# Inuri04/pgtg

Hardware: AMD Instinct MI355X
Metric: env-steps/sec (batched random-action rollout) at 1/2/4/8 MI355X (higher is better)
Workload: dtype int32; 1 GPU; configs[4]: 1048576 envs of 5x5 procedural maps split over the GPUs, random actions, auto-reset, RCCL-reduced global step counter; envs_total=1048576, envs_per_gpu=1048576, map=5x5, autoreset=True, parallelism=dp1 (env shards, no data-path collective)

## Files before the change

pgtg_amd/csrc/pgtg_env.hip:

```cpp
#include <hip/hip_runtime.h>

#include <math.h>
#include <stdint.h>
#include <stdio.h>
#include <stdlib.h>
#include <string.h>

#include <algorithm>
#include <array>
#include <cstddef>
#include <string>
#include <vector>

#include "pgtg_device.h"
#include "pgtg_episode.h"
#include "pgtg_rollout.h"
#include "pgtg_policy.h"
#include "pgtg_snapshot.h"

namespace pgtg {
namespace dv {
#define PGTG_TBL_QUAL __constant__ static const
#include "pgtg_tables.h"
#undef PGTG_TBL_QUAL
}
namespace hs {
#define PGTG_TBL_QUAL static const
#include "pgtg_tables.h"
#undef PGTG_TBL_QUAL
}

__shared__ __attribute__((aligned(16))) TablesHead sT;
__shared__ __attribute__((aligned(16))) TablesTail sTX;

__device__ __forceinline__ void stage_bytes(const void* __restrict__ gsrc, void* ldst, int bytes) {
  const int n4 = bytes >> 4, tid = (int)threadIdx.x;
  const uint4* src = reinterpret_cast<const uint4*>(gsrc);
  uint4* dst = reinterpret_cast<uint4*>(ldst);
  uint4 r[4];
#pragma unroll
  for (int j = 0; j < 4; j++) r[j] = src[tid + j * kBlock < n4 ? tid + j * kBlock : 0];
#pragma unroll
  for (int j = 0; j < 4; j++)
    if (tid + j * kBlock < n4) dst[tid + j * kBlock] = r[j];
  for (int k = tid + 4 * kBlock; k < n4; k += kBlock) dst[k] = src[k];
  for (int k = n4 * 4 + tid; k < bytes / 4; k += kBlock)
    reinterpret_cast<uint32_t*>(ldst)[k] = reinterpret_cast<const uint32_t*>(gsrc)[k];
}
__device__ __forceinline__ void stage_tables(const Tables* __restrict__ gtab, bool tail) {
  stage_bytes(gtab, &sT, (int)sizeof(TablesHead));
  if (tail) stage_bytes(reinterpret_cast<const uint8_t*>(gtab) + kTabHead, &sTX, (int)sizeof(TablesTail));
}

__device__ __forceinline__ void lds_barrier() {
  __builtin_amdgcn_fence(__ATOMIC_RELEASE, "workgroup", "local");
  __builtin_amdgcn_s_barrier();
  __builtin_amdgcn_fence(__ATOMIC_ACQUIRE, "workgroup", "local");
}

template <bool BIG>
__device__ __forceinline__ void stage_plan(const uint16_t* __restrict__ plan, int nq, uint32_t* dst, int pdw) {
  const uint4* src = reinterpret_cast<const uint4*>(plan);
  for (int k0 = 0; k0 < (BIG ? nq : 1); k0 += 8) {
    uint4 q[8];
#pragma unroll
    for (int k = 0; k < 8; k++) q[k] = src[k0 + k < nq ? k0 + k : k0];
#pragma unroll
    for (int k = 0; k < 8; k++) {
      if (k0 + k < nq) {
        const uint32_t wv[4] = {q[k].x, q[k].y, q[k].z, q[k].w};
#pragma unroll
        for (int j = 0; j < 4; j++)
          if ((k0 + k) * 4 + j < pdw) dst[(k0 + k) * 4 + j] = wv[j];
      }
    }
  }
}

#ifdef PGTG_STAMPS
__device__ unsigned long long g_stamps[1 << 21];
#define STAMP(k)                                                                          \
  do {                                                                                    \
    if ((threadIdx.x & 63) == 0) {                                                        \
      unsigned long long t_ = __builtin_amdgcn_s_memtime();                               \
      g_stamps[((blockIdx.x * (kBlock / 64) + (threadIdx.x >> 6)) * 32 + (k)) & ((1 << 21) - 1)] = t_; \
    }                                                                                     \
  } while (0)
#define STAMPR(k)                                                                                     \
  do {                                                                                                \
    if ((threadIdx.x & 63) == 0)                                                                      \
      g_stamps[(1 << 20) | ((((blockIdx.x * (kBlock / 64) + (threadIdx.x >> 6)) * 8 + (k))) & ((1 << 20) - 1))] = \
          __builtin_amdgcn_s_memrealtime();                                                           \
  } while (0)
#else
#define STAMP(k) \
  do {           \
  } while (0)
#define STAMPR(k) \
  do {            \
  } while (0)
#endif

__device__ __forceinline__ uint32_t bit81(const uint32_t* m3, int sq) { return (m3[sq >> 5] >> (sq & 31)) & 1u; }

__device__ __forceinline__ int seg_dir(int lx, int ly) {
  bool mx = (unsigned)(lx - 3) <= 2u, my = (unsigned)(ly - 3) <= 2u;
  if (ly == 0 && mx) return 0;
  if (lx == 8 && my) return 1;
  if (ly == 8 && mx) return 2;
  if (lx == 0 && my) return 3;
  return -1;
}

struct EnvView {
  int px, py, vx, vy;
  uint32_t phase, flags, path_len, elapsed;
  uint32_t sg, spawn;
  uint64_t used;
};

__device__ __forceinline__ EnvView rec_view(const EnvRec& e) {
  EnvView v;
  v.px = (int)(int16_t)(e.a.x & 0xffffu);
  v.py = (int)(int16_t)(e.a.x >> 16);
  v.vx = (int)(int16_t)(e.a.y & 0xffffu);
  v.vy = (int)(int16_t)(e.a.y >> 16);
  v.phase = e.a.z & 0xffffu;
  v.flags = (e.a.z >> 16) & 0xfu;
  v.path_len = e.a.z >> 20;
  v.elapsed = e.a.w;
  v.sg = e.b.x;
  v.spawn = e.b.y;
  v.used = (uint64_t)e.b.z | ((uint64_t)e.b.w << 32);
  return v;
}
__device__ __forceinline__ EnvView rec_load(const EnvRec* r, uint64_t i) { return rec_view(r[i]); }
__device__ __forceinline__ void rec_store(EnvRec* r, uint64_t i, const EnvView& v) {
  EnvRec e;
  e.a.x = ((uint32_t)v.px & 0xffffu) | ((uint32_t)v.py << 16);
  e.a.y = ((uint32_t)v.vx & 0xffffu) | ((uint32_t)v.vy << 16);
  e.a.z = (v.phase & 0xffffu) | ((v.flags & 0xfu) << 16) | (v.path_len << 20);
  e.a.w = v.elapsed;
  e.b.x = v.sg;
  e.b.y = v.spawn;
  e.b.z = (uint32_t)v.used;
  e.b.w = (uint32_t)(v.used >> 32);
  r[i] = e;
}

__device__ __forceinline__ uint32_t plan_word_mask(const DevCfg& c, int word) {
  const int t0 = 2 * word;
  return t0 + 1 < c.nt ? ~0u : (t0 < c.nt ? 0xffffu : 0u);
}
__device__ __forceinline__ void store_plan_row(const DevCfg& c, const DevState& S, uint64_t i, const uint32_t* pw, int pdw) {
  uint4* dstp = reinterpret_cast<uint4*>(S.plan + i * (uint64_t)c.plan_stride);
  for (int k = 0; k < c.plan_stride / 8; k++) {
    uint32_t wv[4];
#pragma unroll
    for (int j = 0; j < 4; j++) wv[j] = (k * 4 + j < pdw) ? pw[k * 4 + j] & plan_word_mask(c, k * 4 + j) : 0u;
    dstp[k] = make_uint4(wv[0], wv[1], wv[2], wv[3]);
  }
}

struct Plan {
  uint16_t* p;
  __device__ __forceinline__ uint32_t operator[](int t) const { return p[t]; }
};

template <bool BIG>
__device__ __forceinline__ bool used_bit(const EnvView& v, uint32_t p, int t) {
  return BIG ? (p & kPlanUsed) != 0u : ((v.used >> t) & 1ull) != 0ull;
}

template <bool BIG>
__device__ __forceinline__ uint32_t square_flags(const DevCfg& c, const Plan& pl, const EnvView& v, int x, int y) {
  int tx = x / kTile, ty = y / kTile;
  int lx = x - tx * kTile, ly = y - ty * kTile;
  int t = ty * c.tw + tx;
  uint32_t p = pl[t];
  uint32_t ex = plan_exits(p);
  int sq = lx * 9 + ly;
  uint32_t f = 0;
  uint32_t wall = bit81(sT.wall[ex], sq);
  if (wall) f |= SQ_WALL;
  int d = seg_dir(lx, ly);
  if (d >= 0 && ((ex >> d) & 1u)) {
    if (plan_sgdir(p) == d) f |= used_bit<BIG>(v, p, t) ? SQ_USED : SQ_SUBGOAL;
    if ((int)(v.sg & 0xffu) == t && (int)((v.sg >> 8) & 0xffu) == d) f |= SQ_START;
    if ((int)((v.sg >> 16) & 0xffu) == t && (int)(v.sg >> 24) == d) f |= SQ_FINAL;
  }
  const uint32_t ob = bit81(sT.obst[min(plan_omask(p), (uint32_t)PGTG_N_OBST_MASKS - 1u)], sq);
  uint32_t ot = plan_otype(p);
  if (ot && !wall && ob) f |= SQ_ICE << (ot - 1);
  return f;
}
__device__ __forceinline__ uint32_t square_lanes(const DevCfg& c, const Plan& pl, int x, int y) {
  int tx = x / kTile, ty = y / kTile;
  int lx = x - tx * kTile, ly = y - ty * kTile;
  uint32_t ex = plan_exits(pl[ty * c.tw + tx]);
  return ex ? sTX.lanes[ex][lx * 9 + ly] : 0u;
}
__device__ __forceinline__ bool square_spawner(const DevCfg& c, const Plan& pl, int x, int y) {
  int tx = x / kTile, ty = y / kTile;
  int lx = x - tx * kTile, ly = y - ty * kTile;
  uint32_t ex = plan_exits(pl[ty * c.tw + tx]);
  if (!ex) return false;
  int sq = lx * 9 + ly;
  if (bit81(sT.spawner[ex], sq)) return true;
  uint32_t l = sTX.lanes[ex][sq];
  return (tx == 0 && (l >> 31 & 1u)) || (tx == c.tw - 1 && (l >> 30 & 1u)) || (ty == 0 && (l >> 29 & 1u)) ||
         (ty == c.th - 1 && (l >> 28 & 1u));
}
__device__ __forceinline__ bool inside(const DevCfg& c, int x, int y) {
  return (unsigned)x < (unsigned)c.W && (unsigned)y < (unsigned)c.H;
}
__device__ __forceinline__ int phase_color(const DevCfg& c, uint32_t ph) {
  return (int)ph < c.phase_g ? 0 : ((int)ph < c.phase_gy ? 1 : 2);
}

__device__ __forceinline__ int lane_slot_tw(int tw, const Plan& pl, int x, int y) {
  int tx = x / kTile, ty = y / kTile;
  int lx = x - tx * kTile, ly = y - ty * kTile;
  int t = ty * tw + tx;
  uint32_t ex = plan_exits(pl[t]);
  const int li_raw = sTX.li[ex][lx * 9 + ly];
  const int li = ex ? li_raw : 255;
  return li == 255 ? -1 : t * 32 + li;
}
__device__ __forceinline__ int lane_slot(const DevCfg& c, const Plan& pl, int x, int y) {
  return lane_slot_tw(c.tw, pl, x, y);
}
__device__ __forceinline__ int pinned(int x) {
  __asm__ volatile("" : "+s"(x));
  return x;
}
__device__ __forceinline__ bool square_tlight(const DevCfg& c, const Plan& pl, int x, int y) {
  int tx = x / kTile, ty = y / kTile;
  int lx = x - tx * kTile, ly = y - ty * kTile;
  uint32_t p = pl[ty * c.tw + tx];
  int sq = lx * 9 + ly;
  return plan_otype(p) == 4 && !bit81(sT.wall[plan_exits(p)], sq) && bit81(sT.obst[plan_omask(p)], sq);
}
#ifndef PGTG_OCC_MAX
#define PGTG_OCC_MAX 15
#endif
constexpr int kOccMax = PGTG_OCC_MAX;
static_assert(kOccMax >= 1 && kOccMax <= 15, "4-bit occupancy counters");
__device__ __forceinline__ int occ_get(const uint8_t* o, int s) { return (o[s >> 1] >> ((s & 1) << 2)) & 15; }
__device__ __forceinline__ void occ_put(uint8_t* o, int s, int v) {
  const int sh = (s & 1) << 2;
  o[s >> 1] = (uint8_t)((o[s >> 1] & ~(15 << sh)) | (v << sh));
}
__device__ __forceinline__ void occ_inc(uint8_t* o, int s, bool& sat) {
  const int v = occ_get(o, s);
  if (v >= kOccMax) sat = true;
  else occ_put(o, s, v + 1);
}
__device__ __forceinline__ int occ_at(const DevCfg& c, const Plan& pl, const uint8_t* occ, int x, int y) {
  int s = lane_slot(c, pl, x, y);
  return s < 0 ? 0 : occ_get(occ, s);
}
__device__ __forceinline__ int select32(uint32_t x, int k) {
  int pos = 0;
#pragma unroll
  for (int sh = 16; sh >= 1; sh >>= 1) {
    const int c = __popc(x & ((1u << sh) - 1u));
    const bool up = k >= c;
    k -= up ? c : 0;
    x = up ? x >> sh : x;
    pos += up ? sh : 0;
  }
  return (x & 1u) && k == 0 ? pos : -1;
}
__device__ __forceinline__ int kth_bit(uint32_t m, int k) {
  for (int j = 0; j < k; j++) m &= m - 1u;
  return __ffs((int)m) - 1;
}

struct ProfileCdf {
  uint64_t t[4];
};
__device__ __forceinline__ ProfileCdf pin_profile_cdf(const DevCfg& c) {
  ProfileCdf p;
#pragma unroll
  for (int j = 0; j < 4; j++) {
    uint64_t x = c.profile_t[j];
    __asm__ volatile("" : "+s"(x));
    p.t[j] = x;
  }
  return p;
}
__device__ __forceinline__ int profile_of(const ProfileCdf& p, uint64_t u) {
  int prof = 0;
#pragma unroll
  for (int j = 0; j < 4; j++) prof += (u < p.t[j]) ? 0 : 1;
  return prof;
}

constexpr uint32_t kCarEmpty = 1u << 31;
typedef __attribute__((address_space(1))) uint32_t gu32;
struct CarSlots {
  gu32 *w0, *w1, *id;
  uint64_t n;
  __device__ __forceinline__ CarSlots(const DevState& S, uint64_t i)
      : w0((gu32*)(S.car_w0 + i)), w1((gu32*)(S.car_w1 + i)), id((gu32*)(S.car_id + i)), n(S.n) {
    __asm__ volatile("" : "+v"(w0), "+v"(w1), "+v"(id));
  }
// ... 1981 lines not shown
    }
    if (f & SQ_ICE) {
      used_ice = true;
      if (pcg_double(ice) < c.ice_p) {
        int a = (int)pcg_int(ice, 9);
        pxp = acc_x(a);
        pyp = acc_y(a);
      }
    }
    if (f & SQ_BROKEN) {
      used_broken = true;
      if (pcg_double(broken) < c.broken_p) v.flags |= kFlagFlatTire;
    }
    if (f & SQ_SAND) {
      used_sand = true;
      if (pcg_double(sand) < c.sand_p) {
        cx += pxp;
        cy += pyp;
        v.vx = v.vy = 0;
        break;
      }
    }
    cx += pxp;
    cy += pyp;
  }
  (void)gl_t;
  (void)gl_d;
  if (used_ice) stream_store_state(S.ice, i, ice);
  if (used_broken) stream_store_state(S.broken, i, broken);
  if (used_sand) stream_store_state(S.sand, i, sand);
  if (v.flags & kFlagFlatTire) v.vx = v.vy = 0;
  const bool accel = !(ax == 0 && ay == 0);
  if (S.visited) {
    uint32_t* vis = S.visited + i * (uint64_t)c.vis_words;
    int b = (cx + 2) * c.vis_pitch + (cy + 2);
    if (c.visited_penalty != 0.0 && accel && ((vis[b >> 5] >> (b & 31)) & 1u)) {
      if (c.separate_cost) cost += c.visited_penalty; else reward -= c.visited_penalty;
    }
    vis[b >> 5] |= 1u << (b & 31);
  }
  const int ox = v.px, oy = v.py;
  v.px = cx;
  v.py = cy;
  if (c.still_penalty != 0.0 && !accel && ox == cx && oy == cy) {
    if (c.separate_cost) cost += c.still_penalty; else reward -= c.still_penalty;
  }
  v.elapsed += 1u;
  if (c.max_steps > 0 && (int)v.elapsed >= c.max_steps) v.flags |= kFlagTruncated;
  res.reward = c.separate_cost ? perf : reward;
  res.cost = cost;
  return 0;
}

__device__ __forceinline__ uint32_t expand4(uint32_t x) { return ((x & 15u) * 0x00204081u) & 0x01010101u; }
__device__ __forceinline__ uint32_t udiv_f(uint32_t x, uint32_t d, float inv) {
  uint32_t q = (uint32_t)((float)x * inv);
  if (q * d > x) q--;
  if ((q + 1) * d <= x) q++;
  return q;
}

__device__ __forceinline__ void mark_lines(uint32_t* lm, const uint8_t* dst, uint32_t e, uint32_t OB) {
  const uintptr_t a0 = (uintptr_t)dst, base = a0 >> 7;
  uint32_t l = (uint32_t)(((a0 + (uintptr_t)e * OB) >> 7) - base);
  const uint32_t l1 = (uint32_t)(((a0 + (uintptr_t)(e + 1) * OB - 1) >> 7) - base);
  while (l <= l1) {
    const uint32_t hi = min(l1, l | 31u), n = hi - l + 1u;
    __hip_atomic_fetch_or(lm + (l >> 5), (n == 32u ? ~0u : ((1u << n) - 1u)) << (l & 31u), __ATOMIC_RELAXED,
                          __HIP_MEMORY_SCOPE_WORKGROUP);
    l = hi + 1u;
  }
}

__device__ __forceinline__ void write_obs(uint8_t* __restrict__ dst, uint32_t cnt, uint32_t OB, const uint32_t* st,
                                          const uint8_t* sel, int rank = -1, int nthr = kBlock,
                                          const uint32_t* lm = nullptr) {
  if (rank < 0) rank = (int)threadIdx.x;
  const uint32_t total = cnt * OB;
  const uintptr_t a0 = (uintptr_t)dst;
  const uintptr_t c0 = a0 & ~(uintptr_t)15;
  const uint32_t nchunks = (uint32_t)((a0 + total - c0 + 15) >> 4);
  const float invOB = 1.0f / (float)OB;
  for (uint32_t ch = (uint32_t)rank; ch < nchunks; ch += (uint32_t)nthr) {
    const int r = (int)((intptr_t)(c0 + ((uintptr_t)ch << 4)) - (intptr_t)a0);
    if (lm) {
      const uint32_t li = (uint32_t)(((c0 + ((uintptr_t)ch << 4)) >> 7) - (a0 >> 7));
      if (!((lm[li >> 5] >> (li & 31u)) & 1u)) continue;
    } else if (sel) {
      const intptr_t l0 = (intptr_t)((c0 + ((uintptr_t)ch << 4)) & ~(uintptr_t)127) - (intptr_t)a0;
      const uint32_t llo = l0 < 0 ? 0u : (uint32_t)l0;
      const uint32_t lhi = min((uint32_t)(l0 + 127), total - 1u);
      const uint32_t e0 = udiv_f(llo, OB, invOB), e1 = udiv_f(lhi, OB, invOB);
      bool any = false;
      for (uint32_t e = e0; e <= e1; e++) any = any || sel[e] == 1;
      if (!any) continue;
    }
    uint8_t* cp = dst + r;
    if (r >= 0 && (uint32_t)r + 16u <= total) {
      const uint32_t w = (uint32_t)r >> 5;
      const uint64_t two = (uint64_t)st[w] | ((uint64_t)st[w + 1] << 32);
      const uint32_t bits = (uint32_t)(two >> (r & 31));
#ifdef PGTG_NT_OBS
      typedef unsigned int v4u __attribute__((ext_vector_type(4)));
      v4u o = {expand4(bits), expand4(bits >> 4), expand4(bits >> 8), expand4(bits >> 12)};
      __builtin_nontemporal_store(o, reinterpret_cast<v4u*>(cp));
#else
      *reinterpret_cast<uint4*>(cp) = make_uint4(expand4(bits), expand4(bits >> 4), expand4(bits >> 8), expand4(bits >> 12));
#endif
    } else {
      for (int b = 0; b < 16; b++) {
        const int rb = r + b;
        if (rb >= 0 && (uint32_t)rb < total) cp[b] = (uint8_t)((st[rb >> 5] >> (rb & 31)) & 1u);
      }
    }
  }
}

struct Lds {
  int envs;
  int plan_stride_dw;
  int scratch_dw;
  int traf_dw;
  int hist_dw;
  int seg_bits;
  int sub_envs;
  int stream_words;
  int spread;
  int compact;
  int queue;
  int gen_off;
  int lm_words;
  int stagger;
  int stagger_wgs;
  int ramp_pct;
  int img_in_traf;
  int prio;
  int abl;
};
constexpr int kQueueLanes = 64;
constexpr int kMaxQueueGrid = 4096;
constexpr int kQctrBlocks = 2 * kMaxQueueGrid;
constexpr int kQctrOvfLen = kQctrBlocks + 3;
constexpr int kQctrWords = kQctrOvfLen + 24;
__device__ __forceinline__ uint32_t wave_sum(uint32_t x) {
#pragma unroll
  for (int o = 32; o > 0; o >>= 1) x += (uint32_t)__shfl_xor((int)x, o);
  return x;
}
__host__ __device__ inline uint64_t queue_req_cap(uint64_t nblk, uint64_t grid, int envs) {
  const uint64_t c = 3 * ((nblk + grid - 1) / grid) * (uint64_t)envs;
  return c < (uint64_t)kQueueLanes ? (uint64_t)kQueueLanes : c;
}
constexpr uint64_t kStaggerMaxTicks = 20000;
constexpr int kQueueDepth = 2;
constexpr int kBlockDepth = 3;
constexpr uint32_t kQueueStale = 0x80u;
constexpr int kViewDw = 8;

__host__ __device__ inline uint32_t queue_tag(uint32_t spawn) { return ~spawn; }
__host__ __device__ inline int odd_up(int x) { return x | 1; }
__host__ inline int img_words(int envs, int bits) { return ((int)(((int64_t)envs * bits + 31) / 32) + 2 + 3) & ~3; }

__host__ inline void lds_tail(Lds& l, const DevCfg& c);
__host__ inline Lds lds_layout(const DevCfg& c, int envs) {
  Lds l;
  l.envs = envs;
  l.plan_stride_dw = odd_up((c.nt + 1) / 2);
  l.scratch_dw = c.need_car ? 0 : 3;
  l.traf_dw = c.need_car ? odd_up(c.traf_bytes / 4) : 0;
  l.hist_dw = (c.n_rules > 0 || c.need_car) ? 5 : 0;
  l.seg_bits = c.n_channels * c.win * c.win;
  const int budget_words = 12 * 1024;
  int sub = l.seg_bits > 0 ? (int)(((int64_t)budget_words - 3) * 32 / l.seg_bits) : envs;
  l.sub_envs = sub > envs ? envs : (sub < 1 ? 1 : sub);
  l.stream_words = img_words(l.sub_envs, l.seg_bits);
  l.spread = c.need_car ? 1 : 0;
  l.compact = 1;
  l.queue = !c.need_car && c.n_rules == 0 && !c.fixed_map && !c.generic_channels && envs <= kBlock - 64 && l.sub_envs >= envs;
  l.stagger = 0;
  l.stagger_wgs = 0;
  l.ramp_pct = 25;
  l.img_in_traf = 0;
  l.abl = 0;
  l.prio = 0;
#ifdef PGTG_TUNING
  if (const char* e = getenv("PGTG_ABL")) l.abl = atoi(e);
  if (const char* e = getenv("PGTG_PRIO")) l.prio = atoi(e);
  if (const char* e = getenv("PGTG_RAMP")) l.ramp_pct = atoi(e);
  if (const char* e = getenv("PGTG_SPREAD")) l.spread = atoi(e);
  if (const char* e = getenv("PGTG_COMPACT")) l.compact = atoi(e);
  if (const char* e = getenv("PGTG_QUEUE")) l.queue = l.queue && atoi(e);
#endif
  lds_tail(l, c);
  return l;
}
__host__ inline int tail_bytes(const Lds& l) {
  return kBlock + (l.queue ? 128 : 32) + 4 * l.lm_words + (l.queue && l.envs <= 32 ? 4 * kViewDw * l.envs : 0);
}
__host__ inline void lds_tail(Lds& l, const DevCfg& c) {
  const int64_t total = (int64_t)l.envs * l.seg_bits;
  const int lines = (int)((127 + total) / 128) + 1;
  l.lm_words = (!c.need_car && l.sub_envs >= l.envs && lines <= 64 * 32) ? (lines + 31) / 32 : 0;
#ifdef PGTG_TUNING
  if (const char* e = getenv("PGTG_LINEMASK")) l.lm_words = atoi(e) ? l.lm_words : 0;
#endif
  l.gen_off = (int)(((size_t)l.envs * (l.plan_stride_dw + l.scratch_dw + l.traf_dw + l.hist_dw) + l.stream_words) +
                    tail_bytes(l) / 4);
}
__host__ inline size_t lds_bytes(const Lds& l) {
  return (size_t)4 * ((size_t)l.envs * (l.plan_stride_dw + l.scratch_dw + l.traf_dw + l.hist_dw) + l.stream_words) +
         tail_bytes(l) + (l.queue ? (size_t)4 * kQueueLanes * l.plan_stride_dw : 0);
}

__host__ inline void lds_img_in_traf(Lds& l, const DevCfg& c) {
  if (!c.need_car || !c.obs_fast || l.envs < 1) return;
  if ((int64_t)img_words(l.envs, l.seg_bits) > (int64_t)l.envs * l.traf_dw) return;
  l.img_in_traf = 1;
  l.sub_envs = l.envs;
  l.stream_words = 0;
  l.hist_dw = 7;
  lds_tail(l, c);
}

enum { MODE_STEP = 0, MODE_RESET_SEEDED = 1, MODE_RESET_UNSEEDED = 2, MODE_OBSERVE = 3 };

__device__ __forceinline__ void write_small_outputs(const DevCfg& c, const PgtgOutputs& o, uint64_t i, const EnvView& v,
                                                    const ObsInfo& oi, bool final) {
  if (!final) {
    if (o.position) reinterpret_cast<int2*>(o.position)[i] = make_int2(oi.posx, oi.posy);
    if (o.velocity) reinterpret_cast<int2*>(o.velocity)[i] = make_int2(v.vx, v.vy);
    if (o.next_subgoal) o.next_subgoal[i] = oi.nsd;
  } else {
    if (o.final_position) reinterpret_cast<int2*>(o.final_position)[i] = make_int2(oi.posx, oi.posy);
    if (o.final_velocity) reinterpret_cast<int2*>(o.final_velocity)[i] = make_int2(v.vx, v.vy);
    if (o.final_next_subgoal) o.final_next_subgoal[i] = oi.nsd;
  }
}

template <bool TR, bool BIG>
__device__ __forceinline__ void obs_pass(const DevCfg& c, const DevState& S, const Plan& pl, const EnvView& v,
                                         const PgtgOutputs& o, uint8_t* dst, uint64_t env0, int nb, bool want,
                                         bool final, const uint8_t* sel, uint32_t* st, const Lds& L,
                                         const uint8_t* occ, int slot) {
  for (int sb = 0; sb < nb; sb += L.sub_envs) {
    const int cnt = min(L.sub_envs, nb - sb);
    if (want && slot >= sb && slot < sb + cnt) {
      ObsInfo oi;
      build_obs<TR, BIG, true, !TR>(c, S, pl, v, st, (uint32_t)(slot - sb) * (uint32_t)c.obs_bytes, oi, occ);
      write_small_outputs(c, o, env0 + slot, v, oi, final);
    }
    lds_barrier();
    if (dst)
      write_obs(dst + (env0 + sb) * (uint64_t)c.obs_bytes, (uint32_t)cnt, (uint32_t)c.obs_bytes, st, sel ? sel + sb : nullptr);
    lds_barrier();
  }
}

__device__ __forceinline__ uint64_t stagger_start(const Lds& L, const DevState& S) {
  if (!L.stagger) return 0;
  const uint64_t t0 = wall_clock64();
  if (blockIdx.x == 0 || blockIdx.x >= (unsigned)L.stagger_wgs) return t0;
  const uint64_t span = min(S.wg_ticks[0] * (uint64_t)L.ramp_pct / 100ull, (unsigned long long)kStaggerMaxTicks);
  const uint64_t wait = span * blockIdx.x / (unsigned)L.stagger_wgs;
  while (wall_clock64() - t0 < wait) __builtin_amdgcn_s_sleep(16);
  return t0;
}
__device__ __forceinline__ void stagger_record(const Lds& L, const DevState& S, uint64_t t0) {
  if (L.stagger && blockIdx.x == 0 && threadIdx.x == 0) S.wg_ticks[0] = wall_clock64() - t0;
}

template <bool TR, bool BIG>
__global__ void __launch_bounds__(kBlock, TR ? 3 : 4) k_env(const DevCfg* __restrict__ cfg, const Tables* __restrict__ gtab,
                                                 DevState S, const uint8_t* __restrict__ actions,
                                                 const uint8_t* __restrict__ mask, PgtgOutputs out, int mode, Lds L,
                                                 uint32_t tr_slot) {
  extern __shared__ uint32_t lds[];
  const DevCfg& c = *cfg;
  const int tid = threadIdx.x;
  const uint64_t t_start = TR ? 0 : stagger_start(L, S);
  STAMP(0);
  if ((TR && c.need_car) && mode != MODE_OBSERVE && blockIdx.x == 0 && tid == 0) S.tr_count[tr_slot ^ 1u] = 0u;
  stage_tables(gtab, c.generic_channels || (TR && c.need_car));
  const uint64_t env0 = (uint64_t)blockIdx.x * L.envs;
  const int nb = (int)min((uint64_t)L.envs, S.n - env0);
  const int per_wave = (!L.spread || L.envs >= kBlock) ? 64 : L.envs / 4;
  const bool has_slot = (tid & 63) < per_wave;
  const int slot = has_slot ? (tid >> 6) * per_wave + (tid & 63) : 0;
  const uint64_t i = env0 + slot;
  const bool live = has_slot && slot < nb;
  const int my_slot = slot;
  uint32_t* plan_w = lds + my_slot * L.plan_stride_dw;
  uint32_t* traf_w = lds + L.envs * (L.plan_stride_dw + L.scratch_dw) + my_slot * L.traf_dw;
  uint32_t* hist_w = lds + L.envs * (L.plan_stride_dw + L.scratch_dw + L.traf_dw) + my_slot * L.hist_dw;
  const int env_dw = L.plan_stride_dw + L.scratch_dw + L.traf_dw + L.hist_dw;
  uint32_t* st = (TR && L.img_in_traf) ? lds + L.envs * (L.plan_stride_dw + L.scratch_dw) : lds + L.envs * env_dw;
  uint8_t* sel = reinterpret_cast<uint8_t*>(lds + L.envs * env_dw + L.stream_words);
  uint64_t* wmask = reinterpret_cast<uint64_t*>(sel + kBlock);
  uint32_t* lm = L.lm_words ? reinterpret_cast<uint32_t*>(sel + kBlock + 32) : nullptr;
  const bool img_traf = TR && L.img_in_traf;
  const int xf_off = img_traf ? L.envs * (L.plan_stride_dw + L.scratch_dw + L.traf_dw) + 4
                   : L.envs * L.plan_stride_dw + ((TR && c.need_car) ? L.envs * L.scratch_dw : 0);
  const int xf_dw = img_traf ? L.hist_dw : (TR && c.need_car) ? L.traf_dw : L.scratch_dw;
  uint32_t* xf = lds + xf_off + my_slot * xf_dw;
  uint8_t* occ = reinterpret_cast<uint8_t*>(traf_w);
  uint16_t* sp_l = reinterpret_cast<uint16_t*>(occ + c.sp_cache_off);
  uint8_t* hist = reinterpret_cast<uint8_t*>(hist_w);
  Plan pl{reinterpret_cast<uint16_t*>(plan_w)};

  EnvView v{};
  TrafState ts{0, 0, 0, 0};
  bool occ_sat = false;
  bool occ_valid = false;
  int err = 0;
  int act = 0;
  if (live) {
    v = rec_load(S.rec, i);
    if (mode == MODE_STEP) act = actions[i];
    if ((TR && c.need_car)) {
      uint4 tr4 = S.traf[i];
      ts.n_cars = tr4.x & 0xffffu;
      ts.n_spawners = tr4.x >> 16;
      ts.next_id = tr4.y;
      ts.tail = tr4.z;
      ts.fresh = (tr4.w & kTrafFresh) ? 1u : 0u;
      occ_valid = (tr4.w & kTrafOccValid) != 0u;
    }
    stage_plan<BIG>(S.plan + i * (uint64_t)c.plan_stride, c.plan_dq, plan_w, L.plan_stride_dw);
  }
  for (int k = tid; k < L.lm_words; k += kBlock) lm[k] = 0u;
  lds_barrier();
  if (live && (TR && c.need_car) && occ_valid) {
    const int nw = c.nt * 4;
    const gu32* ob = ts.fresh ? fresh_block(S, i) + S.fresh_occ : (const gu32*)(S.occ + i);
    const uint64_t ostep = ts.fresh ? 1ull : S.n;
    for (int w0 = 0; w0 < nw; w0 += 16) {
      uint32_t r[16];
#pragma unroll
      for (int u = 0; u < 16; u++) r[u] = ob[(uint64_t)min(w0 + u, nw - 1) * ostep];
#pragma unroll
      for (int u = 0; u < 16; u++)
        if (w0 + u < nw) traf_w[w0 + u] = r[u];
    }
  }
  if (live && (TR && c.need_car) && !occ_valid) {
    for (int w = 0; w < c.nt * 4; w++) traf_w[w] = 0u;
    const CarSlots cs(S, i);
    const gu32* rb = ts.fresh ? fresh_block(S, i) : cs.w0;
    const uint64_t rstep = ts.fresh ? 1ull : S.n;
    const int tail = (int)ts.tail, tw = pinned(c.tw);
    uint32_t nx16[16];
#pragma unroll
    for (int g = 0; g < 16; g++) nx16[g] = rb[(uint64_t)(g < tail ? g : 0) * rstep];
    for (int k0 = 0; k0 < tail; k0 += 16) {
      uint32_t a16[16];
#pragma unroll
      for (int g = 0; g < 16; g++) a16[g] = nx16[g];
#pragma unroll
      for (int g = 0; g < 16; g++) nx16[g] = rb[(uint64_t)(k0 + 16 + g < tail ? k0 + 16 + g : 0) * rstep];
      int sl[16];
#pragma unroll
      for (int g = 0; g < 16; g++) sl[g] = lane_slot_tw(tw, pl, (int)(a16[g] & 255u), (int)((a16[g] >> 8) & 255u));
#pragma unroll
      for (int g = 0; g < 16; g++) {
        if (k0 + g < tail && !(a16[g] & kCarEmpty)) {
          if (sl[g] < 0) err = PGTG_E_UNSUPPORTED;
          else occ_inc(occ, sl[g], occ_sat);
        }
      }
    }
  }
  if (live && (TR && c.need_car)) {
    const int nsp = min((int)ts.n_spawners, kSpCache);
    const uint4* src = reinterpret_cast<const uint4*>(S.spawners + i * (uint64_t)S.sp_pitch);
    const int q_last = (int)(S.sp_pitch / 8u) - 1;
    uint4 q4[kSpCache / 8];
#pragma unroll
    for (int q = 0; q < kSpCache / 8; q++) q4[q] = src[min(q, q_last)];
    uint32_t* dl = reinterpret_cast<uint32_t*>(sp_l);
#pragma unroll
    for (int q = 0; q < kSpCache / 8; q++) {
      if (q * 8 < nsp) {
        dl[4 * q] = q4[q].x;
        dl[4 * q + 1] = q4[q].y;
        dl[4 * q + 2] = q4[q].z;
        dl[4 * q + 3] = q4[q].w;
      }
    }
  }
  STAMP(1);
  uint8_t my_sel = 0;
  if (live) {
    if (mode == MODE_STEP) {
      StepResult res{0.0, 0.0, 0u};
      if (!err) err = env_step<TR, BIG>(c, S, i, v, pl, act, res, occ, occ_sat, sp_l, ts, hist);
      if ((TR && c.need_car) && !occ_sat) {
        const int nw = c.nt * 4;
        for (int w = 0; w < nw; w++) S.occ[(uint64_t)w * S.n + i] = traf_w[w];
      }
      occ_valid = (TR && c.need_car) && !occ_sat && err == 0;
      const bool done = (v.flags & (kFlagTerminated | kFlagTruncated)) != 0;
      if (BIG && res.plan_dirty && !(done && c.autoreset && err == 0)) store_plan_row(c, S, i, plan_w, L.plan_stride_dw);
      if (out.reward) out.reward[i] = res.reward;
      if (out.cost) out.cost[i] = res.cost;
      if (out.terminated) out.terminated[i] = (v.flags & kFlagTerminated) ? 1 : 0;
      if (out.truncated) out.truncated[i] = (v.flags & kFlagTruncated) ? 1 : 0;
      if (out.braking) out.braking[i] = (uint8_t)res.triggered;
      my_sel = (done && c.autoreset && err == 0) ? 1 : 0;
      if (lm && my_sel && out.final_obs) mark_lines(lm, out.final_obs + env0 * (uint64_t)c.obs_bytes, (uint32_t)slot, (uint32_t)c.obs_bytes);
    } else if (mode == MODE_RESET_SEEDED || mode == MODE_RESET_UNSEEDED) {
      const bool do_reset = mask == nullptr || mask[i] != 0;
      if (do_reset && mode == MODE_RESET_SEEDED) v.spawn = 0;
      my_sel = do_reset ? 2 : 0;
    }
  }
  if (has_slot) sel[slot] = my_sel;
  const uint8_t* occ_img = occ;
  if (img_traf) {
    if (live) {
      const int pix = min(max(0, v.px), c.W - 1), piy = min(max(0, v.py), c.H - 1);
      const int t = (piy / kTile) * c.tw + pix / kTile;
#pragma unroll
      for (int q = 0; q < 4; q++) hist_w[q] = traf_w[t * 4 + q];
    }
    occ_img = hist;
  }
  STAMP(2);
  const bool single = L.sub_envs >= nb;
  const bool reset_now = my_sel != 0;
  if (L.compact) {
    const uint64_t m = __ballot(reset_now);
    if ((tid & 63) == 0) wmask[tid >> 6] = m;
  }
  int n_final = 0;
  if (L.compact) {
    lds_barrier();
    if (mode == MODE_STEP)
      for (int w = 0; w < kBlock / 64; w++) n_final += __popcll(wmask[w]);
  } else {
    n_final = __syncthreads_count(my_sel == 1);
  }
  const bool want_final = mode == MODE_STEP && n_final && (out.final_obs || out.final_position || out.final_velocity);
  int n_resets = 0, wslot = -1;
  if (L.compact) {
#pragma unroll
    for (int w = 0; w < kBlock / 64; w++) {
      const uint64_t m = wmask[w];
      const int cw = __popcll(m);
      if (tid >= n_resets && tid < n_resets + cw) wslot = w * per_wave + select64(m, tid - n_resets);
      n_resets += cw;
    }
  }
  const int t_help = L.compact ? ((n_resets + 63) / 64) * 64
                               : ((L.spread || L.envs >= kBlock) ? kBlock : ((L.envs + 63) / 64) * 64);
  const bool helpers = single && t_help < kBlock;
  if (single) {
    if (live && (my_sel != 2)) {
      ObsInfo oi;
      build_obs<TR, BIG, true, !TR>(c, S, pl, v, st, (uint32_t)slot * (uint32_t)c.obs_bytes, oi, occ_img, 0, -1, true, false, img_traf);
      write_small_outputs(c, out, i, v, oi, my_sel == 1);
    }
    if (L.compact && reset_now) xf[0] = v.spawn;
    STAMP(28);
    lds_barrier();
    STAMP(29);
    if (want_final && out.final_obs && !helpers)
      write_obs(out.final_obs + env0 * (uint64_t)c.obs_bytes, (uint32_t)nb, (uint32_t)c.obs_bytes, st, sel, -1, kBlock, lm);
  } else {
    if (want_final) obs_pass<TR, BIG>(c, S, pl, v, out, out.final_obs, env0, nb, my_sel == 1, true, sel, st, L, occ, slot);
    if (L.compact) {
      if (reset_now) xf[0] = v.spawn;
      lds_barrier();
    }
  }
  STAMP(3);
  bool tr_push = false;
  if (!L.compact) n_resets = __syncthreads_count(reset_now);
  if (tid == 0 && n_resets) atomicAdd(&S.counters[1], (unsigned long long)n_resets);
  if (helpers && want_final && out.final_obs && tid >= t_help)
    write_obs(out.final_obs + env0 * (uint64_t)c.obs_bytes, (uint32_t)nb, (uint32_t)c.obs_bytes, st, sel, tid - t_help,
              kBlock - t_help, lm);
  if (L.compact) {
    if (wslot >= 0) {
      uint32_t* xw = lds + xf_off + wslot * xf_dw;
      uint32_t* pw = lds + wslot * L.plan_stride_dw;
      const uint64_t iw = env0 + wslot;
      EnvView vv{};
      vv.spawn = xw[0];
      TrafState tw{0, 0, 0, 0};
      const int e2 = env_reset<TR, BIG>(c, S, iw, vv, reinterpret_cast<uint16_t*>(pw), tw);
      store_plan_row(c, S, iw, pw, L.plan_stride_dw);
      xw[0] = ((uint32_t)vv.px & 0xffffu) | ((uint32_t)vv.py << 16);
      xw[1] = vv.sg;
      xw[2] = vv.path_len | (uint32_t)(-e2) << 16;
    }
    lds_barrier();
    if (reset_now) {
      const uint32_t x0 = xf[0], x2 = xf[2];
      v.px = (int)(int16_t)(x0 & 0xffffu);
      v.py = (int)(int16_t)(x0 >> 16);
      v.sg = xf[1];
      v.path_len = x2 & 0xffffu;
      v.spawn += 5u;
      v.used = 0;
      v.flags = 0;
      v.phase = 0;
      v.elapsed = 0;
      v.vx = v.vy = 0;
      const int e2 = -(int)(x2 >> 16);
      if (e2) err = e2;
      tr_push = (TR && c.need_car) && e2 == 0;
      if ((TR && c.need_car) && e2 == 0) ts = TrafState{0, 0, 0, 0};
    }
  } else if (reset_now) {
    int e2 = env_reset<TR, BIG>(c, S, i, v, pl.p, ts);
    if (e2) err = e2;
    tr_push = (TR && c.need_car) && e2 == 0;
    store_plan_row(c, S, i, plan_w, L.plan_stride_dw);
  }
  STAMP(4);
  if (live) {
    if (mode != MODE_OBSERVE) {
      rec_store(S.rec, i, v);
      if ((TR && c.need_car))
        S.traf[i] = make_uint4(ts.n_cars | ts.n_spawners << 16, ts.next_id, ts.tail,
                               (occ_valid && !reset_now ? kTrafOccValid : 0u) | (ts.fresh ? kTrafFresh : 0u));
    }
    if (mode != MODE_OBSERVE || err) S.err[i] = (uint8_t)(-err);
    if (S.qstate && reset_now) S.qstate[i] = (uint8_t)kQueueStale;
  }
  if (TR && c.need_car) {
    const uint64_t m = __ballot(tr_push);
    if (m) {
      const int lane = tid & 63, leader = __ffsll((long long)m) - 1;
      uint32_t base = 0;
      if (lane == leader) base = atomicAdd(&S.tr_count[tr_slot], (uint32_t)__popcll(m));
      base = __shfl(base, leader);
      if (tr_push) S.tr_list[base + __popcll(m & ((1ull << lane) - 1ull))] = (uint32_t)i;
    }
  }
  STAMP(5);
  if (single) {
    if (helpers && !L.compact) lds_barrier();
    if (reset_now) {
      ObsInfo oi;
      build_obs<TR, BIG, true, !TR>(c, S, pl, v, st, (uint32_t)slot * (uint32_t)c.obs_bytes, oi, nullptr);
      write_small_outputs(c, out, i, v, oi, false);
    }
    STAMP(30);
    lds_barrier();
    STAMP(31);
    if (out.obs)
      write_obs(out.obs + env0 * (uint64_t)c.obs_bytes, (uint32_t)nb, (uint32_t)c.obs_bytes, st, nullptr);
  } else {
    obs_pass<TR, BIG>(c, S, pl, v, out, out.obs, env0, nb, live, false, nullptr, st, L, reset_now ? nullptr : occ,
                 slot);
  }
  if (mode == MODE_STEP && tid == 0) atomicAdd(&S.counters[0], (unsigned long long)nb);
  if (!TR) stagger_record(L, S, t_start);
  STAMP(6);
  if (TR) STAMPR(0);
}

template <bool BIG>
__device__ __forceinline__ void gen_queue_entry(const DevCfg& c, const DevState& S, uint64_t i, uint32_t k,
                                                uint16_t* plan, int pdw, uint32_t* __restrict__ dst,
                                                bool no_store = false, bool fold_ok = true) {
  SeedPool sp = ss_pool(S.seed[i]);
  Pcg map_rng = ss_child(sp, k);
  int st_t, st_d, gl_t, gl_d;
  uint64_t ix[4];
  generate_map<BIG>(c, BIG ? S.epk : sT.epk, map_rng, plan, st_t, st_d, gl_t, gl_d, ix);
  uint64_t dirs[4] = {0ull, 0ull, 0ull, 0ull};
  const bool fold = !BIG && c.dual && fold_ok;
  int len = compile_generated<BIG>(c, plan, st_t, gl_t, ix, fold ? dirs : nullptr);
  int px = 0, py = 0, err = 0;
  if (len <= 0 || !((plan_exits(plan[st_t]) >> st_d) & 1u)) {
    err = len < 0 ? PGTG_E_DEVICE : PGTG_E_MAP;
    len = 0;
  } else {
    const int j = (int)pcg_int(map_rng, 3);
    const int tx = st_t % c.tw, ty = st_t / c.tw;
    int lx, ly;
    switch (st_d) {
      case 0: lx = 3 + j; ly = 0; break;
      case 1: lx = 8; ly = 3 + j; break;
      case 2: lx = 3 + j; ly = 8; break;
      default: lx = 0; ly = 3 + j; break;
    }
    px = tx * kTile + lx;
    py = ty * kTile + ly;
  }
  const uint32_t* pw = reinterpret_cast<const uint32_t*>(plan);
  uint4* d4 = reinterpret_cast<uint4*>(dst);
  const int pwords = c.plan_dq * 4;
#ifdef PGTG_TUNING
  if (no_store) {
    if (len == 12345 && px == 7) d4[0] = make_uint4(0, 0, 0, 0);
    return;
  }
#endif
  for (int q = 0; q < pwords / 4; q++) {
    uint32_t wv[4];
#pragma unroll
    for (int j = 0; j < 4; j++) {
      wv[j] = (q * 4 + j < pdw) ? (pw[q * 4 + j] & plan_word_mask(c, q * 4 + j)) : 0u;
      if (fold) {
        const int t0 = 2 * (q * 4 + j);
        const uint32_t d0 = (uint32_t)((dirs[0] >> t0) & 1ull) + 2u * (uint32_t)((dirs[1] >> t0) & 1ull) +
                            3u * (uint32_t)((dirs[2] >> t0) & 1ull) + 4u * (uint32_t)((dirs[3] >> t0) & 1ull);
        const uint32_t d1 = t0 + 1 < 64 ? (uint32_t)((dirs[0] >> (t0 + 1)) & 1ull) + 2u * (uint32_t)((dirs[1] >> (t0 + 1)) & 1ull) +
                                          3u * (uint32_t)((dirs[2] >> (t0 + 1)) & 1ull) + 4u * (uint32_t)((dirs[3] >> (t0 + 1)) & 1ull)
                                        : 0u;
        wv[j] |= (d0 << 11 | d1 << 27) & plan_word_mask(c, q * 4 + j);
      }
    }
    d4[q] = make_uint4(wv[0], wv[1], wv[2], wv[3]);
  }
  d4[pwords / 4] = make_uint4(((uint32_t)px & 0xffffu) | ((uint32_t)py << 16),
                              (uint32_t)st_t | (uint32_t)st_d << 8 | (uint32_t)gl_t << 16 | (uint32_t)gl_d << 24,
                              (uint32_t)len | (uint32_t)(-err) << 16, queue_tag(k));
  for (int q = pwords / 4 + 1; q < c.qrec_dw / 4; q++) d4[q] = make_uint4(0u, 0u, 0u, 0u);
}

#ifdef PGTG_TUNING
#define ABLATE(L, bit) (((L).abl & (bit)) != 0)
#else
#define ABLATE(L, bit) false
#endif

__device__ __forceinline__ void sub_barrier(uint32_t* ctr, uint32_t target) {
  __builtin_amdgcn_fence(__ATOMIC_RELEASE, "workgroup", "local");
  if ((threadIdx.x & 63) == 0) __hip_atomic_fetch_add(ctr, 1u, __ATOMIC_RELAXED, __HIP_MEMORY_SCOPE_WORKGROUP);
  while (__hip_atomic_load(ctr, __ATOMIC_RELAXED, __HIP_MEMORY_SCOPE_WORKGROUP) < target) __builtin_amdgcn_s_sleep(1);
  __builtin_amdgcn_fence(__ATOMIC_ACQUIRE, "workgroup", "local");
}

template <bool BIG>
__device__ __forceinline__ void group_obs(const DevCfg& c, const DevState& S, const EnvView& v, bool want,
                                          uint32_t* st, ObsInfo& oi, const Lds& L, int wave, int lane,
                                          uint32_t* ctr, uint32_t& bar, int np, int rank, uint32_t* vw,
                                          bool post = true) {
  const int vtid = wave * 64 + lane;
  const int E = L.envs;
  if (E <= 32) {
    if (wave == 0 && lane < E) {
      uint32_t* q = vw + lane * kViewDw;
      q[0] = (uint32_t)v.px;
      q[1] = (uint32_t)v.py;
      q[2] = v.sg;
      q[3] = v.phase;
      q[4] = (uint32_t)v.used;
      q[5] = (uint32_t)(v.used >> 32);
      q[6] = want ? 1u : 0u;
    }
    sub_barrier(ctr, bar += (uint32_t)np);
    STAMP(post ? 9 : 16);
    const int G = np * 64 / E, e = rank % E, sub = rank / E;
    if (sub >= G) return;
    const uint32_t* q = vw + e * kViewDw;
    if (!q[6]) return;
    const int C = c.n_channels, lo = sub * C / G, hi = (sub + 1) * C / G;
    if (lo == hi && sub != 0) return;
    EnvView ve{};
    ve.px = (int)q[0];
    ve.py = (int)q[1];
    ve.sg = q[2];
    ve.phase = q[3];
    ve.used = (uint64_t)q[4] | (uint64_t)q[5] << 32;
    STAMP(post ? 10 : 17);
    extern __shared__ uint32_t lds[];
    const Plan pl{reinterpret_cast<uint16_t*>(lds + e * L.plan_stride_dw)};
    build_obs<false, BIG, false, false>(c, S, pl, ve, st, (uint32_t)e * (uint32_t)c.obs_bytes, oi, nullptr, lo, hi, sub == 0,
                                 true);
    STAMP(post ? 11 : 18);
    return;
  }
  if (want) {
    extern __shared__ uint32_t lds[];
    const int slot = vtid;
    const Plan pl{reinterpret_cast<uint16_t*>(lds + slot * L.plan_stride_dw)};
    build_obs<false, BIG, false, false>(c, S, pl, v, st, (uint32_t)slot * (uint32_t)c.obs_bytes, oi, nullptr);
  }
}

template <bool BIG>
__device__ __forceinline__ uint3 ring_take(const DevCfg& c, const DevState& S, const Lds& L, uint64_t i, uint32_t qh,
                                           uint32_t k0, uint32_t* plan_w, int pdw, int depth = kQueueDepth) {
  const uint4* q4 = reinterpret_cast<const uint4*>(S.qbuf + (i * (uint64_t)depth + qh) * (uint64_t)c.qrec_dw);
  uint4* dstp = reinterpret_cast<uint4*>(S.plan + i * (uint64_t)c.plan_stride);
  const int nq = c.plan_dq;
  const uint4 meta = q4[nq];
  for (int k0q = 0; k0q < (BIG ? nq : 1); k0q += 8) {
    uint4 qw[8];
#pragma unroll
    for (int k = 0; k < 8; k++) qw[k] = q4[k0q + k < nq ? k0q + k : k0q];
#pragma unroll
    for (int k = 0; k < 8; k++) {
      if (k0q + k < nq) {
        if (!ABLATE(L, 32)) dstp[k0q + k] = qw[k];
        const uint32_t wv[4] = {qw[k].x, qw[k].y, qw[k].z, qw[k].w};
#pragma unroll
        for (int j = 0; j < 4; j++)
          if ((k0q + k) * 4 + j < pdw) plan_w[(k0q + k) * 4 + j] = wv[j];
      }
    }
  }
  if (!ABLATE(L, 32))
    for (int k = nq; k < c.plan_stride / 8; k++) dstp[k] = make_uint4(0u, 0u, 0u, 0u);
  if (c.need_ice || c.need_broken || c.need_sand) {
    SeedPool sp = ss_pool(S.seed[i]);
    if (c.need_ice) stream_store_all(S.ice, i, ss_child(sp, k0 + 2u));
    if (c.need_broken) stream_store_all(S.broken, i, ss_child(sp, k0 + 3u));
    if (c.need_sand) stream_store_all(S.sand, i, ss_child(sp, k0 + 4u));
  }
  const int e2 = (meta.w != queue_tag(k0) && !ABLATE(L, 1 | 16)) ? PGTG_E_DEVICE : -(int)(meta.z >> 16);
  return make_uint3(meta.x, meta.y, (meta.z & 0xffffu) | (uint32_t)(-e2) << 16);
}

template <bool BIG>
__global__ void __launch_bounds__(kBlock, 4) k_envq(const DevCfg* __restrict__ cfg, const Tables* __restrict__ gtab,
                                                    DevState S, const uint8_t* __restrict__ actions, PgtgOutputs out,
                                                    Lds L, uint32_t qsel) {
  extern __shared__ uint32_t lds[];
  const DevCfg& c = *cfg;
  const int tid = threadIdx.x, wave = tid >> 6, lane = tid & 63;
  const uint64_t t_start = stagger_start(L, S);
  STAMP(0);
  STAMPR(2);
  const int env_waves = (L.envs + 63) / 64, gen_wave = env_waves;
  const bool env_wave = wave < env_waves;
  const uint32_t par = qsel >> 2;
  const uint64_t nblk = (S.n + (uint64_t)L.envs - 1) / (uint64_t)L.envs;
  const uint64_t cap = queue_req_cap(nblk, gridDim.x, L.envs);
  uint2* req_new = S.qreq + ((uint64_t)par * gridDim.x + blockIdx.x) * cap;
  const uint2* req_old = S.qreq + ((uint64_t)(par ^ 1u) * gridDim.x + blockIdx.x) * cap;
  const bool one_round = nblk <= gridDim.x;
  const uint32_t ox = blockIdx.x & 7u, set_new = qsel & 3u, set_old = (set_new + 2u) % 3u;
  const uint64_t ocap = ((gridDim.x + 7u) / 8u) * (uint64_t)L.envs;
  uint32_t cnt = 0;
  uint2 r0 = make_uint2(0u, 0u);
  if (wave == gen_wave) {
    cnt = S.qctr[(par ^ 1u) * gridDim.x + blockIdx.x];
    r0 = req_old[lane];
  }
  if (blockIdx.x == 0 && tid < 8) S.qctr[kQctrOvfLen + ((set_new + 1u) % 3u) * 8u + tid] = 0u;
  const int pdw = L.plan_stride_dw;
  stage_tables(gtab, false);
  uint32_t* st = lds + L.envs * (pdw + L.scratch_dw + L.traf_dw + L.hist_dw);
  uint8_t* sel = reinterpret_cast<uint8_t*>(st + L.stream_words);
  uint32_t* ctr = reinterpret_cast<uint32_t*>(sel + kBlock);
  uint32_t* lm = L.lm_words ? reinterpret_cast<uint32_t*>(sel + kBlock + 128) : nullptr;
  uint32_t* vw = reinterpret_cast<uint32_t*>(sel + kBlock + 128) + L.lm_words;
  uint32_t* qn = ctr + 1;
  uint32_t* nxt = ctr + 2;
  uint32_t* bctr = S.qctr + kQctrBlocks;
  if (blockIdx.x == 0 && tid == 0) bctr[((qsel & 3u) + 1u) % 3u] = 0u;
  if (tid == 0) {
    *ctr = 0u;
    *qn = 0u;
  }
  lds_barrier();

  if (wave == gen_wave) {
    STAMP(1);
    uint16_t* gplan = reinterpret_cast<uint16_t*>(lds + L.gen_off + lane * pdw);
    uint32_t made = 0, ovs = 0;
    if (!ABLATE(L, 1)) {
      const uint2* ovf = S.qovf + ((uint64_t)(par ^ 1u) * 8u + ox) * ocap;
      uint32_t ob = 0, on = 0, olen = 0, tot = 0;
      const uint32_t nj = (gridDim.x - ox + 7u) / 8u, jme = blockIdx.x / 8u;
      if (one_round) {
        olen = S.qctr[kQctrOvfLen + set_old * 8u + ox];
        if (olen > 0) {
          uint32_t pre = 0;
          for (uint32_t j0 = 0; j0 < nj; j0 += kQueueLanes) {
            const uint32_t j = j0 + (uint32_t)lane;
            const uint32_t sp = j < nj ? kQueueLanes - min(S.qctr[(par ^ 1u) * gridDim.x + ox + 8u * j], (uint32_t)kQueueLanes) : 0u;
            pre += wave_sum(j < jme ? sp : 0u);
            tot += wave_sum(sp);
          }
          on = olen > pre ? min(olen - pre, kQueueLanes - min(cnt, (uint32_t)kQueueLanes)) : 0u;
          ob = pre;
        }
      }
      for (uint32_t base = 0;; base += kQueueLanes) {
        const uint32_t own = base < cnt ? min((uint32_t)kQueueLanes, cnt - base) : 0u;
        const uint32_t oth = base == 0 ? on : 0u;
        if (own + oth == 0) break;
        made += own + oth;
        ovs += oth;
        if ((uint32_t)lane < own + oth) {
          const uint2 r = (uint32_t)lane >= own ? ovf[ob + (lane - own)] : base == 0 ? r0 : req_old[base + lane];
          const uint64_t ie = r.x >> 1;
          gen_queue_entry<BIG>(c, S, ie, r.y, gplan, pdw, S.qbuf + (ie * kQueueDepth + (r.x & 1u)) * (uint64_t)c.qrec_dw,
                               ABLATE(L, 16), false);
        }
        if (base + kQueueLanes >= cnt) break;
      }
      for (uint64_t st0 = tot + (uint64_t)jme * kQueueLanes; st0 < olen; st0 += (uint64_t)nj * kQueueLanes) {
        const uint32_t m = (uint32_t)min((uint64_t)kQueueLanes, olen - st0);
        made += m;
        ovs += m;
        if ((uint32_t)lane < m) {
          const uint2 r = ovf[st0 + lane];
          const uint64_t ie = r.x >> 1;
          gen_queue_entry<BIG>(c, S, ie, r.y, gplan, pdw, S.qbuf + (ie * kQueueDepth + (r.x & 1u)) * (uint64_t)c.qrec_dw,
                               ABLATE(L, 16), false);
        }
      }
    }
    if (lane == 0 && made) atomicAdd(&S.counters[2], (unsigned long long)made);
    if (lane == 0 && ovs) atomicAdd(&S.counters[3], (unsigned long long)ovs);
    STAMP(7);
    STAMPR(3);
    return;
  }

  const int np = kBlock / 64 - 1;
  const int nthr = np * 64;
  uint32_t bar = 0;
  for (uint64_t blk = blockIdx.x; blk < nblk;) {
    STAMP(0);
    uint32_t got = 0xffffffffu;
    if (tid == 0 && nblk > gridDim.x && *qn + 2u * (uint32_t)L.envs <= cap) got = atomicAdd(&bctr[qsel & 3u], 1u);
    int tid_o = tid;
    asm volatile("" : "+v"(tid_o));
    const int lane = tid_o & 63;
    const int rank = (wave < gen_wave ? wave : wave - 1) * 64 + lane;
    const int slot = tid_o;
    uint32_t* plan_w = lds + (env_wave ? slot : 0) * pdw;
    Plan pl{reinterpret_cast<uint16_t*>(plan_w)};
    const uint64_t env0 = blk * (uint64_t)L.envs;
    const int nb = (int)min((uint64_t)L.envs, S.n - env0);
    const uint64_t i = env0 + slot;
    const bool live = env_wave && slot < nb;
    EnvView v{};
    uint32_t qh = 0;
    int act = 0;
    if (live) {
      v = rec_load(S.rec, i);
      qh = S.qstate[i] & 1u;
      act = actions[i];
      stage_plan<BIG>(S.plan + i * (uint64_t)c.plan_stride, c.plan_dq, plan_w, pdw);
    }
    for (int k = rank; k < L.lm_words; k += nthr) lm[k] = 0u;
    sub_barrier(ctr, bar += (uint32_t)np);
    STAMP(1);
    uint8_t my_sel = 0;
    int err = 0;
    if (live) {
      StepResult res{0.0, 0.0, 0u};
      bool occ_sat = false;
      TrafState ts{0, 0, 0, 0};
      err = env_step<false, BIG>(c, S, i, v, pl, act, res, nullptr, occ_sat, nullptr, ts, nullptr);
      STAMP(22);
      const bool done = (v.flags & (kFlagTerminated | kFlagTruncated)) != 0;
      if (out.reward) out.reward[i] = res.reward;
      if (out.cost) out.cost[i] = res.cost;
      if (out.terminated) out.terminated[i] = (v.flags & kFlagTerminated) ? 1 : 0;
      if (out.truncated) out.truncated[i] = (v.flags & kFlagTruncated) ? 1 : 0;
      if (out.braking) out.braking[i] = 0;
      my_sel = (done && c.autoreset && err == 0) ? 1 : 0;
      if (BIG && res.plan_dirty && !my_sel) store_plan_row(c, S, i, plan_w, pdw);
      if (lm && my_sel && out.final_obs) mark_lines(lm, out.final_obs + env0 * (uint64_t)c.obs_bytes, (uint32_t)slot, (uint32_t)c.obs_bytes);
      STAMP(23);
    }
    {
      ObsInfo oi;
      group_obs<BIG>(c, S, v, live, st, oi, L, wave, lane, ctr, bar, np, rank, vw);
      if (live) write_small_outputs(c, out, i, v, oi, my_sel == 1);
    }
    if (env_wave) sel[slot] = my_sel;
    const uint64_t rm = __ballot(my_sel == 1);
    if (env_wave && lane == 0 && rm) atomicAdd(&S.counters[1], (unsigned long long)__popcll(rm));
    STAMP(2);
    STAMP(28);
    sub_barrier(ctr, bar += (uint32_t)np);
    STAMP(29);
    if (out.final_obs && !ABLATE(L, 2))
      write_obs(out.final_obs + env0 * (uint64_t)c.obs_bytes, (uint32_t)nb, (uint32_t)c.obs_bytes, st, sel, rank, nthr, lm);
    STAMP(3);
    sub_barrier(ctr, bar += (uint32_t)np);
    const bool reset_now = my_sel != 0;
    const uint32_t k0 = v.spawn;
    if (reset_now) {
      const uint4* q4 = reinterpret_cast<const uint4*>(S.qbuf + (i * kQueueDepth + qh) * (uint64_t)c.qrec_dw);
      uint4* dstp = reinterpret_cast<uint4*>(S.plan + i * (uint64_t)c.plan_stride);
      const int nq = c.plan_dq;
      const uint4 meta = q4[nq];
      for (int k0q = 0; k0q < (BIG ? nq : 1); k0q += 8) {
        uint4 qw[8];
#pragma unroll
        for (int k = 0; k < 8; k++) qw[k] = q4[k0q + k < nq ? k0q + k : k0q];
#pragma unroll
        for (int k = 0; k < 8; k++) {
          if (k0q + k < nq) {
            if (!ABLATE(L, 32)) dstp[k0q + k] = qw[k];
            const uint32_t wv[4] = {qw[k].x, qw[k].y, qw[k].z, qw[k].w};
#pragma unroll
            for (int j = 0; j < 4; j++)
              if ((k0q + k) * 4 + j < pdw) plan_w[(k0q + k) * 4 + j] = wv[j];
          }
        }
      }
      if (!ABLATE(L, 32))
        for (int k = nq; k < c.plan_stride / 8; k++) dstp[k] = make_uint4(0u, 0u, 0u, 0u);
      if (c.need_ice || c.need_broken || c.need_sand) {
        SeedPool sp = ss_pool(S.seed[i]);
        if (c.need_ice) stream_store_all(S.ice, i, ss_child(sp, k0 + 2u));
        if (c.need_broken) stream_store_all(S.broken, i, ss_child(sp, k0 + 3u));
        if (c.need_sand) stream_store_all(S.sand, i, ss_child(sp, k0 + 4u));
      }
      v.spawn = k0 + 5u;
      v.sg = meta.y;
      v.used = 0;
      v.path_len = meta.z & 0xffffu;
      v.flags = 0;
      v.phase = 0;
      v.elapsed = 0;
      v.vx = v.vy = 0;
      v.px = (int)(int16_t)(meta.x & 0xffffu);
      v.py = (int)(int16_t)(meta.x >> 16);
      const int e2 = (meta.w != queue_tag(k0) && !ABLATE(L, 1 | 16)) ? PGTG_E_DEVICE : -(int)(meta.z >> 16);
      if (e2) err = e2;
      if (S.visited && e2 == 0) {
        uint32_t* vis = S.visited + i * (uint64_t)c.vis_words;
        for (int q2 = 0; q2 < c.vis_words; q2++) vis[q2] = 0;
        int b = (v.px + 2) * c.vis_pitch + (v.py + 2);
        vis[b >> 5] |= 1u << (b & 31);
      }
    }
    STAMP(4);
    const uint64_t rb = __ballot(reset_now);
    if (rb) {
      uint32_t base = 0;
      if (lane == 0) base = atomicAdd(qn, (uint32_t)__popcll(rb));
      base = __builtin_amdgcn_readfirstlane(base);
      const uint32_t k = (uint32_t)__popcll(rb);
      const uint32_t ovn = (one_round && base + k > (uint32_t)kQueueLanes) ? base + k - max(base, (uint32_t)kQueueLanes) : 0u;
      uint32_t obase = 0;
      if (ovn) {
        if (lane == 0) obase = atomicAdd(&S.qctr[kQctrOvfLen + set_new * 8u + ox], ovn);
        obase = __builtin_amdgcn_readfirstlane(obase);
      }
      if (reset_now) {
        const uint32_t p = base + (uint32_t)__popcll(rb & ((1ull << lane) - 1ull));
        const uint2 r = make_uint2((uint32_t)i << 1 | qh, k0 + 10u);
        if (one_round && p >= (uint32_t)kQueueLanes)
          S.qovf[((uint64_t)par * 8u + ox) * ocap + obase + (p - max(base, (uint32_t)kQueueLanes))] = r;
        else
          req_new[p] = r;
        S.qstate[i] = (uint8_t)(qh ^ 1u);
      }
    }
    if (live) {
      rec_store(S.rec, i, v);
      S.err[i] = (uint8_t)(-err);
    }
    STAMP(5);
    {
      ObsInfo oi;
      group_obs<BIG>(c, S, v, reset_now, st, oi, L, wave, lane, ctr, bar, np, rank, vw, false);
      if (reset_now) write_small_outputs(c, out, i, v, oi, false);
    }
    if (tid == 0) *nxt = got;
    STAMP(30);
    sub_barrier(ctr, bar += (uint32_t)np);
    STAMP(31);
    if (tid == 0)
      S.qctr[par * gridDim.x + blockIdx.x] = one_round ? min(*qn, (uint32_t)kQueueLanes) : *qn;
    const uint32_t g = *nxt;
    if (out.obs && !ABLATE(L, 4))
      write_obs(out.obs + env0 * (uint64_t)c.obs_bytes, (uint32_t)nb, (uint32_t)c.obs_bytes, st, nullptr, rank, nthr);
    if (tid == 0) atomicAdd(&S.counters[0], (unsigned long long)nb);
    if (blk == blockIdx.x) stagger_record(L, S, t_start);
    STAMP(6);
    blk = g == 0xffffffffu ? nblk : (uint64_t)gridDim.x + g;
  }  STAMPR(3);
}

template <bool BIG>
__global__ void __launch_bounds__(kBlock, 4) k_envb(const DevCfg* __restrict__ cfg, const Tables* __restrict__ gtab,
                                                    DevState S, const uint8_t* __restrict__ actions, PgtgOutputs out,
                                                    Lds L) {
  extern __shared__ uint32_t lds[];
  const DevCfg& c = *cfg;
  const int tid = threadIdx.x, wave = tid >> 6, lane = tid & 63;
  const uint64_t t_start = stagger_start(L, S);
  STAMP(0);
  STAMPR(2);
  stage_tables(gtab, false);
  const uint64_t env0 = (uint64_t)blockIdx.x * L.envs;
  const int nb = (int)min((uint64_t)L.envs, S.n - env0);
  const int env_waves = (L.envs + 63) / 64, gen_wave = env_waves;
#ifdef PGTG_TUNING
  if (wave != gen_wave) {
    if (L.prio == 1) __builtin_amdgcn_s_setprio(1);
    else if (L.prio == 2) __builtin_amdgcn_s_setprio(2);
    else if (L.prio == 3) __builtin_amdgcn_s_setprio(3);
  }
#endif
  const int qcap = env_waves > 2 ? 2 * kQueueLanes : kQueueLanes;
  const bool env_wave = wave < env_waves;
  const int slot = tid;
  const uint64_t i = env0 + slot;
  const bool live = env_wave && slot < nb;
  const int pdw = L.plan_stride_dw;
  uint32_t* plan_w = lds + (env_wave ? slot : 0) * pdw;
  uint32_t* xf = lds + L.envs * pdw;
  uint32_t* st = lds + L.envs * (pdw + L.scratch_dw + L.traf_dw + L.hist_dw);
  uint8_t* sel = reinterpret_cast<uint8_t*>(st + L.stream_words);
  uint64_t* fm = reinterpret_cast<uint64_t*>(sel + kBlock);
  uint32_t* ctr = reinterpret_cast<uint32_t*>(fm + 3 * kBlockDepth);
  uint32_t* lm = L.lm_words ? reinterpret_cast<uint32_t*>(sel + kBlock + 128) : nullptr;
  uint32_t* vw = reinterpret_cast<uint32_t*>(sel + kBlock + 128) + L.lm_words;
  Plan pl{reinterpret_cast<uint16_t*>(plan_w)};

  EnvView v{};
  uint32_t qs = 0;
  int act = 0;
  if (live) {
    v = rec_load(S.rec, i);
    qs = S.qstate[i];
    act = actions[i];
    stage_plan<BIG>(S.plan + i * (uint64_t)c.plan_stride, c.plan_dq, plan_w, pdw);
    xf[slot * L.scratch_dw] = v.spawn;
    xf[slot * L.scratch_dw + 1] = qs;
  }
  const uint32_t qn = qs & 3u, qh = (qs >> 2) & 3u;
  if (env_wave) {
#pragma unroll
    for (int l = 0; l < kBlockDepth; l++) {
      const uint64_t m = __ballot(live && qn <= (uint32_t)l);
      if (lane == 0) fm[l * 3 + wave] = m;
    }
  }
  if (tid == 0) *ctr = 0u;
  for (int k = tid; k < L.lm_words; k += kBlock) lm[k] = 0u;
  lds_barrier();
  STAMP(1);
  int F[kBlockDepth];
#pragma unroll
  for (int l = 0; l < kBlockDepth; l++) {
    F[l] = 0;
    for (int w = 0; w < env_waves; w++) F[l] += __popcll(fm[l * 3 + w]);
  }
  const bool any_empty = F[0] != 0;
#ifdef PGTG_STAMPS
  if ((threadIdx.x & 63) == 0)
    g_stamps[((blockIdx.x * (kBlock / 64) + (threadIdx.x >> 6)) * 32 + 12) & ((1 << 21) - 1)] =
        (unsigned long long)F[0] | (unsigned long long)F[1] << 16 | (unsigned long long)F[2] << 32;
#endif

  if (wave == gen_wave) {
    uint16_t* gplan = reinterpret_cast<uint16_t*>(lds + L.gen_off + lane * pdw);
    auto refill = [&](int k, int l) {
      int e = 0, pre = 0;
      for (int w = 0; w < env_waves; w++) {
        const uint64_t m = fm[l * 3 + w];
        const int cw = __popcll(m);
        if (k >= pre && k < pre + cw) e = w * 64 + select64(m, k - pre);
        pre += cw;
      }
      const uint64_t ie = env0 + e;
      const uint32_t qe = xf[e * L.scratch_dw + 1];
      const uint32_t rslot = (((qe >> 2) & 3u) + (uint32_t)l) % (uint32_t)kBlockDepth;
      gen_queue_entry<BIG>(c, S, ie, xf[e * L.scratch_dw] + 5u * (uint32_t)l, gplan, pdw,
                      S.qbuf + (ie * kBlockDepth + rslot) * (uint64_t)c.qrec_dw, ABLATE(L, 16), !ABLATE(L, 512));
    };
    if (ABLATE(L, 1)) {
      if (any_empty) __syncthreads();
      return;
    }
    for (int k = lane; k < F[0]; k += kQueueLanes) refill(k, 0);
    if (any_empty) __syncthreads();
    for (int k0 = lane; k0 < qcap; k0 += kQueueLanes) {
      int k = k0, l = 1;
      while (l < kBlockDepth && k >= F[l]) {
        k -= F[l];
        l++;
      }
      if (l < kBlockDepth) refill(k, l);
    }
    if (lane == 0) {
      int rest = 0;
      for (int l = 1; l < kBlockDepth; l++) rest += F[l];
      atomicAdd(&S.counters[2], (unsigned long long)(F[0] + min(rest, qcap)));
    }
    STAMP(7);
    STAMPR(3);
    return;
  }

  const int np = kBlock / 64 - 1;
  const int rank = (wave < gen_wave ? wave : wave - 1) * 64 + lane, nthr = np * 64;
  uint32_t bar = 0;
  uint8_t my_sel = 0;
  int err = 0;
  if (live) {
    StepResult res{0.0, 0.0, 0u};
    bool occ_sat = false;
    TrafState ts{0, 0, 0, 0};
    err = env_step<false, BIG>(c, S, i, v, pl, act, res, nullptr, occ_sat, nullptr, ts, nullptr);
    STAMP(22);
    const bool done = (v.flags & (kFlagTerminated | kFlagTruncated)) != 0;
    if (out.reward) out.reward[i] = res.reward;
    if (out.cost) out.cost[i] = res.cost;
    if (out.terminated) out.terminated[i] = (v.flags & kFlagTerminated) ? 1 : 0;
    if (out.truncated) out.truncated[i] = (v.flags & kFlagTruncated) ? 1 : 0;
    if (out.braking) out.braking[i] = 0;
    my_sel = (done && c.autoreset && err == 0) ? 1 : 0;
    if (BIG && res.plan_dirty && !my_sel) store_plan_row(c, S, i, plan_w, pdw);
    if (lm && my_sel && out.final_obs) mark_lines(lm, out.final_obs + env0 * (uint64_t)c.obs_bytes, (uint32_t)slot, (uint32_t)c.obs_bytes);
    STAMP(23);
  }
  {
    ObsInfo oi;
    group_obs<BIG>(c, S, v, live, st, oi, L, wave, lane, ctr, bar, np, rank, vw);
    if (live) write_small_outputs(c, out, i, v, oi, my_sel == 1);
  }
  if (env_wave) sel[slot] = my_sel;
  const uint64_t rm = __ballot(my_sel == 1);
  if (env_wave && lane == 0 && rm) atomicAdd(&S.counters[1], (unsigned long long)__popcll(rm));
  STAMP(2);
  STAMP(28);
  sub_barrier(ctr, bar += (uint32_t)np);
  STAMP(29);
  if (out.final_obs && !ABLATE(L, 2))
    write_obs(out.final_obs + env0 * (uint64_t)c.obs_bytes, (uint32_t)nb, (uint32_t)c.obs_bytes, st,
              ABLATE(L, 128) ? nullptr : sel, rank, nthr, ABLATE(L, 128) ? nullptr : lm);
  STAMP(3);
  sub_barrier(ctr, bar += (uint32_t)np);
  if (any_empty) __syncthreads();
  const bool reset_now = my_sel != 0;
  if (reset_now) {
    const uint32_t k0 = v.spawn;
    const uint3 tk = ring_take<BIG>(c, S, L, i, qh, k0, plan_w, pdw, kBlockDepth);
    v.spawn = k0 + 5u;
    v.sg = tk.y;
    v.used = 0;
    v.path_len = tk.z & 0xffffu;
    v.flags = 0;
    v.phase = 0;
    v.elapsed = 0;
    v.vx = v.vy = 0;
    v.px = (int)(int16_t)(tk.x & 0xffffu);
    v.py = (int)(int16_t)(tk.x >> 16);
    const int e2 = -(int)(tk.z >> 16);
    if (e2) err = e2;
    if (S.visited && e2 == 0) {
      uint32_t* vis = S.visited + i * (uint64_t)c.vis_words;
      for (int q2 = 0; q2 < c.vis_words; q2++) vis[q2] = 0;
      int b = (v.px + 2) * c.vis_pitch + (v.py + 2);
      vis[b >> 5] |= 1u << (b & 31);
    }
  }
  STAMP(4);
  if (live) {
    rec_store(S.rec, i, v);
    S.err[i] = (uint8_t)(-err);
    uint32_t have = qn == 0u ? 1u : qn;
    int base = 0;
#pragma unroll
    for (int l = 1; l < kBlockDepth; l++) {
      int pre = 0;
      for (int w = 0; w < wave; w++) pre += __popcll(fm[l * 3 + w]);
      if (qn <= (uint32_t)l && base + pre + __popcll(fm[l * 3 + wave] & ((1ull << lane) - 1ull)) < qcap) have++;
      base += F[l];
    }
    const uint32_t nq = reset_now ? have - 1u : have;
    const uint32_t nh = reset_now ? (qh + 1u) % (uint32_t)kBlockDepth : qh;
    S.qstate[i] = (uint8_t)(nq | nh << 2);
  }
  STAMP(5);
  {
    ObsInfo oi;
    group_obs<BIG>(c, S, v, reset_now, st, oi, L, wave, lane, ctr, bar, np, rank, vw, false);
    if (reset_now) write_small_outputs(c, out, i, v, oi, false);
  }
  STAMP(30);
  sub_barrier(ctr, bar += (uint32_t)np);
  STAMP(31);
  if (out.obs && !ABLATE(L, 4))
    write_obs(out.obs + env0 * (uint64_t)c.obs_bytes, (uint32_t)nb, (uint32_t)c.obs_bytes, st, nullptr, rank, nthr);
  if (tid == 0) atomicAdd(&S.counters[0], (unsigned long long)nb);
  stagger_record(L, S, t_start);
  STAMP(6);
  STAMPR(3);
}


template <bool BIG>
__global__ void __launch_bounds__(kBlock) k_qfill(const DevCfg* __restrict__ cfg, const Tables* __restrict__ gtab,
                                                  DevState S, int pdw) {
  extern __shared__ uint32_t lds[];
  const DevCfg& c = *cfg;
  stage_tables(gtab, false);
  lds_barrier();
  const uint64_t i = (uint64_t)blockIdx.x * kBlock + threadIdx.x;
  uint32_t made = 0;
  if (i < S.n) {
    const uint32_t qs = S.qstate[i];
    const bool stale = (qs & kQueueStale) != 0;
    const uint32_t qh = stale ? 0u : (qs & 1u);
    const uint32_t spawn = S.rec[i].b.y;
    const int tag_w = c.plan_dq * 4 + 3;
    uint16_t* plan = reinterpret_cast<uint16_t*>(lds + threadIdx.x * pdw);
    for (uint32_t l = 0; l < (uint32_t)kQueueDepth; l++) {
      uint32_t* dst = S.qbuf + (i * kQueueDepth + (qh ^ l)) * (uint64_t)c.qrec_dw;
      if (stale || dst[tag_w] != queue_tag(spawn + 5u * l)) {
        gen_queue_entry<BIG>(c, S, i, spawn + 5u * l, plan, pdw, dst);
        made++;
      }
    }
    if (stale) S.qstate[i] = 0;
  }
  const uint32_t wsum = (uint32_t)__popcll(__ballot(made & 1u)) + 2u * (uint32_t)__popcll(__ballot(made & 2u));
  if ((threadIdx.x & 63) == 0 && wsum) atomicAdd(&S.counters[2], (unsigned long long)wsum);
}

template <bool BIG>
__global__ void __launch_bounds__(kBlock) k_qfill_b(const DevCfg* __restrict__ cfg, const Tables* __restrict__ gtab,
                                                    DevState S, int pdw) {
  extern __shared__ uint32_t lds[];
  const DevCfg& c = *cfg;
  stage_tables(gtab, false);
  lds_barrier();
  const uint64_t i = (uint64_t)blockIdx.x * kBlock + threadIdx.x;
  uint32_t made = 0;
  if (i < S.n) {
    const uint32_t qs = S.qstate[i];
    const uint32_t qn = (qs & kQueueStale) ? 0u : (qs & 3u), qh = (qs & kQueueStale) ? 0u : ((qs >> 2) & 3u);
    if (qn < (uint32_t)kBlockDepth) {
      const uint32_t spawn = S.rec[i].b.y;
      uint16_t* plan = reinterpret_cast<uint16_t*>(lds + threadIdx.x * pdw);
      for (uint32_t l = qn; l < (uint32_t)kBlockDepth; l++)
        gen_queue_entry<BIG>(c, S, i, spawn + 5u * l, plan, pdw,
                             S.qbuf + (i * kBlockDepth + (qh + l) % (uint32_t)kBlockDepth) * (uint64_t)c.qrec_dw);
      S.qstate[i] = (uint8_t)((uint32_t)kBlockDepth | qh << 2);
      made = (uint32_t)kBlockDepth - qn;
    }
  }
  const uint32_t wsum = (uint32_t)__popcll(__ballot(made & 1u)) + 2u * (uint32_t)__popcll(__ballot(made & 2u));
  if ((threadIdx.x & 63) == 0 && wsum) atomicAdd(&S.counters[2], (unsigned long long)wsum);
}

#ifdef PGTG_STAMPS
__global__ void __launch_bounds__(kBlock) k_gen_bench(const DevCfg* __restrict__ cfg, const Tables* __restrict__ gtab,
                                                      DevState S, int reps, int active, int pdw) {
  extern __shared__ uint32_t lds[];
  const DevCfg& c = *cfg;
  {
    const uint32_t* src = reinterpret_cast<const uint32_t*>(gtab);
    uint32_t* dstt = reinterpret_cast<uint32_t*>(&sT);
    for (int k = threadIdx.x; k < (int)(sizeof(TablesHead) / 4); k += blockDim.x) dstt[k] = src[k];
  }
  __syncthreads();
  const uint64_t i = (uint64_t)blockIdx.x * kBlock + threadIdx.x;
  uint16_t* plan = reinterpret_cast<uint16_t*>(lds + threadIdx.x * pdw);
  unsigned long long tg = 0, tc = 0;
  uint32_t chk = 0;
  if ((threadIdx.x & 63) < active && i < S.n) {
    SeedPool sp = ss_pool(S.seed[i]);
    for (int r = 0; r < reps; r++) {
      Pcg g = ss_child(sp, 5u * (uint32_t)r);
      int st_t, st_d, gl_t, gl_d;
      const unsigned long long t0 = __builtin_amdgcn_s_memtime();
      uint64_t ix[4];
      generate_map<false>(c, sT.epk, g, plan, st_t, st_d, gl_t, gl_d, ix);
      const unsigned long long t1 = __builtin_amdgcn_s_memtime();
      const int len = compile_generated<false>(c, plan, st_t, gl_t, ix);
      const unsigned long long t2 = __builtin_amdgcn_s_memtime();
      tg += t1 - t0;
      tc += t2 - t1;
      chk += (uint32_t)len + plan[st_t];
    }
  }
  const uint64_t wv = (uint64_t)blockIdx.x * (kBlock / 64) + (threadIdx.x >> 6);
  if ((threadIdx.x & 63) == 0) {
    g_stamps[(wv * 32 + 0) & ((1 << 21) - 1)] = tg;
    g_stamps[(wv * 32 + 1) & ((1 << 21) - 1)] = tc;
  }
  if (chk == 0xdeadbeefu) S.err[i] = 1;
}
#endif

__global__ void __launch_bounds__(kBlock) k_traffic(const DevCfg* __restrict__ cfg, const Tables* __restrict__ gtab,
                                                    DevState S, PgtgOutputs out, uint32_t tr_slot, int plan_dw,
                                                    int rs_dw, int cap_w) {
  extern __shared__ uint32_t lds[];
  STAMP(27);
  STAMPR(1);
  const DevCfg& c = *cfg;
  const uint32_t n = S.tr_count[tr_slot];
  const uint32_t W = gridDim.x * (kBlock / 64);
  const uint32_t rounds = (n + W * (uint32_t)cap_w - 1) / (W * (uint32_t)cap_w);
  if (rounds == 0) return;
  const uint32_t e = (n + W * rounds - 1) / (W * rounds);
  if ((uint64_t)blockIdx.x * (kBlock / 64) * e >= n) return;
  const int g = min(kMaxGroup, 64 / (int)e);
  const int wave = (int)(threadIdx.x >> 6), lane = (int)(threadIdx.x & 63u);
  const int slot = lane / g, sub = lane - slot * g;
  stage_tables(gtab, true);
  __syncthreads();
  STAMP(25);
#ifdef PGTG_STAMPS
  if ((threadIdx.x & 63) == 0)
    g_stamps[((blockIdx.x * (kBlock / 64) + (threadIdx.x >> 6)) * 32 + 15) & ((1 << 21) - 1)] =
        (unsigned long long)n | (unsigned long long)rounds << 32 | (unsigned long long)e << 40 | (unsigned long long)cap_w << 48;
#endif
  if ((uint32_t)slot >= e) return;
  const int ls = wave * cap_w + slot;
  uint32_t* plan_w = lds + ls * plan_dw;
  uint8_t* rs = reinterpret_cast<uint8_t*>(lds + (kBlock / 64) * cap_w * plan_dw + ls * rs_dw);
  for (uint32_t r = 0; r < rounds; r++) {
    const uint32_t j = (r * W + blockIdx.x * (kBlock / 64) + (uint32_t)wave) * e + (uint32_t)slot;
    if (j >= n) break;
    const uint64_t i = S.tr_list[j];
    if (c.nt > kSmallTiles) stage_plan<true>(S.plan + i * (uint64_t)c.plan_stride, c.plan_dq, plan_w, plan_dw);
    else stage_plan<false>(S.plan + i * (uint64_t)c.plan_stride, c.plan_dq, plan_w, plan_dw);
    Plan pl{reinterpret_cast<uint16_t*>(plan_w)};
    const EnvView v = rec_load(S.rec, i);
    const int pix = min(max(0, v.px), c.W - 1), piy = min(max(0, v.py), c.H - 1);
    const int at = (piy / kTile) * c.tw + pix / kTile;
    Pcg cr = stream_load(S.car, i);
    TrafState ts{0, 0, 0, 0};
    uint32_t CR[3] = {0u, 0u, 0u};
    const int err = traffic_reset(c, S, i, pl, cr, rs, ts, at, CR, sub, g);
    const int q0 = lane - sub;
    const int err0 = __shfl(err, q0), k0 = __shfl((int)ts.n_cars, q0);
    if (err0 == 0) {
      store_initial_counters(c, S, i, pl, rs, k0, sub, g);
      if (!c.obs_fast && c.traffic_ch >= 0 && out.obs && k0 > 0) {
        const int win = c.win;
        const int x0 = c.sliding ? v.px - c.ss : (pix / kTile) * kTile;
        const int y0 = c.sliding ? v.py - c.ss : (piy / kTile) * kTile;
        const uint16_t* sqs = reinterpret_cast<const uint16_t*>(rs);
        uint8_t* o = out.obs + i * (uint64_t)c.obs_bytes + (uint64_t)c.traffic_ch * (uint64_t)(win * win);
        for (int m = sub; m < k0; m += g) {
          const uint32_t code = sqs[m];
          const int a = (int)(code & 255u) - x0, b = (int)(code >> 8) - y0;
          if (a >= 0 && a < win && b >= 0 && b < win) o[a * win + b] = 1;
        }
      }
    }
    if (sub == 0) {
      stream_store_state(S.car, i, cr);
      S.traf[i] = make_uint4(ts.n_cars | ts.n_spawners << 16, ts.next_id, ts.tail, err == 0 ? kTrafOccValid | kTrafFresh : 0u);
      if (err) S.err[i] = (uint8_t)(-err);
      if (c.obs_fast && c.traffic_ch >= 0 && out.obs) {
        uint8_t* o = out.obs + i * (uint64_t)c.obs_bytes + (uint64_t)c.traffic_ch * 81u;
#pragma unroll
        for (int k = 0; k < 3; k++) {
          uint32_t m = CR[k];
          while (m) {
            const int b = __ffs((int)m) - 1;
            m &= m - 1u;
            o[k * 32 + b] = 1;
          }
        }
      }
    }
    wave_lds_sync();
  }
  STAMP(24);
}

__global__ void __launch_bounds__(kBlock) k_squares(const DevCfg* __restrict__ cfg, const Tables* __restrict__ gtab,
                                                    DevState S, uint64_t i, uint64_t* __restrict__ words) {
  __shared__ uint16_t plan_s[kMaxTiles];
  const DevCfg& c = *cfg;
  const int tid = threadIdx.x;
  {
    const uint32_t* src = reinterpret_cast<const uint32_t*>(gtab);
    uint32_t* dstt = reinterpret_cast<uint32_t*>(&sT);
    for (int k = tid; k < (int)(sizeof(TablesHead) / 4); k += blockDim.x) dstt[k] = src[k];
    uint32_t* dstx = reinterpret_cast<uint32_t*>(&sTX);
    for (int k = tid; k < (int)(sizeof(TablesTail) / 4); k += blockDim.x) dstx[k] = src[kTabHead / 4 + k];
    for (int t = tid; t < c.nt; t += blockDim.x) plan_s[t] = S.plan[i * (uint64_t)c.plan_stride + t];
  }
  __syncthreads();
  const EnvView v = rec_load(S.rec, i);
  const Plan pl{plan_s};
  for (int q = tid; q < c.W * c.H; q += blockDim.x) {
    const int x = q / c.H, y = q - x * c.H;
    const uint32_t f = c.nt > kSmallTiles ? square_flags<true>(c, pl, v, x, y) : square_flags<false>(c, pl, v, x, y);
    uint64_t w = square_lanes(c, pl, x, y);
    if (f & SQ_WALL) w |= 1ull << 32;
    if (square_spawner(c, pl, x, y)) w |= 1ull << 37;
    if (f & SQ_START) w |= 1ull << 38;
    if (f & SQ_SUBGOAL) w |= 1ull << 39;
    if (f & SQ_USED) w |= 1ull << 40;
    if (f & SQ_FINAL) w |= 1ull << 41;
    if (f & SQ_ICE) w |= 1ull << 42;
    if (f & SQ_BROKEN) w |= 1ull << 43;
    if (f & SQ_SAND) w |= 1ull << 44;
    if (f & SQ_TLIGHT) w |= 1ull << 45;
    words[q] = w;
  }
}

__global__ void k_random_actions(uint8_t* a, uint64_t n, uint64_t seed, uint64_t t, uint64_t offset) {
  uint64_t i = (uint64_t)blockIdx.x * blockDim.x + threadIdx.x;
  if (i >= n) return;
  const uint64_t g = i + offset;
  uint64_t z = seed ^ (t * 0x9E3779B97F4A7C15ull) ^ (g * 0xD1B54A32D192ED03ull);
  z += 0x9E3779B97F4A7C15ull;
  z = (z ^ (z >> 30)) * 0xBF58476D1CE4E5B9ull;
  z = (z ^ (z >> 27)) * 0x94D049BB133111EBull;
  z ^= z >> 31;
  a[i] = (uint8_t)(((z >> 32) * 9ull) >> 32);
}

typedef unsigned int u32x4 __attribute__((ext_vector_type(4)));
template <int U, bool NT>
__global__ void __launch_bounds__(256) k_hbm_copy(const u32x4* __restrict__ src, u32x4* __restrict__ dst, uint64_t n16) {
  const uint64_t stride = (uint64_t)gridDim.x * 256 * U;
  for (uint64_t b = (uint64_t)blockIdx.x * 256 * U + threadIdx.x; b < n16; b += stride) {
    u32x4 r[U];
#pragma unroll
    for (int j = 0; j < U; j++) {
      const uint64_t k = b + j * 256 < n16 ? b + j * 256 : b;
      r[j] = NT ? __builtin_nontemporal_load(src + k) : src[k];
    }
#pragma unroll
    for (int j = 0; j < U; j++)
      if (b + j * 256 < n16) {
        if (NT) __builtin_nontemporal_store(r[j], dst + b + j * 256);
        else dst[b + j * 256] = r[j];
      }
  }
}

__device__ __forceinline__ uint64_t dg_w(uint64_t j) {
  uint64_t z = j + 1 + 0x9E3779B97F4A7C15ull;
  z = (z ^ (z >> 30)) * 0xBF58476D1CE4E5B9ull;
  z = (z ^ (z >> 27)) * 0x94D049BB133111EBull;
  return z ^ (z >> 31);
}
__global__ void __launch_bounds__(256) k_car_digest(DevState S, uint64_t* __restrict__ out) {
  const uint64_t i = (uint64_t)blockIdx.x * blockDim.x + threadIdx.x;
  if (i >= S.n) return;
  constexpr uint64_t CB = 1ull << 40;
  const uint4 t = S.traf[i];
  const CarSlots cs(S, i);
  const bool fresh = (t.w & kTrafFresh) != 0u;
  const gu32* fb = fresh_block(S, i);
  uint64_t d = (uint64_t)(t.x & 0xffffu) * dg_w(CB), j = 0;
  for (int k = 0; k < (int)t.z; k++) {
    const uint32_t w0 = fresh ? fb[k] : cs.w0[cs.at(k)];
    if (w0 & kCarEmpty) continue;
    const uint32_t id = fresh ? (uint32_t)k : cs.id[cs.at(k)];
    const uint64_t pk = (uint64_t)id | (uint64_t)(w0 & 255u) << 32 | (uint64_t)((w0 >> 8) & 255u) << 40 |
                        (uint64_t)((w0 >> 16) & 31u) << 48 | (uint64_t)((w0 >> 21) & 7u) << 53 |
                        (uint64_t)((w0 >> 24) & 3u) << 56;
    const uint32_t w1 = fresh ? 0u : cs.w1[cs.at(k)];
    d += (pk + 1) * dg_w(CB + 1 + 2 * j) + (uint64_t)w1 * dg_w(CB + 2 + 2 * j);
    j++;
  }
  out[i] = d;
}

struct FlatArgs {
  const uint8_t* obs;
  const int32_t* pos;
  const int32_t* vel;
  const int32_t* nsd;
  const uint8_t* term;
  const uint8_t* trunc;
  void* dst;
  const double* rew;
  float* rew32;
  uint8_t* dones;
  uint8_t* tonly;
  const uint8_t* fobs;
  const int32_t* fpos;
  const int32_t* fvel;
  const int32_t* fnsd;
  void* fdst;
  uint64_t n;
  int32_t D, OB, w2, cw2, nsd_on, final;
  uint8_t order[PGTG_MAX_CHANNELS];
};
template <typename T>
__device__ __forceinline__ T flat_tail(const FlatArgs& a, int k, int nsdv, int px, int py, int vx, int vy) {
  if (a.nsd_on) {
    if (k < 9) return (T)(k == nsdv ? 1 : 0);
    k -= 9;
  }
  if (k < 9) return (T)(k == px ? 1 : 0);
  if (k < 18) return (T)(k - 9 == py ? 1 : 0);
  return (T)(k == 18 ? vx : vy);
}
typedef uint32_t u32x4 __attribute__((ext_vector_type(4)));
constexpr int kFlatU = 18;
__device__ __forceinline__ void* uniform_ptr(const void* p) {
  const uint64_t u = (uint64_t)(uintptr_t)p;
  const uint32_t lo = __builtin_amdgcn_readfirstlane((uint32_t)u), hi = __builtin_amdgcn_readfirstlane((uint32_t)(u >> 32));
  return (void*)(uintptr_t)((uint64_t)hi << 32 | lo);
}
__device__ __forceinline__ void flat_store(__amdgpu_buffer_rsrc_t r, uint32_t off, float v) {
  __builtin_amdgcn_raw_buffer_store_b32(__builtin_bit_cast(uint32_t, v), r, off, 0, 0);
}
__device__ __forceinline__ void flat_store(__amdgpu_buffer_rsrc_t r, uint32_t off, int8_t v) {
  __builtin_amdgcn_raw_buffer_store_b8((uint8_t)v, r, off, 0, 0);
}
template <typename T, int V>
__device__ __forceinline__ void flat_store_v(__amdgpu_buffer_rsrc_t r, uint32_t off, const T (&f)[V]) {
  if constexpr (V == 1) {
    flat_store(r, off, f[0]);
  } else {
    static_assert(V == 2 && sizeof(T) == 4, "pairs of float32 only");
    typedef uint32_t u32x2 __attribute__((ext_vector_type(2)));
    const u32x2 x = {__builtin_bit_cast(uint32_t, f[0]), __builtin_bit_cast(uint32_t, f[1])};
    __builtin_amdgcn_raw_buffer_store_b64(x, r, off, 0, 0);
  }
}
template <typename T, bool ONE, int V>
__global__ void __launch_bounds__(256, 6) k_flatten(FlatArgs a) {
  __shared__ uint32_t offs[kFlatU * 64];
  __shared__ uint32_t rows[512];
  __shared__ uint32_t nrows;
  const int t = threadIdx.x;
  const uint32_t D = (uint32_t)a.D, w2 = (uint32_t)a.w2, cw2 = (uint32_t)a.cw2;
  for (uint32_t j = t; j < (uint32_t)(kFlatU * 64); j += 256) {
    const uint32_t slot = j < cw2 ? j / w2 : 0u;
    offs[j] = j < cw2 ? (uint32_t)a.order[slot] * w2 + (j - slot * w2) : 0u;
  }
  if (t == 0) nrows = 0u;
  __syncthreads();
  const uint64_t K = (a.n + gridDim.x - 1) / gridDim.x;
  const uint64_t e = (uint64_t)blockIdx.x * K + (uint64_t)t;
// ... 38 lines not shown
    const uint32_t lo4 = (uint32_t)ln * 4u, ovel = ln >= 2 ? lo4 - 8u : 1u << 20, onsd = ln >= 4 ? lo4 - 16u : 1u << 20;
    uint32_t offv[NC + 1][V];
#pragma unroll
    for (int u = 0; u <= NC; u++)
#pragma unroll
      for (int h = 0; h < V; h++) {
        const uint32_t j = (uint32_t)(V * ln + h) + (u == NC ? pb : (uint32_t)u) * CH;
        offv[u][h] = j < cw2 ? offs[j] : 0u;
      }
    auto load_row = [&](uint32_t r, Row& m) {
      const uint32_t ent = __builtin_amdgcn_readfirstlane(rows[r]);
      const bool fr = ent >= 256u;
      const uint64_t er = (uint64_t)blockIdx.x * K + (ent & 255u);
      const uint8_t* orow = (fr ? a.fobs : a.obs) + er * (uint64_t)OB;
      T* row = reinterpret_cast<T*>(fr ? a.fdst : a.dst) + er * (uint64_t)D;
      const auto src = __builtin_amdgcn_make_buffer_rsrc(uniform_ptr(orow), 0, (int)OB, 0x00020000);
      m.dst = __builtin_amdgcn_make_buffer_rsrc(uniform_ptr(row), 0,
                                                __builtin_amdgcn_readfirstlane((int)(D * sizeof(T))), 0x00020000);
      m.dsto = __builtin_amdgcn_make_buffer_rsrc(uniform_ptr(row), 0,
                                                 __builtin_amdgcn_readfirstlane((int)(pb * CH * sizeof(T))), 0x00020000);
      const auto dpos = __builtin_amdgcn_make_buffer_rsrc(uniform_ptr((fr ? a.fpos : a.pos) + 2 * er), 0, 8, 0x00020000);
      const auto dvel = __builtin_amdgcn_make_buffer_rsrc(uniform_ptr((fr ? a.fvel : a.vel) + 2 * er), 0, 8, 0x00020000);
      const auto dnsd = __builtin_amdgcn_make_buffer_rsrc(
          uniform_ptr(a.nsd_on ? (fr ? a.fnsd : a.nsd) + er : (fr ? a.fpos : a.pos)), 0, a.nsd_on ? 4 : 0, 0x00020000);
      m.mv[0] = (int)__builtin_amdgcn_raw_buffer_load_b32(dpos, lo4, 0, 0);
      m.mv[1] = (int)__builtin_amdgcn_raw_buffer_load_b32(dvel, ovel, 0, 0);
      m.mv[2] = (int)__builtin_amdgcn_raw_buffer_load_b32(dnsd, onsd, 0, 0);
      m.q0 = __builtin_amdgcn_raw_buffer_load_b128(src, lo4 * 4u, 0, 0);
      m.q1 = __builtin_amdgcn_raw_buffer_load_b128(src, 1024u + lo4 * 4u, 0, 0);
      m.tb = __builtin_amdgcn_raw_buffer_load_b8(src, obt + (uint32_t)ln, 0, 0);
    };
    auto store_row = [&](const Row& m) {
      win[wv][ln] = m.q0;
      win[wv][64 + ln] = m.q1;
      if ((uint32_t)ln < OB - obt) wb[obt + (uint32_t)ln] = (uint8_t)m.tb;
      const int mv = m.mv[0] + m.mv[1] + m.mv[2];
      const int px = __builtin_amdgcn_readlane(mv, 0), py = __builtin_amdgcn_readlane(mv, 1);
      const int vx = __builtin_amdgcn_readlane(mv, 2), vy = __builtin_amdgcn_readlane(mv, 3);
      const int nsdv = __builtin_amdgcn_readlane(mv, 4) + 1;
#pragma unroll
      for (int p = 0; p < NC; p++) {
        T f[V];
#pragma unroll
        for (int h = 0; h < V; h++) f[h] = (T)wb[offv[p][h]];
        flat_store_v<T, V>(m.dsto, lo + (uint32_t)p * CH * (uint32_t)sizeof(T), f);
      }
      uint32_t obb[V];
#pragma unroll
      for (int h = 0; h < V; h++) obb[h] = wb[offv[NC][h]];
#pragma unroll
      for (int s = 0; s < 2; s++) {
        const uint32_t pc = pb + (uint32_t)s;
        T f[V];
#pragma unroll
        for (int h = 0; h < V; h++) {
          const int k = V * ln + h + (int)(pc * CH) - (int)cw2;
          const int k2 = a.nsd_on ? k - 9 : k;
          int tv = (int)(k2 == px);
          tv = k2 < 9 ? tv : (int)(k2 - 9 == py);
          tv = k2 < 18 ? tv : (k2 == 18 ? vx : vy);
          tv = (a.nsd_on && k < 9) ? (int)(k == nsdv) : tv;
          f[h] = k < 0 ? (T)obb[h] : (T)tv;
        }
        if (pc * CH < D) flat_store_v<T, V>(m.dst, lo + pc * CH * (uint32_t)sizeof(T), f);
      }
    };
    Row mA{}, mB{};
    uint32_t r = wv;
    if (r < nr) {
      load_row(r, mA);
      load_row(min(r + 4u, nr - 1u), mB);
      store_row(mA);
      r += 4u;
      while (r < nr) {
        load_row(min(r + 4u, nr - 1u), mA);
        store_row(mB);
        r += 4u;
        if (r >= nr) break;
        load_row(min(r + 4u, nr - 1u), mB);
        store_row(mA);
        r += 4u;
      }
    }
  } else {
    for (uint32_t r = wv; r < nr; r += 4u) {
      const uint32_t ent = rows[r];
      const bool fr = ent >= 256u;
      const uint64_t er = (uint64_t)blockIdx.x * K + (ent & 255u);
      const uint8_t* __restrict__ orow = (fr ? a.fobs : a.obs) + er * (uint64_t)a.OB;
      T* __restrict__ row = reinterpret_cast<T*>(fr ? a.fdst : a.dst) + er * (uint64_t)D;
      const int32_t* pos = fr ? a.fpos : a.pos;
      const int32_t* vel = fr ? a.fvel : a.vel;
      const int nsdv = a.nsd_on ? (fr ? a.fnsd : a.nsd)[er] + 1 : -1;
      const int px = pos[2 * er], py = pos[2 * er + 1], vx = vel[2 * er], vy = vel[2 * er + 1];
      for (uint32_t j0 = 0; j0 < D; j0 += kFlatU * 64u) {
        uint32_t ob[kFlatU];
#pragma unroll
        for (int u = 0; u < kFlatU; u++) {
          const uint32_t j = j0 + (uint32_t)ln + (uint32_t)u * 64u;
          const uint32_t off = j0 == 0 ? offs[j - j0] : (j < cw2 ? (uint32_t)a.order[j / w2] * w2 + j % w2 : 0u);
          ob[u] = orow[j < cw2 ? off : 0u];
        }
#pragma unroll
        for (int p = 0; p < kFlatU; p++) {
          const uint32_t j = j0 + (uint32_t)ln + (uint32_t)p * 64u;
          const T f = j < cw2 ? (T)ob[p] : flat_tail<T>(a, (int)(j - cw2), nsdv, px, py, vx, vy);
          if (j < D) row[j] = f;
        }
      }
    }
  }
}

__global__ void k_fill_seeds(uint64_t* seed, uint64_t n, uint64_t base, const uint64_t* src, const uint8_t* mask) {
  uint64_t i = (uint64_t)blockIdx.x * blockDim.x + threadIdx.x;
  if (i < n && (mask == nullptr || mask[i] != 0)) seed[i] = src ? src[i] : base + i;
}

}

using namespace pgtg;

struct pgtg_handle {
  int device = 0;
  uint64_t n = 0;
  hipStream_t stream = nullptr;
  DevCfg hcfg{};
  DevCfg* dcfg = nullptr;
  Tables* dtab = nullptr;
  DevState S{};
  PgtgOutputs out{};
  Lds L{};
  size_t lds = 0;
  std::vector<void*> allocs;
  std::string err;
  uint64_t seed_offset = 0;
  uint64_t* seed_stage = nullptr;
  int tune_epb = 0, tune_obs_sub = 0, tune_kt_grid = 0, tune_kt_cap = 0, tune_kt_wpc = 0;
  int timing = 0;
  uint64_t step_launches = 0;
  std::vector<hipEvent_t> evpool;
  size_t ev_used = 0;
  double acc_ms = 0.0;
  uint64_t acc_n = 0;
  std::vector<uint32_t> epk;
  std::vector<uint16_t> ewl;
  uint32_t tr_slot = 0;
  int kt_grid = 0, kt_cap = 16;
  int kt_plan_dw = 0, kt_rs_dw = 0;
  size_t kt_lds = 0;
  uint64_t q_launch = 0;
  uint64_t q_grid = 0;
  int q_block = -1;
  int tune_queue_mode = 0;
  FlatArgs flat{};
  const void* flat_fn = nullptr;
  uint64_t flat_wgs = 1536;
  void* flat_dst = nullptr;
  void* final_flat_dst = nullptr;
  float* flat_rew32 = nullptr;
  uint8_t* flat_dones = nullptr;
  uint8_t* flat_tonly = nullptr;
  int flat_dtype = 0;
  EpisodeArgs ep{};
  uint64_t ep_rows = 0;
};


static const void* step_fn(const pgtg_handle* h, int mode) {
  const bool big = h->hcfg.nt > kSmallTiles;
  if (h->hcfg.need_car || h->hcfg.n_rules > 0) return big ? (const void*)k_env<true, true> : (const void*)k_env<true, false>;
  if (mode == MODE_STEP && h->L.queue) {
    if (h->q_block == 1) return big ? (const void*)k_envb<true> : (const void*)k_envb<false>;
    return big ? (const void*)k_envq<true> : (const void*)k_envq<false>;
  }
  return big ? (const void*)k_env<false, true> : (const void*)k_env<false, false>;
}

static int queue_depth(const pgtg_handle* h) { return h->q_block == 1 ? kBlockDepth : kQueueDepth; }

static thread_local std::string g_create_err;

#define HIPCHK(h, x)                                                                 \
  do {                                                                               \
    hipError_t e_ = (x);                                                             \
    if (e_ != hipSuccess) {                                                          \
      (h)->err = std::string(#x) + ": " + hipGetErrorString(e_);                     \
      return PGTG_E_DEVICE;                                                          \
    }                                                                                \
  } while (0)

static int timing_flush(pgtg_handle* h) {
  for (size_t k = 0; k + 1 < h->ev_used; k += 2) {
    float ms = 0.f;
    HIPCHK(h, hipEventSynchronize(h->evpool[k + 1]));
    HIPCHK(h, hipEventElapsedTime(&ms, h->evpool[k], h->evpool[k + 1]));
    h->acc_ms += ms;
    h->acc_n++;
  }
  h->ev_used = 0;
  return 0;
}

template <typename T>
static int dalloc(pgtg_handle* h, T** p, size_t count) {
  void* q = nullptr;
  if (count == 0) count = 1;
  HIPCHK(h, hipMalloc(&q, count * sizeof(T)));
  HIPCHK(h, hipMemset(q, 0, count * sizeof(T)));
  h->allocs.push_back(q);
  *p = reinterpret_cast<T*>(q);
  return 0;
}

static int fail(pgtg_handle* h, int code, const std::string& m) {
  h->err = m;
  return code;
}

static int8_t nsd_dir(int dx, int dy) {
  double angle = atan2(-(double)dy, (double)dx);
  double q = (angle + M_PI) / (M_PI / 4);
  double mq = fmod(q, 8.0);
  if (mq < 0) mq += 8.0;
  static const int remap[8] = {2, 1, 0, 7, 6, 5, 4, 3};
  return (int8_t)remap[(int)mq];
}
static int8_t compass_dir(int dx, int dy, int s) {
  if (abs(dx) <= s && abs(dy) <= s) return -1;
  double angle = atan2((double)dy, (double)dx);
  double P8 = M_PI / 8;
  if (-P8 <= angle && angle < P8) return 2;
  if (P8 <= angle && angle < 3 * P8) return 3;
  if (3 * P8 <= angle && angle < 5 * P8) return 4;
  if (5 * P8 <= angle && angle < 7 * P8) return 5;
  if (angle >= 7 * P8 || angle < -7 * P8) return 6;
  if (-7 * P8 <= angle && angle < -5 * P8) return 7;
  if (-5 * P8 <= angle && angle < -3 * P8) return 0;
  if (-3 * P8 <= angle && angle < -P8) return 1;
  return -1;
}

static uint64_t u53_threshold(double p) {
  if (!(p > 0.0)) return 0;
  if (p >= 1.0) return 1ull << 53;
  return (uint64_t)ceil(ldexp(p, 53));
}

static int derive_cfg(pgtg_handle* h, const PgtgConfig& in, DevCfg& c) {
  memset(&c, 0, sizeof c);
  if (in.abi_version != PGTG_ABI_VERSION) return fail(h, PGTG_E_INVALID, "ABI version mismatch");
  int tw = in.fixed_map ? in.fm_w : in.width, th = in.fixed_map ? in.fm_h : in.height;
  if (tw < 1 || th < 1) return fail(h, PGTG_E_INVALID, "map width and height must be >= 1");
  if (tw * th > PGTG_MAX_TILES) return fail(h, PGTG_E_UNSUPPORTED, "this build supports width*height <= 256 tiles");
  c.tw = tw;
  c.th = th;
  c.nt = tw * th;
  c.W = tw * kTile;
  c.H = th * kTile;
  c.fixed_map = in.fixed_map;
  c.tune_fault = in.tune_fault;
  if (in.fixed_map) {
    for (int t = 0; t < c.nt; t++) {
      uint32_t p = in.fm_exits[t] & 15u;
      if (in.fm_obst_type[t] >= 0) p |= (uint32_t)(in.fm_obst_type[t] + 1) << 4 | (uint32_t)in.fm_obst_mask[t] << 7;
      c.fixed_plan[t] = (uint16_t)p;
    }
    int st = in.fm_start[1] * tw + in.fm_start[0], gl = in.fm_goal[1] * tw + in.fm_goal[0];
    if (in.fm_start[0] < 0 || in.fm_start[0] >= tw || in.fm_start[1] < 0 || in.fm_start[1] >= th || in.fm_goal[0] < 0 ||
        in.fm_goal[0] >= tw || in.fm_goal[1] < 0 || in.fm_goal[1] >= th)
      return fail(h, PGTG_E_INVALID, "fixed map start/goal outside the map");
    c.fixed_sg = (uint32_t)st | (uint32_t)in.fm_start[2] << 8 | (uint32_t)gl << 16 | (uint32_t)in.fm_goal[2] << 24;
  }
  c.start_mode = in.start_mode;
  c.goal_mode = in.goal_mode;
  c.sx = in.start_x;
  c.sy = in.start_y;
  c.sdir = in.start_dir;
  c.gx = in.goal_x;
  c.gy = in.goal_y;
  c.gdir = in.goal_dir;
  c.min_distance = in.min_distance;
  {
    std::vector<int> keys;
    std::vector<std::vector<std::array<int, 2>>> dst(c.nt);
    std::vector<int> seen(c.nt, 0);
    auto add1 = [&](int a, int b, int d) {
      if (!seen[a]) {
        seen[a] = 1;
        keys.push_back(a);
      }
      dst[a].push_back({b, d});
    };
    for (int x = 0; x < tw; x++)
      for (int y = 0; y < th; y++) {
        int t = y * tw + x;
        if (x < tw - 1) {
          add1(t, t + 1, 1);
          add1(t + 1, t, 3);
        }
        if (y < th - 1) {
          add1(t, t + tw, 2);
          add1(t + tw, t, 0);
        }
      }
    std::vector<int> ea, eb, ed;
    for (int a : keys)
      for (const auto& bd : dst[a]) {
        ea.push_back(a);
        eb.push_back(bd[0]);
        ed.push_back(bd[1]);
      }
    const int n = (int)ea.size();
    if (n > kMaxEdges) return fail(h, PGTG_E_UNSUPPORTED, "too many map edges");
    c.n_edges = n;
    memset(c.h0, 0, sizeof c.h0);
    for (int e = 0; e < n; e++) c.h0[ea[e] >> 6][ed[e]] |= 1ull << (ea[e] & 63);
    std::vector<int> pos(c.nt * 4, -1);
    for (int e = 0; e < n; e++) pos[ea[e] * 4 + ed[e]] = e;
    h->epk.assign(n, 0u);
    for (int e = 0; e < n; e++) {
      int a = ea[e], b = eb[e], d = ed[e];
      const int rev = pos[b * 4 + (d + 2) % 4];
// ... 136 lines not shown
    c.car_slots = 3 * cap + kCompactSlack;
    if (in.tune_car_slots > 0) {
      if (in.tune_car_slots < c.car_slots) return fail(h, PGTG_E_INVALID, "tune_car_slots < 3 x car capacity + 4");
      c.car_slots = in.tune_car_slots;
    }
    c.max_spawners = c.nt * 5;
    c.sp_cache_off = c.nt * 16;
    c.traf_bytes = c.sp_cache_off + 2 * kSpCache;
    c.rs_jj_off = ((2 * cap + 3) / 4) * 4;
    c.rs_seen_off = c.rs_jj_off + ((2 * cap + 3) / 4) * 4;
    c.rs_pre_off = c.rs_seen_off + 4 * c.nt;
    c.rs_bytes = (c.rs_pre_off + 2 * (c.W + 1) + 3) / 4 * 4;
    c.rs_bytes = std::max(c.rs_bytes, c.rs_jj_off + 16 * c.nt);
    c.rs_cm_off = 0;
    if (c.th <= 7) {
      c.rs_cm_off = c.rs_bytes;
      c.rs_bytes += 8 * c.W;
    }
  }
  {
    const double ys[5] = {0.95, 0.75, 0.3, 0.98, 0.1}, rv[5] = {0.01, 0.05, 0.15, 0.001, 0.3};
    const int mf[5] = {2, 1, 0, 3, 0};
    const double pl[5] = {0.9, 0.7, 0.3, 0.95, 0.1}, sm[5] = {0.8, 1.0, 1.3, 0.6, 1.5}, rd[5] = {0.1, 0.15, 0.05, 0.3, 0.1};
    for (int k = 0; k < 5; k++) {
      c.beh_t[BEH_YELLOW][k] = u53_threshold(ys[k]);
      c.beh_t[BEH_RED][k] = u53_threshold(rv[k]);
      c.beh_min_follow[k] = mf[k];
      c.beh_patience_thr[k] = (int)floor(pl[k] * 10);
      c.beh_t[BEH_GO][k] = u53_threshold(1.0 - pl[k]);
      c.beh_t[BEH_SPEED][k] = u53_threshold(sm[k]);
      c.beh_t[BEH_DELAY][k] = u53_threshold(rd[k]);
    }
  }
  {
    double tot = 0.0, p[5];
    for (int k = 0; k < 5; k++) tot += in.profile_pct[k];
    for (int k = 0; k < 5; k++) p[k] = tot > 0 ? in.profile_pct[k] / tot : (k == 1 ? 1.0 : 0.0);
    double acc = 0.0, cdf[5];
    for (int k = 0; k < 5; k++) {
      acc += p[k];
      cdf[k] = acc;
    }
    for (int k = 0; k < 5; k++) c.profile_t[k] = u53_threshold(cdf[k] / cdf[4]);
  }
  c.n_rules = in.n_rules;
  if (in.n_rules < 0 || in.n_rules > PGTG_MAX_RULES) return fail(h, PGTG_E_INVALID, "bad rule count");
  for (int k = 0; k < in.n_rules; k++) c.rules[k] = in.rules[k];
  {
    bool possible = c.need_car;
    for (int k = 0; k < in.n_rules; k++) possible = possible || in.rules[k].min_traffic <= 0;
    if (!possible) c.n_rules = 0;
  }
  c.nsd_off = c.W > c.H ? c.W : c.H;
  c.nsd_pitch = 2 * c.nsd_off + 1;
  c.cmp_off = c.nsd_off + 2;
  c.cmp_pitch = 2 * c.cmp_off + 1;
  c.vis_pitch = c.H + 4;
  c.vis_words = ((c.W + 4) * (c.H + 4) + 31) / 32;
  c.plan_dq = (c.nt + 7) / 8;
  c.plan_stride = (!c.need_car && !c.fixed_map && c.nt >= 16) ? ((c.nt + 63) / 64) * 64 : c.plan_dq * 8;
  c.qrec_dw = (c.plan_dq * 4 + 4 + 31) & ~31;
#ifdef PGTG_TUNING
  if (const char* e = getenv("PGTG_QPAD"))
    if (!atoi(e)) c.qrec_dw = c.plan_dq * 4 + 4;
  if (const char* e = getenv("PGTG_PPAD"))
    if (!atoi(e)) c.plan_stride = c.plan_dq * 8;
#endif
  return 0;
}

extern "C" {

static int choose_launch(pgtg_handle* h, bool allow_queue) {
  const DevCfg& c = h->hcfg;
  const uint64_t n_envs = h->n;
  const bool queue_able = allow_queue && !c.need_car && c.n_rules == 0 && !c.fixed_map && !c.generic_channels && c.nt >= 16;
  int envs = c.need_car ? 128
           : n_envs <= (uint64_t)8 * 1024 ? 16
           : n_envs <= (uint64_t)16 * 1024 ? 32
           : n_envs <= (uint64_t)64 * 1024 ? 64
           : (n_envs <= (uint64_t)128 * 1024 || queue_able) ? 128 : kBlock;
  if (h->tune_epb) envs = h->tune_epb;
  if (envs != 16 && envs != 32 && envs != 64 && envs != 128 && envs != 192 && envs != kBlock) envs = kBlock;
  if (envs == 192 && !queue_able) envs = kBlock;
  while (envs > 16 && lds_bytes(lds_layout(c, envs)) + sizeof(Tables) > 150 * 1024) envs /= 2;
  h->L = lds_layout(c, envs);
  if (c.need_car) {
    auto shrink = [&](Lds l) {
      while (l.sub_envs > 8 && lds_bytes(l) + sizeof(Tables) > 80 * 1024) {
        l.sub_envs /= 2;
        l.stream_words = img_words(l.sub_envs, l.seg_bits);
      }
      return l;
    };
    Lds best = shrink(lds_layout(c, envs));
    while (best.envs > 16 && lds_bytes(best) + sizeof(Tables) > 80 * 1024) best = shrink(lds_layout(c, best.envs / 2));
    if (lds_bytes(best) + sizeof(Tables) > 80 * 1024) best = shrink(lds_layout(c, envs));
    if ((h->tune_epb == 0 && n_envs >= (uint64_t)256 * kBlock) || h->tune_epb == kBlock) {
      Lds l = lds_layout(c, kBlock);
      while (l.sub_envs > 8 && lds_bytes(l) + sizeof(Tables) > 160 * 1024) {
        l.sub_envs /= 2;
        l.stream_words = img_words(l.sub_envs, l.seg_bits);
      }
      if (lds_bytes(l) + sizeof(Tables) <= 160 * 1024) best = l;
    }
    h->L = best;
  }
  if (!c.need_car && h->L.envs == kBlock) {
    const uint64_t blocks = (n_envs + kBlock - 1) / kBlock;
    const int want = (int)std::min<uint64_t>(4, (blocks + 255) / 256);
    auto fit = [&](const Lds& l) { return (int)((160 * 1024) / (lds_bytes(l) + sizeof(Tables))); };
    while (fit(h->L) < want && h->L.sub_envs > 64) {
      h->L.sub_envs /= 2;
      h->L.stream_words = img_words(h->L.sub_envs, h->L.seg_bits);
    }
  }
  if (h->tune_obs_sub >= 1 && h->tune_obs_sub < h->L.sub_envs) {
    h->L.sub_envs = h->tune_obs_sub;
    h->L.stream_words = img_words(h->tune_obs_sub, h->L.seg_bits);
  } else {
    lds_img_in_traf(h->L, c);
  }
  if (c.need_car) {
    h->kt_plan_dw = odd_up((c.nt + 1) / 2);
    h->kt_rs_dw = odd_up(c.rs_bytes / 4);
    const size_t per_env = (size_t)4 * (h->kt_plan_dw + h->kt_rs_dw);
    int wpc = h->tune_kt_wpc ? std::max(1, std::min(4, h->tune_kt_wpc)) : 2;
    for (;; wpc--) {
      h->kt_cap = 32;
      while (h->kt_cap > 1 && wpc * (4 * h->kt_cap * per_env + sizeof(Tables) + 256) > 160 * 1024) h->kt_cap--;
      if (wpc == 1 || wpc * (4 * h->kt_cap * per_env + sizeof(Tables) + 256) <= 160 * 1024) break;
    }
    if (h->tune_kt_cap >= 1 && h->tune_kt_cap <= h->kt_cap) h->kt_cap = h->tune_kt_cap;
    h->kt_lds = 4 * h->kt_cap * per_env;
    int ncu = 0;
    if (hipDeviceGetAttribute(&ncu, hipDeviceAttributeMultiprocessorCount, h->device) != hipSuccess || ncu < 1) ncu = 256;
    h->kt_grid = (int)std::min<uint64_t>((uint64_t)ncu * wpc, (h->n + 3) / 4);
    if (h->tune_kt_grid > 0) h->kt_grid = h->tune_kt_grid;
    if (h->kt_lds + sizeof(Tables) > 160 * 1024) return fail(h, PGTG_E_UNSUPPORTED, "LDS budget exceeded (traffic reset scratch)");
    if (h->kt_lds > 64 * 1024)
      (void)hipFuncSetAttribute((const void*)k_traffic, hipFuncAttributeMaxDynamicSharedMemorySize, (int)h->kt_lds);
  }
  h->L.queue = h->L.queue && allow_queue && h->L.sub_envs >= h->L.envs && h->L.envs <= kBlock - 64;
  lds_tail(h->L, c);
  if (h->L.queue && lds_bytes(h->L) + kTabHead > 40 * 1024) {
    h->L.queue = 0;
    lds_tail(h->L, c);
  }
  h->lds = lds_bytes(h->L);
  if (h->lds + sizeof(Tables) > 160 * 1024) return fail(h, PGTG_E_UNSUPPORTED, "LDS budget exceeded");
  if (h->lds > 64 * 1024) {
    const void* fns[] = {(const void*)k_env<true, false>, (const void*)k_env<false, false>, (const void*)k_envq<false>,
                         (const void*)k_env<true, true>, (const void*)k_env<false, true>, (const void*)k_envq<true>,
                         (const void*)k_envb<false>, (const void*)k_envb<true>};
    for (const void* f : fns) (void)hipFuncSetAttribute(f, hipFuncAttributeMaxDynamicSharedMemorySize, (int)h->lds);
  }
  if (!c.need_car && c.n_rules == 0) {
    int ncu = 0, per_cu = 0;
    if (hipDeviceGetAttribute(&ncu, hipDeviceAttributeMultiprocessorCount, h->device) != hipSuccess || ncu < 1) ncu = 256;
    const void* fn = step_fn(h, MODE_STEP);
    if (hipOccupancyMaxActiveBlocksPerMultiprocessor(&per_cu, fn, kBlock, h->lds) != hipSuccess || per_cu < 1) per_cu = 1;
    h->L.stagger_wgs = ncu * per_cu;
    const uint64_t blocks = (h->n + h->L.envs - 1) / h->L.envs;
    h->L.stagger = blocks >= (uint64_t)2 * h->L.stagger_wgs ? 1 : 0;
    h->q_grid = std::max<uint64_t>(1, std::min(std::min(blocks, (uint64_t)h->L.stagger_wgs), (uint64_t)kMaxQueueGrid));
    if (h->q_block < 0 && h->L.queue)
      h->q_block = h->tune_queue_mode ? (h->tune_queue_mode == 2 ? 1 : 0)
                                      : (blocks <= (uint64_t)2 * h->L.stagger_wgs ? 1 : 0);
#ifdef PGTG_TUNING
    if (const char* e = getenv("PGTG_STAGGER")) h->L.stagger = atoi(e);
#endif
  }
  return PGTG_OK;
}

int pgtg_create(const PgtgConfig* cfg, uint64_t n_envs, int32_t device, pgtg_handle** out) {
  if (!cfg || !out) return PGTG_E_INVALID;
  pgtg_handle* h = new pgtg_handle();
  *out = nullptr;
  h->device = device;
  h->n = n_envs;
  h->tune_epb = cfg->tune_envs_per_block;
  h->tune_obs_sub = cfg->tune_obs_sub;
  h->tune_kt_grid = cfg->tune_kt_grid;
  h->tune_kt_cap = cfg->tune_kt_cap;
  h->tune_kt_wpc = cfg->tune_kt_wpc;
  h->tune_queue_mode = cfg->tune_queue_mode;
  int rc = 0;
  if (n_envs == 0) rc = fail(h, PGTG_E_INVALID, "n_envs must be > 0");
  if (!rc) rc = derive_cfg(h, *cfg, h->hcfg);
  if (rc) {
    g_create_err = h->err;
    delete h;
    return rc;
  }
  if (hipSetDevice(device) != hipSuccess) {
    g_create_err = "hipSetDevice failed";
    delete h;
    return PGTG_E_DEVICE;
  }
  const DevCfg& c = h->hcfg;
  DevState& S = h->S;
  S.n = n_envs;
  uint64_t n = n_envs;
#define ALLOC(p, cnt)                 \
  if ((rc = dalloc(h, &(p), (cnt)))) { \
    g_create_err = h->err;            \
    pgtg_destroy(h);                  \
    return rc;                        \
  }
  ALLOC(h->dcfg, 1);
  ALLOC(S.rec, n);
  ALLOC(S.seed, n);
  ALLOC(S.plan, n * (uint64_t)c.plan_stride);
  ALLOC(S.err, n);
  ALLOC(S.counters, 4);
  ALLOC(S.wg_ticks, 1);
  DevStream* streams[4] = {&S.car, &S.ice, &S.broken, &S.sand};
  int needs[4] = {c.need_car, c.need_ice, c.need_broken, c.need_sand};
  for (int k = 0; k < 4; k++)
    if (needs[k]) {
      ALLOC(streams[k]->shi, n);
      ALLOC(streams[k]->slo, n);
      ALLOC(streams[k]->ihi, n);
      ALLOC(streams[k]->ilo, n);
      ALLOC(streams[k]->buf, n);
    }
  if (c.visited_penalty != 0.0) ALLOC(S.visited, n * (uint64_t)c.vis_words);
  if (c.nt > kSmallTiles) {
    uint32_t* e = nullptr;
    ALLOC(e, h->epk.size());
    if (hipMemcpy(e, h->epk.data(), h->epk.size() * sizeof(uint32_t), hipMemcpyHostToDevice) != hipSuccess) {
      g_create_err = "edge table upload failed";
      pgtg_destroy(h);
      return PGTG_E_DEVICE;
    }
    S.epk = e;
  }
  if (c.need_car) {
    ALLOC(S.car_w0, (uint64_t)c.car_slots * n);
    ALLOC(S.car_w1, (uint64_t)c.car_slots * n);
    S.sp_pitch = (uint32_t)((c.max_spawners + 7) & ~7);
    S.fresh_occ = (uint32_t)((c.car_cap + 3) & ~3);
    S.fresh_dw = S.fresh_occ + (uint32_t)c.nt * 4u;
    ALLOC(S.car_id, (uint64_t)c.car_slots * n);
    ALLOC(S.traf, n);
    ALLOC(S.occ, (uint64_t)c.nt * 4 * n);
    ALLOC(S.fresh, (uint64_t)S.fresh_dw * n);
    ALLOC(S.spawners, (uint64_t)S.sp_pitch * n);
    ALLOC(S.tr_list, n);
    ALLOC(S.tr_count, 2);
  }
  {
    std::vector<int8_t> nsd((size_t)c.nsd_pitch * c.nsd_pitch), cmp((size_t)c.cmp_pitch * c.cmp_pitch);
    for (int a = 0; a < c.nsd_pitch; a++)
      for (int b = 0; b < c.nsd_pitch; b++) nsd[(size_t)a * c.nsd_pitch + b] = nsd_dir(a - c.nsd_off, b - c.nsd_off);
    for (int a = 0; a < c.cmp_pitch; a++)
      for (int b = 0; b < c.cmp_pitch; b++)
        cmp[(size_t)a * c.cmp_pitch + b] = compass_dir(a - c.cmp_off, b - c.cmp_off, cfg->sliding_size);
    int8_t *dn = nullptr, *dc = nullptr;
    ALLOC(dn, nsd.size());
    ALLOC(dc, cmp.size());
    if (hipMemcpy(dn, nsd.data(), nsd.size(), hipMemcpyHostToDevice) != hipSuccess ||
        hipMemcpy(dc, cmp.data(), cmp.size(), hipMemcpyHostToDevice) != hipSuccess) {
      g_create_err = "table upload failed";
      pgtg_destroy(h);
      return PGTG_E_DEVICE;
    }
    S.nsd_tab = dn;
    S.cmp_tab = dc;
  }
#undef ALLOC
  {
    Tables t;
    memset(&t, 0, sizeof t);
    memcpy(t.wall, hs::kTileWall, sizeof t.wall);
    memcpy(t.seg, hs::kExitSeg, sizeof t.seg);
    memcpy(t.obst, hs::kObstMask, sizeof t.obst);
    memcpy(t.spawner, hs::kLaneSpawner, sizeof t.spawner);
    memcpy(t.lanes, hs::kLanes, sizeof t.lanes);
    memcpy(t.ind, c.ind_reward, sizeof t.ind);
    if (c.n_edges <= kSmallEdges) memcpy(t.epk, h->epk.data(), h->epk.size() * sizeof(uint32_t));
    if (c.n_edges <= kSmallEdges) memcpy(t.ewl, h->ewl.data(), h->ewl.size() * sizeof(uint16_t));
    memcpy(t.bt, c.bt, sizeof t.bt);
    memcpy(t.bd, c.bd, sizeof t.bd);
    for (int k = 0; k < PGTG_MAX_CHANNELS; k++) t.chan[k] = (uint8_t)c.channels[k];
    memset(t.li, 255, sizeof t.li);
    memset(t.slot_sq, 255, sizeof t.slot_sq);
    for (int ex = 0; ex < 16; ex++) {
      int n = 0;
      for (int lx = 0; lx < 9; lx++)
        for (int ly = 0; ly < 9; ly++) {
          int sq = lx * 9 + ly;
          uint32_t ln = hs::kLanes[ex][sq];
          if (ln) {
            t.li[ex][sq] = (uint8_t)n;
            t.slot_sq[ex][n] = (uint8_t)sq;
            n++;
            t.lanecol[ex][lx] |= (uint16_t)(1u << ly);
          }
          if ((hs::kLaneSpawner[ex][sq >> 5] >> (sq & 31)) & 1u) t.spcol[ex][lx] |= (uint16_t)(1u << ly);
          for (int ty = 0; ty < 4; ty++)
            if ((ln >> (28 + ty)) & 1u) t.allcol[ex][ty][lx] |= (uint16_t)(1u << ly);
        }
    }
    memcpy(t.lane_route, hs::kLaneRoute, sizeof t.lane_route);
    memcpy(t.route_type_lane, hs::kRouteTypeLane, sizeof t.route_type_lane);
    for (int r = 0; r < cfg->n_rules && r < PGTG_MAX_RULES; r++) memcpy(t.rule_w[r], cfg->rules[r].weight, sizeof t.rule_w[r]);
    memcpy(t.beh_t, h->hcfg.beh_t, sizeof t.beh_t);
    memcpy(t.beh_mf, h->hcfg.beh_min_follow, sizeof t.beh_mf);
    memcpy(t.beh_pt, h->hcfg.beh_patience_thr, sizeof t.beh_pt);
    if ((rc = dalloc(h, &h->dtab, 1)) || hipMemcpy(h->dtab, &t, sizeof t, hipMemcpyHostToDevice) != hipSuccess) {
      g_create_err = "table upload failed";
      pgtg_destroy(h);
      return PGTG_E_DEVICE;
    }
  }
  if (hipMemcpy(h->dcfg, &h->hcfg, sizeof(DevCfg), hipMemcpyHostToDevice) != hipSuccess) {
    g_create_err = "config upload failed";
    pgtg_destroy(h);
    return PGTG_E_DEVICE;
  }
  if ((rc = choose_launch(h, true))) {
    g_create_err = h->err;
    pgtg_destroy(h);
    return rc;
  }
  if (h->L.queue) {
    if ((rc = dalloc(h, &h->S.qbuf, n * (uint64_t)queue_depth(h) * (uint64_t)c.qrec_dw)) || (rc = dalloc(h, &h->S.qstate, n)) ||
        (!h->q_block &&
         ((rc = dalloc(h, &h->S.qreq, 2 * h->q_grid * queue_req_cap((n + h->L.envs - 1) / h->L.envs, h->q_grid, h->L.envs))) ||
          (rc = dalloc(h, &h->S.qovf, 2 * 8 * ((h->q_grid + 7) / 8) * (uint64_t)h->L.envs)) ||
          (rc = dalloc(h, &h->S.qctr, kQctrWords))))) {
      g_create_err = h->err;
      pgtg_destroy(h);
      return rc;
    }
  }
  *out = h;
  return PGTG_OK;
}

int pgtg_destroy(pgtg_handle* h) {
  if (!h) return PGTG_OK;
  for (void* p : h->allocs) (void)hipFree(p);
  for (auto e : h->evpool) (void)hipEventDestroy(e);
  delete h;
  return PGTG_OK;
}

int pgtg_set_stream(pgtg_handle* h, void* stream) {
  if (!h) return PGTG_E_INVALID;
  h->stream = reinterpret_cast<hipStream_t>(stream);
  return PGTG_OK;
}

int pgtg_set_outputs(pgtg_handle* h, const PgtgOutputs* o) {
  if (!h || !o) return PGTG_E_INVALID;
  if (h->ep.out_ret && (!o->reward || !o->terminated || !o->truncated))
    return fail(h, PGTG_E_INVALID, "episode statistics are bound: the reward, terminated and truncated outputs must stay");
  h->out = *o;
  return PGTG_OK;
}

static int launch_episode(pgtg_handle* h) {
  EpisodeArgs a = h->ep;
  a.rew = h->out.reward;
  a.term = h->out.terminated;
  a.trunc = h->out.truncated;
  hipLaunchKernelGGL(k_episode, dim3((unsigned)h->ep_rows), dim3(kEpisodeBlock), 0, h->stream, a);
  HIPCHK(h, hipGetLastError());
  return PGTG_OK;
}

static int episode_zero(pgtg_handle* h, const uint8_t* mask) {
  if (!h->ep.ret) return PGTG_OK;
  hipLaunchKernelGGL(k_episode_zero, dim3((unsigned)h->ep_rows), dim3(kEpisodeBlock), 0, h->stream, h->ep.ret, h->ep.len,
                     mask, h->n);
  HIPCHK(h, hipGetLastError());
  return PGTG_OK;
}

static int launch_flatten(pgtg_handle* h, int mode, uint64_t grid) {
  FlatArgs a = h->flat;
  const PgtgOutputs& o = h->out;
  const bool final = mode == 1;
  a.obs = final ? o.final_obs : o.obs;
  a.pos = final ? o.final_position : o.position;
  a.vel = final ? o.final_velocity : o.velocity;
  a.nsd = final ? o.final_next_subgoal : o.next_subgoal;
  a.term = o.terminated;
  a.trunc = o.truncated;
  a.dst = final ? h->final_flat_dst : h->flat_dst;
  a.fobs = o.final_obs;
  a.fpos = o.final_position;
  a.fvel = o.final_velocity;
  a.fnsd = o.final_next_subgoal;
  a.fdst = h->final_flat_dst;
  a.final = mode;
  a.rew = o.reward;
  a.rew32 = final ? nullptr : h->flat_rew32;
  a.dones = final ? nullptr : h->flat_dones;
  a.tonly = final ? nullptr : h->flat_tonly;
  const bool one = a.D <= kFlatU * 64 && a.OB <= 2048;
  const bool pair = one && !h->flat_dtype && a.D % 2 == 0;
  const void* fn = h->flat_dtype ? (one ? (const void*)k_flatten<int8_t, true, 1> : (const void*)k_flatten<int8_t, false, 1>)
                                 : (pair ? (const void*)k_flatten<float, true, 2>
                                         : (one ? (const void*)k_flatten<float, true, 1> : (const void*)k_flatten<float, false, 1>));
  if (h->flat_fn != fn) {
    int ncu = 0, per_cu = 0;
    if (hipDeviceGetAttribute(&ncu, hipDeviceAttributeMultiprocessorCount, h->device) != hipSuccess || ncu < 1) ncu = 256;
    if (hipOccupancyMaxActiveBlocksPerMultiprocessor(&per_cu, fn, 256, 0) != hipSuccess || per_cu < 1) per_cu = 1;
    h->flat_fn = fn;
    h->flat_wgs = (uint64_t)ncu * (uint64_t)per_cu;
  }
  const uint64_t G = grid ? grid : std::max<uint64_t>(std::min<uint64_t>(h->n, h->flat_wgs), (h->n + 255) / 256);
  if (h->flat_dtype) {
    if (one) hipLaunchKernelGGL((k_flatten<int8_t, true, 1>), dim3((unsigned)G), dim3(256), 0, h->stream, a);
    else hipLaunchKernelGGL((k_flatten<int8_t, false, 1>), dim3((unsigned)G), dim3(256), 0, h->stream, a);
  } else if (pair) {
    hipLaunchKernelGGL((k_flatten<float, true, 2>), dim3((unsigned)G), dim3(256), 0, h->stream, a);
  } else {
    if (one) hipLaunchKernelGGL((k_flatten<float, true, 1>), dim3((unsigned)G), dim3(256), 0, h->stream, a);
    else hipLaunchKernelGGL((k_flatten<float, false, 1>), dim3((unsigned)G), dim3(256), 0, h->stream, a);
  }
  HIPCHK(h, hipGetLastError());
  return PGTG_OK;
}

static int launch(pgtg_handle* h, const uint8_t* actions, const uint8_t* mask, int mode) {
  HIPCHK(h, hipSetDevice(h->device));
  uint64_t blocks = (h->n + h->L.envs - 1) / h->L.envs;
  const bool timed = h->timing > 0 && mode == MODE_STEP && (h->step_launches++ % (uint64_t)h->timing) == 0;
  if (timed) {
    if (h->evpool.empty()) {
      h->evpool.resize(2048);
      for (auto& e : h->evpool) HIPCHK(h, hipEventCreate(&e));
    }
    if (h->ev_used + 2 > h->evpool.size()) {
      int rc = timing_flush(h);
      if (rc) return rc;
    }
    HIPCHK(h, hipEventRecord(h->evpool[h->ev_used], h->stream));
  }
  const void* fn = step_fn(h, mode);
  void* args[] = {&h->dcfg, &h->dtab, &h->S, &actions, &mask, &h->out, &mode, &h->L, &h->tr_slot};
  if (fn == (const void*)k_envb<false> || fn == (const void*)k_envb<true>) {
    void* bargs[] = {&h->dcfg, &h->dtab, &h->S, &actions, &h->out, &h->L};
    HIPCHK(h, hipLaunchKernel(fn, dim3((unsigned)blocks), dim3(kBlock), bargs, h->lds, h->stream));
  } else if (fn == (const void*)k_envq<false> || fn == (const void*)k_envq<true>) {
    uint32_t qsel = (uint32_t)(h->q_launch % 3) | (uint32_t)(h->q_launch & 1) << 2;
    h->q_launch++;
    void* qargs[] = {&h->dcfg, &h->dtab, &h->S, &actions, &h->out, &h->L, &qsel};
    HIPCHK(h, hipLaunchKernel(fn, dim3((unsigned)std::min(blocks, h->q_grid)), dim3(kBlock), qargs, h->lds, h->stream));
  } else {
    HIPCHK(h, hipLaunchKernel(fn, dim3((unsigned)blocks), dim3(kBlock), args, h->lds, h->stream));
  }
  HIPCHK(h, hipGetLastError());
  if (h->hcfg.need_car && mode != MODE_OBSERVE) {
    hipLaunchKernelGGL(k_traffic, dim3((unsigned)h->kt_grid), dim3(kBlock), h->kt_lds, h->stream, h->dcfg, h->dtab,
                       h->S, h->out, h->tr_slot, h->kt_plan_dw, h->kt_rs_dw, h->kt_cap);
    HIPCHK(h, hipGetLastError());
    h->tr_slot ^= 1u;
  }
  {
    const bool fl = h->flat_dst != nullptr, ff = h->final_flat_dst != nullptr && mode == MODE_STEP;
    if (fl || ff)
      if (int rc = launch_flatten(h, fl && ff ? 2 : (ff ? 1 : 0), 0)) return rc;
  }
  if (timed) {
    HIPCHK(h, hipEventRecord(h->evpool[h->ev_used + 1], h->stream));
    h->ev_used += 2;
  }
  if (h->ep.out_ret && mode == MODE_STEP)
    if (int rc = launch_episode(h)) return rc;
  return PGTG_OK;
}

static int queue_fill(pgtg_handle* h) {
  if (!h->L.queue || !h->S.qbuf) return PGTG_OK;
  if (h->S.qctr) HIPCHK(h, hipMemsetAsync(h->S.qctr, 0, kQctrWords * sizeof(uint32_t), h->stream));
#ifdef PGTG_TUNING
  if (const char* e = getenv("PGTG_QFILL"))
    if (!atoi(e)) return PGTG_OK;
#endif
  const int pdw = h->L.plan_stride_dw;
  const size_t lds = (size_t)4 * kBlock * pdw;
  const bool big = h->hcfg.nt > kSmallTiles;
  const void* fn = h->q_block == 1 ? (big ? (const void*)k_qfill_b<true> : (const void*)k_qfill_b<false>)
                                   : (big ? (const void*)k_qfill<true> : (const void*)k_qfill<false>);
  if (lds > 64 * 1024) HIPCHK(h, hipFuncSetAttribute(fn, hipFuncAttributeMaxDynamicSharedMemorySize, (int)lds));
  const uint64_t blocks = (h->n + kBlock - 1) / kBlock;
  void* args[] = {&h->dcfg, &h->dtab, &h->S, (void*)&pdw};
  HIPCHK(h, hipLaunchKernel(fn, dim3((unsigned)blocks), dim3(kBlock), args, lds, h->stream));
  HIPCHK(h, hipGetLastError());
  return PGTG_OK;
}

int pgtg_reset(pgtg_handle* h, const uint64_t* seeds_host, uint64_t seed_base, const uint8_t* mask_dev) {
  if (!h) return PGTG_E_INVALID;
  HIPCHK(h, hipSetDevice(h->device));
  if (seeds_host && !mask_dev) {
    HIPCHK(h, hipMemcpyAsync(h->S.seed, seeds_host, h->n * sizeof(uint64_t), hipMemcpyHostToDevice, h->stream));
  } else {
    const uint64_t* src = nullptr;
    if (seeds_host) {
      if (!h->seed_stage)
        if (int rc = dalloc(h, &h->seed_stage, h->n)) return rc;
      HIPCHK(h, hipMemcpyAsync(h->seed_stage, seeds_host, h->n * sizeof(uint64_t), hipMemcpyHostToDevice, h->stream));
      src = h->seed_stage;
    }
    hipLaunchKernelGGL(k_fill_seeds, dim3((unsigned)((h->n + 255) / 256)), dim3(256), 0, h->stream, h->S.seed, h->n,
                       seed_base, src, mask_dev);
    HIPCHK(h, hipGetLastError());
  }
  if (int rc = launch(h, nullptr, mask_dev, MODE_RESET_SEEDED)) return rc;
  if (int rc = episode_zero(h, mask_dev)) return rc;
  return queue_fill(h);
}

int pgtg_reset_unseeded(pgtg_handle* h, const uint8_t* mask_dev) {
  if (!h) return PGTG_E_INVALID;
  if (int rc = launch(h, nullptr, mask_dev, MODE_RESET_UNSEEDED)) return rc;
  if (int rc = episode_zero(h, mask_dev)) return rc;
  return queue_fill(h);
}

int pgtg_step(pgtg_handle* h, const uint8_t* actions_dev) {
  if (!h || !actions_dev) return PGTG_E_INVALID;
  return launch(h, actions_dev, nullptr, MODE_STEP);
}

int pgtg_step_many(pgtg_handle* h, const uint8_t* actions_dev, uint64_t row_stride, uint64_t ticks) {
  if (!h || !actions_dev || row_stride < h->n) return PGTG_E_INVALID;
  for (uint64_t k = 0; k < ticks; k++)
    if (int rc = launch(h, actions_dev + k * row_stride, nullptr, MODE_STEP)) return rc;
  return PGTG_OK;
}

int pgtg_observe(pgtg_handle* h) {
  if (!h) return PGTG_E_INVALID;
  return launch(h, nullptr, nullptr, MODE_OBSERVE);
}

int pgtg_random_actions(pgtg_handle* h, uint8_t* actions_dev, uint64_t seed, uint64_t t, uint64_t env_offset) {
  if (!h || !actions_dev) return PGTG_E_INVALID;
  HIPCHK(h, hipSetDevice(h->device));
  hipLaunchKernelGGL(k_random_actions, dim3((unsigned)((h->n + 255) / 256)), dim3(256), 0, h->stream, actions_dev, h->n,
                     seed, t, env_offset);
  HIPCHK(h, hipGetLastError());
  return PGTG_OK;
}

static int read_traf(pgtg_handle* h, uint64_t env, uint4* t) {
  HIPCHK(h, hipMemcpy(t, h->S.traf + env, sizeof *t, hipMemcpyDeviceToHost));
  return 0;
}

int pgtg_get_env_state(pgtg_handle* h, uint64_t env, PgtgEnvState* st) {
  if (!h || !st || env >= h->n) return PGTG_E_INVALID;
  HIPCHK(h, hipSetDevice(h->device));
  HIPCHK(h, hipStreamSynchronize(h->stream));
  EnvRec r;
  uint64_t seed;
  uint8_t e;
  HIPCHK(h, hipMemcpy(&r, h->S.rec + env, sizeof r, hipMemcpyDeviceToHost));
  HIPCHK(h, hipMemcpy(&seed, h->S.seed + env, sizeof seed, hipMemcpyDeviceToHost));
  HIPCHK(h, hipMemcpy(&e, h->S.err + env, 1, hipMemcpyDeviceToHost));
  memset(st, 0, sizeof *st);
  st->x = (int16_t)(r.a.x & 0xffffu);
  st->y = (int16_t)(r.a.x >> 16);
  st->vx = (int16_t)(r.a.y & 0xffffu);
  st->vy = (int16_t)(r.a.y >> 16);
  st->phase = (int)(r.a.z & 0xffffu);
  uint32_t fl = (r.a.z >> 16) & 0xfu;
  st->terminated = (fl & kFlagTerminated) ? 1 : 0;
  st->flat_tire = (fl & kFlagFlatTire) ? 1 : 0;
  st->path_len = (int)(r.a.z >> 20);
  st->elapsed = (int)r.a.w;
  st->spawn_counter = r.b.y;
  st->used_subgoals[0] = (uint64_t)r.b.z | ((uint64_t)r.b.w << 32);
  if (h->hcfg.nt > kSmallTiles) {
    std::vector<uint16_t> p(h->hcfg.plan_stride);
    HIPCHK(h, hipMemcpy(p.data(), h->S.plan + env * (uint64_t)h->hcfg.plan_stride, p.size() * 2, hipMemcpyDeviceToHost));
    st->used_subgoals[0] = 0;
    for (int t = 0; t < h->hcfg.nt; t++) st->used_subgoals[t >> 6] |= (uint64_t)((p[t] & kPlanUsed) != 0) << (t & 63);
  }
  st->seed = seed;
  st->error = -(int)e;
  if (h->hcfg.need_car) {
    uint4 t;
    if (int rc = read_traf(h, env, &t)) return rc;
    st->n_cars = (int)(t.x & 0xffffu);
    st->n_spawners = (int)(t.x >> 16);
    st->next_car_id = (int)t.y;
    st->car_tail = (int)t.z;
  }
  return PGTG_OK;
}


static int host_read_cars(pgtg_handle* h, uint64_t env, const uint4& t, std::vector<PgtgCar>& cars) {
  cars.clear();
  const int tail = (int)t.z;
  if (tail == 0) return 0;
  const uint64_t N = h->n;
  std::vector<uint32_t> w0(tail), w1(tail, 0u), id(tail);
  if (t.w & kTrafFresh) {
    HIPCHK(h, hipMemcpy(w0.data(), h->S.fresh + env * (uint64_t)h->S.fresh_dw, 4 * (size_t)tail, hipMemcpyDeviceToHost));
    for (int k = 0; k < tail; k++) id[k] = (uint32_t)k;
  } else {
    HIPCHK(h, hipMemcpy2D(w0.data(), 4, h->S.car_w0 + env, N * 4, 4, tail, hipMemcpyDeviceToHost));
    HIPCHK(h, hipMemcpy2D(w1.data(), 4, h->S.car_w1 + env, N * 4, 4, tail, hipMemcpyDeviceToHost));
    HIPCHK(h, hipMemcpy2D(id.data(), 4, h->S.car_id + env, N * 4, 4, tail, hipMemcpyDeviceToHost));
  }
  for (int k = 0; k < tail; k++) {
    if (w0[k] & kCarEmpty) continue;
    cars.push_back(PgtgCar{(int32_t)id[k], (int32_t)(w0[k] & 255u), (int32_t)((w0[k] >> 8) & 255u),
                           (int32_t)((w0[k] >> 16) & 31u), (int32_t)((w0[k] >> 21) & 7u), (int32_t)w1[k],
                           (int32_t)((w0[k] >> 24) & 3u)});
  }
  if ((int)cars.size() != (int)(t.x & 0xffffu)) return fail(h, PGTG_E_DEVICE, "car slots disagree with the car count");
  return 0;
}

static int host_write_cars(pgtg_handle* h, uint64_t env, uint4 t, const std::vector<PgtgCar>& cars, uint32_t next_id) {
  const int n = (int)cars.size();
  if (n > h->hcfg.car_cap) return fail(h, PGTG_E_UNSUPPORTED, "more cars than the handle's car capacity");
  const uint64_t N = h->n;
  std::vector<uint32_t> w0(n), w1(n), id(n);
  for (int k = 0; k < n; k++) {
    const PgtgCar& q = cars[k];
    w0[k] = (uint32_t)q.x | (uint32_t)q.y << 8 | (uint32_t)q.route << 16 | (uint32_t)q.profile << 21 |
            (uint32_t)q.delay << 24;
    w1[k] = (uint32_t)q.patience;
    id[k] = (uint32_t)q.id;
  }
  if (n > 0) {
    HIPCHK(h, hipMemcpy2D(h->S.car_w0 + env, N * 4, w0.data(), 4, 4, n, hipMemcpyHostToDevice));
    HIPCHK(h, hipMemcpy2D(h->S.car_w1 + env, N * 4, w1.data(), 4, 4, n, hipMemcpyHostToDevice));
    HIPCHK(h, hipMemcpy2D(h->S.car_id + env, N * 4, id.data(), 4, 4, n, hipMemcpyHostToDevice));
  }
  t.x = (t.x & 0xffff0000u) | (uint32_t)n;
  t.y = next_id;
  t.z = (uint32_t)n;
  t.w = 0u;
  HIPCHK(h, hipMemcpy(h->S.traf + env, &t, sizeof t, hipMemcpyHostToDevice));
  return 0;
}

int pgtg_get_cars(pgtg_handle* h, uint64_t env, PgtgCar* cars, int32_t cap, int32_t* n) {
  if (!h || env >= h->n || !n) return PGTG_E_INVALID;
  *n = 0;
  if (!h->hcfg.need_car) return PGTG_OK;
  HIPCHK(h, hipSetDevice(h->device));
  HIPCHK(h, hipStreamSynchronize(h->stream));
  uint4 t;
  if (int rc = read_traf(h, env, &t)) return rc;
  *n = (int)(t.x & 0xffffu);
  if (cars && cap > 0 && *n > 0) {
    std::vector<PgtgCar> v;
    if (int rc = host_read_cars(h, env, t, v)) return rc;
    for (int k = 0; k < (int)v.size() && k < cap; k++) cars[k] = v[k];
  }
  return PGTG_OK;
}

int pgtg_get_map_plan(pgtg_handle* h, uint64_t env, int32_t* w, int32_t* h_, uint8_t* exits, int8_t* otype,
                      int8_t* omask, int32_t* start3, int32_t* goal3) {
  if (!h || env >= h->n) return PGTG_E_INVALID;
  HIPCHK(h, hipSetDevice(h->device));
  HIPCHK(h, hipStreamSynchronize(h->stream));
  const DevCfg& c = h->hcfg;
  std::vector<uint16_t> p(c.plan_stride);
  EnvRec r;
  HIPCHK(h, hipMemcpy(p.data(), h->S.plan + env * (uint64_t)c.plan_stride, c.plan_stride * 2, hipMemcpyDeviceToHost));
  HIPCHK(h, hipMemcpy(&r, h->S.rec + env, sizeof r, hipMemcpyDeviceToHost));
  *w = c.tw;
  *h_ = c.th;
  for (int t = 0; t < c.nt; t++) {
    exits[t] = (uint8_t)plan_exits(p[t]);
    int ot = (int)plan_otype(p[t]);
    otype[t] = (int8_t)(ot - 1);
    omask[t] = (int8_t)(ot ? (int)plan_omask(p[t]) : -1);
  }
  uint32_t sg = r.b.x;
  start3[0] = (int)(sg & 0xffu) % c.tw;
  start3[1] = (int)(sg & 0xffu) / c.tw;
  start3[2] = (int)((sg >> 8) & 0xffu);
  goal3[0] = (int)((sg >> 16) & 0xffu) % c.tw;
  goal3[1] = (int)((sg >> 16) & 0xffu) / c.tw;
  goal3[2] = (int)(sg >> 24);
  return PGTG_OK;
}

int pgtg_get_squares(pgtg_handle* h, uint64_t env, uint64_t* words, int32_t cap, int32_t* width, int32_t* height) {
  if (!h || env >= h->n) return PGTG_E_INVALID;
  const DevCfg& c = h->hcfg;
  if (width) *width = c.W;
  if (height) *height = c.H;
  if (!words) return PGTG_OK;
  if (cap < c.W * c.H) return fail(h, PGTG_E_INVALID, "squares buffer too small");
  HIPCHK(h, hipSetDevice(h->device));
  uint64_t* d = nullptr;
  HIPCHK(h, hipMalloc(&d, (size_t)c.W * c.H * 8));
  hipLaunchKernelGGL(k_squares, dim3(1), dim3(kBlock), 0, h->stream, h->dcfg, h->dtab, h->S, env, d);
  hipError_t e = hipGetLastError();
  if (e == hipSuccess) e = hipStreamSynchronize(h->stream);
  if (e == hipSuccess) e = hipMemcpy(words, d, (size_t)c.W * c.H * 8, hipMemcpyDeviceToHost);
  (void)hipFree(d);
  if (e != hipSuccess) return fail(h, PGTG_E_DEVICE, std::string("pgtg_get_squares: ") + hipGetErrorString(e));
  return PGTG_OK;
}

int pgtg_set_rules(pgtg_handle* h, const PgtgRule* rules, int32_t n_rules) {
  if (!h || n_rules < 0 || n_rules > PGTG_MAX_RULES || (n_rules > 0 && !rules))
    return h ? fail(h, PGTG_E_INVALID, "bad rule count") : PGTG_E_INVALID;
  HIPCHK(h, hipSetDevice(h->device));
  HIPCHK(h, hipStreamSynchronize(h->stream));
  DevCfg& c = h->hcfg;
  const DevCfg old_cfg = c;
  const Lds old_L = h->L;
  const size_t old_lds = h->lds;
  bool possible = c.need_car;
  for (int k = 0; k < n_rules; k++) {
    c.rules[k] = rules[k];
    possible = possible || rules[k].min_traffic <= 0;
  }
  c.n_rules = possible ? n_rules : 0;
  if ((old_cfg.n_rules > 0) != (c.n_rules > 0)) {
    if (int rc = choose_launch(h, h->S.qbuf != nullptr)) {
      c = old_cfg;
      h->L = old_L;
      h->lds = old_lds;
      return rc;
    }
  }
  const bool refill = h->L.queue && !old_L.queue;
  uint8_t w[PGTG_MAX_RULES][6][20] = {};
  for (int k = 0; k < n_rules; k++) memcpy(w[k], rules[k].weight, sizeof w[k]);
  HIPCHK(h, hipMemcpy(h->dcfg, &c, sizeof(DevCfg), hipMemcpyHostToDevice));
  HIPCHK(h, hipMemcpy(reinterpret_cast<uint8_t*>(h->dtab) + kTabHead + offsetof(TablesTail, rule_w), w, sizeof w, hipMemcpyHostToDevice));
  if (refill) return queue_fill(h);
  return PGTG_OK;
}

int pgtg_set_agent(pgtg_handle* h, uint64_t env, int32_t x, int32_t y, int32_t vx, int32_t vy) {
  if (!h || env >= h->n) return PGTG_E_INVALID;
  HIPCHK(h, hipSetDevice(h->device));
  HIPCHK(h, hipStreamSynchronize(h->stream));
  EnvRec r;
  HIPCHK(h, hipMemcpy(&r, h->S.rec + env, sizeof r, hipMemcpyDeviceToHost));
  r.a.x = ((uint32_t)x & 0xffffu) | ((uint32_t)y << 16);
  r.a.y = ((uint32_t)vx & 0xffffu) | ((uint32_t)vy << 16);
  HIPCHK(h, hipMemcpy(h->S.rec + env, &r, sizeof r, hipMemcpyHostToDevice));
  return PGTG_OK;
}

int pgtg_add_car(pgtg_handle* h, uint64_t env, int32_t x, int32_t y, int32_t route, int32_t profile, int32_t car_id) {
  if (!h || env >= h->n) return PGTG_E_INVALID;
  if (!h->hcfg.need_car) return fail(h, PGTG_E_UNSUPPORTED, "create the handle with min_car_capacity > 0 or traffic");
  if (x < 0 || y < 0 || x >= h->hcfg.W || y >= h->hcfg.H || route < 0 || route >= 20 || profile < 0 || profile >= 5)
    return fail(h, PGTG_E_INVALID, "car outside the map or bad route/profile");
  HIPCHK(h, hipSetDevice(h->device));
  HIPCHK(h, hipStreamSynchronize(h->stream));
  uint4 t;
  if (int rc = read_traf(h, env, &t)) return rc;
  std::vector<PgtgCar> v;
  if (int rc = host_read_cars(h, env, t, v)) return rc;
  if ((int)v.size() >= h->hcfg.car_cap) return fail(h, PGTG_E_UNSUPPORTED, "car capacity exhausted");
  const uint32_t id = car_id < 0 ? t.y : (uint32_t)car_id;
  v.push_back(PgtgCar{(int32_t)id, x, y, route, profile, 0, 0});
  return host_write_cars(h, env, t, v, car_id < 0 ? t.y + 1u : t.y);
}

namespace {
struct StateSection {
  uint32_t id;
  void* ptr;
  uint32_t kind;
  uint64_t row;
  uint64_t bytes;
};
struct PgtgStateHeader {
  char magic[4];
  uint32_t version;
  uint64_t n;
  uint32_t n_sections, nt, car_cap, plan_stride;
  uint32_t max_spawners, vis_words, qrec_dw, car_slots;
  uint64_t cfg_hash;
};
struct PgtgSectionEntry {
  uint32_t id, pad;
  uint64_t bytes;
};
constexpr uint32_t kStateVersion = 5;
uint64_t cfg_hash(const DevCfg& c) {
  const uint8_t* p = reinterpret_cast<const uint8_t*>(&c);
  uint64_t h = 0xcbf29ce484222325ull;
  for (size_t k = 0; k < sizeof c; k++) h = (h ^ p[k]) * 0x100000001b3ull;
  return h;
}
}

static std::vector<StateSection> state_sections(pgtg_handle* h) {
  const DevCfg& c = h->hcfg;
  const DevState& S = h->S;
  const uint64_t n = h->n;
  std::vector<StateSection> v;
  auto rows = [&](uint32_t id, void* p, uint64_t row_bytes) {
    if (p) v.push_back({id, p, kSecRows, row_bytes, n * row_bytes});
  };
  auto slots = [&](uint32_t id, void* p, uint64_t nrows) {
    if (p) v.push_back({id, p, kSecSlots, nrows, nrows * n * 4});
  };
  rows(1, S.rec, sizeof(EnvRec));
  rows(2, S.seed, 8);
  rows(3, S.plan, (uint64_t)c.plan_stride * 2);
  rows(4, S.err, 1);
  if (S.counters) v.push_back({5, S.counters, kSecBatch, 16, 16});
  const DevStream* st[4] = {&S.car, &S.ice, &S.broken, &S.sand};
  for (uint32_t k = 0; k < 4; k++) {
    rows(10 + 5 * k, st[k]->shi, 8);
    rows(11 + 5 * k, st[k]->slo, 8);
    rows(12 + 5 * k, st[k]->ihi, 8);
    rows(13 + 5 * k, st[k]->ilo, 8);
    rows(14 + 5 * k, st[k]->buf, 8);
  }
  rows(30, S.visited, (uint64_t)c.vis_words * 4);
  slots(31, S.car_w0, (uint64_t)c.car_slots);
  slots(32, S.car_w1, (uint64_t)c.car_slots);
  slots(33, S.car_id, (uint64_t)c.car_slots);
  rows(34, S.traf, sizeof(uint4));
  slots(36, S.occ, (uint64_t)c.nt * 4);
  rows(35, S.spawners, (uint64_t)S.sp_pitch * 2);
  rows(37, S.fresh, (uint64_t)S.fresh_dw * 4);
  rows(40, S.qbuf, (uint64_t)queue_depth(h) * (uint64_t)c.qrec_dw * 4);
  rows(41, S.qstate, 1);
  return v;
}

static uint64_t state_blob_bytes(const std::vector<StateSection>& v) {
  uint64_t b = sizeof(PgtgStateHeader) + v.size() * sizeof(PgtgSectionEntry);
  for (const auto& s : v) b = ((b + 15) & ~15ull) + s.bytes;
  return b;
}

int pgtg_state_size(pgtg_handle* h, uint64_t* bytes) {
  if (!h || !bytes) return PGTG_E_INVALID;
  *bytes = state_blob_bytes(state_sections(h));
  return PGTG_OK;
}

int pgtg_dump_state(pgtg_handle* h, void* buf, uint64_t bytes) {
  if (!h || !buf) return PGTG_E_INVALID;
  const auto v = state_sections(h);
  if (bytes < state_blob_bytes(v)) return fail(h, PGTG_E_INVALID, "pgtg_dump_state: buffer smaller than pgtg_state_size");
  HIPCHK(h, hipSetDevice(h->device));
  if (int rc = queue_fill(h)) return rc;
  HIPCHK(h, hipStreamSynchronize(h->stream));
  uint8_t* p = static_cast<uint8_t*>(buf);
  PgtgStateHeader hd{};
  memcpy(hd.magic, "PGTS", 4);
  hd.version = kStateVersion;
  hd.n = h->n;
  hd.n_sections = (uint32_t)v.size();
  hd.nt = (uint32_t)h->hcfg.nt;
  hd.car_cap = (uint32_t)h->hcfg.car_cap;
  hd.plan_stride = (uint32_t)h->hcfg.plan_stride;
  hd.max_spawners = (uint32_t)h->hcfg.max_spawners;
  hd.vis_words = (uint32_t)h->hcfg.vis_words;
  hd.qrec_dw = (uint32_t)h->hcfg.qrec_dw;
  hd.car_slots = (uint32_t)h->hcfg.car_slots;
  hd.cfg_hash = cfg_hash(h->hcfg);
  memcpy(p, &hd, sizeof hd);
  uint64_t off = sizeof hd;
  for (const auto& s : v) {
    PgtgSectionEntry e{s.id, 0, s.bytes};
    memcpy(p + off, &e, sizeof e);
    off += sizeof e;
  }
  for (const auto& s : v) {
    off = (off + 15) & ~15ull;
    HIPCHK(h, hipMemcpy(p + off, s.ptr, s.bytes, hipMemcpyDeviceToHost));
    off += s.bytes;
  }
  return PGTG_OK;
}

int pgtg_load_state(pgtg_handle* h, const void* buf, uint64_t bytes) {
  if (!h || !buf) return PGTG_E_INVALID;
  const auto v = state_sections(h);
  const uint8_t* p = static_cast<const uint8_t*>(buf);
  PgtgStateHeader hd;
  if (bytes < sizeof hd) return fail(h, PGTG_E_INVALID, "pgtg_load_state: truncated state");
  memcpy(&hd, p, sizeof hd);
  if (memcmp(hd.magic, "PGTS", 4) != 0 || hd.version != kStateVersion)
    return fail(h, PGTG_E_INVALID, "pgtg_load_state: not a state blob of this version");
  if (hd.n != h->n || hd.n_sections != v.size() || hd.nt != (uint32_t)h->hcfg.nt ||
      hd.car_cap != (uint32_t)h->hcfg.car_cap || hd.plan_stride != (uint32_t)h->hcfg.plan_stride ||
      hd.max_spawners != (uint32_t)h->hcfg.max_spawners || hd.vis_words != (uint32_t)h->hcfg.vis_words ||
      hd.qrec_dw != (uint32_t)h->hcfg.qrec_dw || hd.car_slots != (uint32_t)h->hcfg.car_slots ||
      bytes < state_blob_bytes(v))
    return fail(h, PGTG_E_INVALID, "pgtg_load_state: the state was dumped from a handle of another shape");
  if (hd.cfg_hash != cfg_hash(h->hcfg))
    return fail(h, PGTG_E_INVALID, "pgtg_load_state: the state was dumped from a handle of another configuration");
  uint64_t off = sizeof hd;
  for (const auto& s : v) {
    PgtgSectionEntry e;
    memcpy(&e, p + off, sizeof e);
    off += sizeof e;
    if (e.id != s.id || e.bytes != s.bytes) return fail(h, PGTG_E_INVALID, "pgtg_load_state: section table mismatch");
  }
  HIPCHK(h, hipSetDevice(h->device));
  HIPCHK(h, hipStreamSynchronize(h->stream));
  for (const auto& s : v) {
    off = (off + 15) & ~15ull;
    HIPCHK(h, hipMemcpy(s.ptr, p + off, s.bytes, hipMemcpyHostToDevice));
    off += s.bytes;
  }
  if (h->S.tr_count) HIPCHK(h, hipMemset(h->S.tr_count, 0, 2 * sizeof(uint32_t)));
  if (h->S.qctr) HIPCHK(h, hipMemset(h->S.qctr, 0, kQctrWords * sizeof(uint32_t)));
  if (h->ep.ret) {
    HIPCHK(h, hipMemsetAsync(h->ep.ret, 0, h->n * sizeof(float), h->stream));
    HIPCHK(h, hipMemsetAsync(h->ep.len, 0, h->n * sizeof(int32_t), h->stream));
  }
  return PGTG_OK;
}

struct pgtg_snapshot {
  int device = 0;
  uint64_t slots = 0;
  std::vector<StateSection> sec;
  PgtgStateHeader shape{};
  int depth = 0;
  uint64_t device_bytes = 0, bytes_per_env = 0;
};

static void snapshot_shape(pgtg_handle* h, PgtgStateHeader* hd, int* depth) {
  hd->nt = (uint32_t)h->hcfg.nt;
  hd->car_cap = (uint32_t)h->hcfg.car_cap;
  hd->plan_stride = (uint32_t)h->hcfg.plan_stride;
  hd->max_spawners = (uint32_t)h->hcfg.max_spawners;
  hd->vis_words = (uint32_t)h->hcfg.vis_words;
  hd->qrec_dw = (uint32_t)h->hcfg.qrec_dw;
  hd->car_slots = (uint32_t)h->hcfg.car_slots;
  hd->cfg_hash = cfg_hash(h->hcfg);
  *depth = h->S.qbuf ? queue_depth(h) : 0;
}

static uint64_t section_bytes(const StateSection& s, uint64_t n) {
  return s.kind == kSecRows ? n * s.row : s.row * n * 4;
}

int pgtg_snapshot_create(pgtg_handle* h, uint64_t slots, pgtg_snapshot** out) {
  if (!h || !out) return PGTG_E_INVALID;
  if (slots == 0 || slots > 0xffffffffull) return fail(h, PGTG_E_INVALID, "pgtg_snapshot_create: slots outside [1, 2^32)");
  HIPCHK(h, hipSetDevice(h->device));
  pgtg_snapshot* s = new pgtg_snapshot;
  s->device = h->device;
  s->slots = slots;
  snapshot_shape(h, &s->shape, &s->depth);
  for (const auto& hs : state_sections(h)) {
    if (hs.kind == kSecBatch) continue;
    StateSection e = hs;
    e.ptr = nullptr;
    e.bytes = section_bytes(hs, slots);
    hipError_t rc = hipMalloc(&e.ptr, e.bytes);
    if (rc == hipSuccess) rc = hipMemsetAsync(e.ptr, 0, e.bytes, h->stream);
    if (rc != hipSuccess) {
      if (e.ptr) (void)hipFree(e.ptr);
      pgtg_snapshot_destroy(s);
      return fail(h, PGTG_E_DEVICE, std::string("pgtg_snapshot_create: ") + hipGetErrorString(rc));
    }
    s->sec.push_back(e);
    s->device_bytes += e.bytes;
    s->bytes_per_env += section_bytes(hs, 1);
  }
  if (s->sec.size() > (size_t)kMaxCopySections) {
    pgtg_snapshot_destroy(s);
    return fail(h, PGTG_E_UNSUPPORTED, "pgtg_snapshot_create: more state sections than the copy table holds");
  }
  *out = s;
  return PGTG_OK;
}

int pgtg_snapshot_destroy(pgtg_snapshot* s) {
  if (!s) return PGTG_OK;
  (void)hipSetDevice(s->device);
  for (auto& e : s->sec) (void)hipFree(e.ptr);
  delete s;
  return PGTG_OK;
}

int pgtg_snapshot_bytes(const pgtg_snapshot* s, uint64_t* device_bytes, uint64_t* bytes_per_env) {
  if (!s) return PGTG_E_INVALID;
  if (device_bytes) *device_bytes = s->device_bytes;
  if (bytes_per_env) *bytes_per_env = s->bytes_per_env;
  return PGTG_OK;
}

static int snapshot_table(pgtg_handle* h, const pgtg_snapshot* s, bool to_snapshot, const char* who, CopyTable* T) {
  PgtgStateHeader hd{};
  int depth = 0;
  snapshot_shape(h, &hd, &depth);
  const PgtgStateHeader& q = s->shape;
  if (h->device != s->device) return fail(h, PGTG_E_INVALID, std::string(who) + ": the snapshot lives on another device");
  if (hd.nt != q.nt || hd.car_cap != q.car_cap || hd.plan_stride != q.plan_stride || hd.max_spawners != q.max_spawners ||
      hd.vis_words != q.vis_words || hd.qrec_dw != q.qrec_dw || hd.car_slots != q.car_slots)
    return fail(h, PGTG_E_INVALID, std::string(who) + ": the snapshot was created from a handle of another shape");
  if (hd.cfg_hash != q.cfg_hash)
    return fail(h, PGTG_E_INVALID, std::string(who) + ": the snapshot was created from a handle of another configuration");
  if (depth != s->depth)
    return fail(h, PGTG_E_INVALID, std::string(who) + ": the snapshot was created from a handle with another map-queue step "
                                                      "kernel (its rings hold another number of maps)");
  memset(T, 0, sizeof *T);
  uint32_t k = 0;
  for (const auto& hs : state_sections(h)) {
    if (hs.kind == kSecBatch) continue;
    if (k >= s->sec.size() || s->sec[k].id != hs.id || s->sec[k].kind != hs.kind || s->sec[k].row != hs.row)
      return fail(h, PGTG_E_INVALID, std::string(who) + ": section list mismatch");
    CopySection& e = T->sec[k];
    e.src = to_snapshot ? hs.ptr : s->sec[k].ptr;
    e.dst = to_snapshot ? s->sec[k].ptr : hs.ptr;
    e.src_n = to_snapshot ? h->n : s->slots;
    e.dst_n = to_snapshot ? s->slots : h->n;
    e.kind = hs.kind;
    e.row = (uint32_t)hs.row;
    e.unit = 4;
    if (hs.kind == kSecRows) {
      const uint64_t bits = (uint64_t)(uintptr_t)e.src | (uint64_t)(uintptr_t)e.dst | hs.row;
      e.unit = 16;
      while (bits & (e.unit - 1)) e.unit >>= 1;
    }
    k++;
  }
  if (k != s->sec.size()) return fail(h, PGTG_E_INVALID, std::string(who) + ": section list mismatch");
  T->n_sections = k;
  return PGTG_OK;
}

static int snapshot_copy(pgtg_handle* h, const pgtg_snapshot* s, bool to_snapshot, const char* who, const uint32_t* src_idx,
                         const uint32_t* dst_idx, uint64_t count) {
  if (!h || !s) return PGTG_E_INVALID;
  CopyTable T;
  if (int rc = snapshot_table(h, s, to_snapshot, who, &T)) return rc;
  if (count > 0xffffffffull) return fail(h, PGTG_E_INVALID, std::string(who) + ": more than 2^32 - 1 pairs");
  if (count == 0) return PGTG_OK;
  HIPCHK(h, hipSetDevice(h->device));
  if (int rc = queue_fill(h)) return rc;
  T.src_idx = src_idx;
  T.dst_idx = dst_idx;
  T.count = count;
  if (!to_snapshot && h->ep.ret) {
    T.ep_ret = h->ep.ret;
    T.ep_len = h->ep.len;
  }
  hipLaunchKernelGGL(k_state_copy, dim3((unsigned)((count + kCopyBlock - 1) / kCopyBlock)), dim3(kCopyBlock), 0, h->stream, T);
  HIPCHK(h, hipGetLastError());
  return PGTG_OK;
}

int pgtg_snapshot_save(pgtg_handle* h, pgtg_snapshot* s, const uint32_t* env_idx_dev, const uint32_t* slot_idx_dev,
                       uint64_t count) {
  return snapshot_copy(h, s, true, "pgtg_snapshot_save", env_idx_dev, slot_idx_dev, count);
}

int pgtg_snapshot_load(pgtg_handle* h, const pgtg_snapshot* s, const uint32_t* slot_idx_dev, const uint32_t* env_idx_dev,
                       uint64_t count) {
  return snapshot_copy(h, s, false, "pgtg_snapshot_load", slot_idx_dev, env_idx_dev, count);
}

int pgtg_set_to_state(pgtg_handle* h, uint64_t env, int32_t x, int32_t y, int32_t vx, int32_t vy, int32_t flat_tire,
                      const PgtgCar* cars, int32_t n_cars) {
  if (!h || env >= h->n || (n_cars > 0 && !cars)) return PGTG_E_INVALID;
  if (abs(vx) > 30000 || abs(vy) > 30000 || abs(x) > 30000 || abs(y) > 30000)
    return fail(h, PGTG_E_UNSUPPORTED, "position/velocity outside the 16-bit state range");
  const DevCfg& c = h->hcfg;
  if (n_cars > 0 && !c.need_car) return fail(h, PGTG_E_UNSUPPORTED, "create the handle with min_car_capacity > 0 or traffic");
  if (n_cars > c.car_cap) return fail(h, PGTG_E_UNSUPPORTED, "more cars than the handle's car capacity");
  for (int k = 0; k < n_cars; k++) {
    const PgtgCar& q = cars[k];
    if (q.x < 0 || q.y < 0 || q.x >= c.W || q.y >= c.H || q.route < 0 || q.route >= 20 || q.profile < 0 || q.profile >= 5)
      return fail(h, PGTG_E_INVALID, "car outside the map or bad route/profile");
  }
  HIPCHK(h, hipSetDevice(h->device));
  HIPCHK(h, hipStreamSynchronize(h->stream));
  EnvRec r;
  HIPCHK(h, hipMemcpy(&r, h->S.rec + env, sizeof r, hipMemcpyDeviceToHost));
  r.a.x = ((uint32_t)x & 0xffffu) | ((uint32_t)y << 16);
  r.a.y = ((uint32_t)vx & 0xffffu) | ((uint32_t)vy << 16);
  uint32_t flags = (r.a.z >> 16) & 0xfu;
  flags = flat_tire ? (flags | kFlagFlatTire) : (flags & ~kFlagFlatTire);
  r.a.z = (r.a.z & 0xfff0ffffu) | (flags << 16);
  HIPCHK(h, hipMemcpy(h->S.rec + env, &r, sizeof r, hipMemcpyHostToDevice));
  if (c.need_car) {
    uint4 t;
    if (int rc = read_traf(h, env, &t)) return rc;
    std::vector<PgtgCar> v;
    for (int k = 0; k < n_cars; k++) v.push_back(PgtgCar{cars[k].id, cars[k].x, cars[k].y, cars[k].route, cars[k].profile, 0, 0});
    if (int rc = host_write_cars(h, env, t, v, n_cars > 0 ? (uint32_t)cars[n_cars - 1].id + 1u : t.y)) return rc;
  }
  return PGTG_OK;
}

int pgtg_car_digest(pgtg_handle* h, uint64_t* out_dev) {
  if (!h || !out_dev) return PGTG_E_INVALID;
  if (!h->hcfg.need_car) return fail(h, PGTG_E_UNSUPPORTED, "pgtg_car_digest: the handle has no traffic");
  HIPCHK(h, hipSetDevice(h->device));
  hipLaunchKernelGGL(k_car_digest, dim3((unsigned)((h->n + 255) / 256)), dim3(256), 0, h->stream, h->S, out_dev);
  HIPCHK(h, hipGetLastError());
  return PGTG_OK;
}

int pgtg_get_counters(pgtg_handle* h, uint64_t* env_steps, uint64_t* episodes) {
  if (!h) return PGTG_E_INVALID;
  HIPCHK(h, hipSetDevice(h->device));
  HIPCHK(h, hipStreamSynchronize(h->stream));
  unsigned long long c[2];
  HIPCHK(h, hipMemcpy(c, h->S.counters, sizeof c, hipMemcpyDeviceToHost));
  if (env_steps) *env_steps = c[0];
  if (episodes) *episodes = c[1];
  return PGTG_OK;
}

int pgtg_get_queue_maps(pgtg_handle* h, uint64_t* maps) {
  if (!h || !maps) return PGTG_E_INVALID;
  HIPCHK(h, hipSetDevice(h->device));
  HIPCHK(h, hipStreamSynchronize(h->stream));
  unsigned long long c[3];
  HIPCHK(h, hipMemcpy(c, h->S.counters, sizeof c, hipMemcpyDeviceToHost));
  *maps = c[2];
  return PGTG_OK;
}

int pgtg_set_flat_outputs(pgtg_handle* h, const int32_t* order, int32_t n_order, int32_t dtype, void* flat_dev,
                          void* final_flat_dev) {
  if (!h) return PGTG_E_INVALID;
  h->flat_dst = h->final_flat_dst = nullptr;
  if (!flat_dev && !final_flat_dev) return PGTG_OK;
  const DevCfg& c = h->hcfg;
  const PgtgOutputs& o = h->out;
  if (dtype != 0 && dtype != 1) return fail(h, PGTG_E_INVALID, "flat dtype: 0 float32, 1 int8");
  if (!order || n_order != c.n_channels) return fail(h, PGTG_E_INVALID, "flat order: one entry per channel");
  uint64_t seen[2] = {0, 0};
  for (int k = 0; k < n_order; k++) {
    if (order[k] < 0 || order[k] >= n_order || ((seen[order[k] >> 6] >> (order[k] & 63)) & 1u))
      return fail(h, PGTG_E_INVALID, "flat order: not a permutation of the channels");
    seen[order[k] >> 6] |= 1ull << (order[k] & 63);
  }
  if (c.sliding && c.ss >= 9)
    return fail(h, PGTG_E_UNSUPPORTED, "position (s, s) of a sliding window of size >= 9 is outside MultiDiscrete([9, 9])");
  if (flat_dev && (!o.obs || !o.position || !o.velocity || (c.next_subgoal && !o.next_subgoal)))
    return fail(h, PGTG_E_INVALID, "flat rows need the obs, position, velocity (and next_subgoal) outputs");
  if (final_flat_dev && (!o.final_obs || !o.final_position || !o.final_velocity || !o.terminated || !o.truncated ||
                         (c.next_subgoal && !o.final_next_subgoal)))
    return fail(h, PGTG_E_INVALID, "terminal flat rows need the final_* and terminated/truncated outputs");
  if (((uintptr_t)flat_dev | (uintptr_t)final_flat_dev) & 15u) return fail(h, PGTG_E_INVALID, "flat rows: 16-byte aligned buffers");
  FlatArgs& a = h->flat;
  a.n = h->n;
  a.w2 = c.win * c.win;
  a.OB = c.obs_bytes;
  a.cw2 = c.n_channels * a.w2;
  a.nsd_on = c.next_subgoal ? 1 : 0;
  a.D = a.cw2 + (a.nsd_on ? 9 : 0) + 20;
  for (int k = 0; k < n_order; k++) a.order[k] = (uint8_t)order[k];
  h->flat_dtype = dtype;
  h->flat_dst = flat_dev;
// ... 341 lines not shown
```

Before: 2.684 billion env-steps/s.

## Read plans in place from a three-slot map ring instead of copying

With the persistent map-queue kernel, the per-env plan array is removed and each env's current plan lives directly in one of three ring slots in qbuf. The active slot is tracked in qstate. On reset, the kernel stops copying the queued map into the plan array and just flips the current-slot index, which saves a full plan write and read per reset. It also prefetches the next block's qstate early to hide that load's latency. In exchange, qbuf grows by a third, queue bookkeeping gets more complex, env counts are capped at 2^30, and snapshots made with the old layout become incompatible.

```diff
diff --git a/pgtg_amd/csrc/pgtg_env.hip b/pgtg_amd/csrc/pgtg_env.hip
--- a/pgtg_amd/csrc/pgtg_env.hip
+++ b/pgtg_amd/csrc/pgtg_env.hip
@@ -152,7 +152,30 @@
   const int t0 = 2 * word;
   return t0 + 1 < c.nt ? ~0u : (t0 < c.nt ? 0xffffu : 0u);
 }
+constexpr int kQueueDepth = 3;
+__host__ __device__ inline uint32_t queue_slot(uint32_t bits) { return (bits & 3u) < 2u ? (bits & 3u) : 2u; }
+__host__ __device__ inline uint32_t queue_cur(uint32_t qs) { return queue_slot(qs); }
+__host__ __device__ inline uint32_t queue_head(uint32_t qs) { return queue_slot(qs >> 2); }
+__host__ __device__ inline uint32_t queue_spare(uint32_t qc, uint32_t qh) { return qc != qh ? 3u - qc - qh : (qc + 2u) % 3u; }
+template <bool SLOT>
+__device__ __forceinline__ uint16_t* plan_row(const DevCfg& c, const DevState& S, uint64_t i) {
+  if (!SLOT) return S.plan + i * (uint64_t)c.plan_stride;
+  return reinterpret_cast<uint16_t*>(S.qbuf + (i * kQueueDepth + queue_cur(S.qstate[i])) * (uint64_t)c.qrec_dw);
+}
+__device__ __forceinline__ void store_plan_quads(const DevCfg& c, uint4* dstp, int nq, const uint32_t* pw, int pdw) {
+  for (int k = 0; k < nq; k++) {
+    uint32_t wv[4];
+#pragma unroll
+    for (int j = 0; j < 4; j++) wv[j] = (k * 4 + j < pdw) ? pw[k * 4 + j] & plan_word_mask(c, k * 4 + j) : 0u;
+    dstp[k] = make_uint4(wv[0], wv[1], wv[2], wv[3]);
+  }
+}
+template <bool SLOT>
 __device__ __forceinline__ void store_plan_row(const DevCfg& c, const DevState& S, uint64_t i, const uint32_t* pw, int pdw) {
+  if (SLOT) {
+    store_plan_quads(c, reinterpret_cast<uint4*>(plan_row<true>(c, S, i)), c.qrec_dw / 4, pw, pdw);
+    return;
+  }
   uint4* dstp = reinterpret_cast<uint4*>(S.plan + i * (uint64_t)c.plan_stride);
   for (int k = 0; k < c.plan_stride / 8; k++) {
     uint32_t wv[4];
@@ -2440,7 +2463,6 @@
   return c < (uint64_t)kQueueLanes ? (uint64_t)kQueueLanes : c;
 }
 constexpr uint64_t kStaggerMaxTicks = 20000;
-constexpr int kQueueDepth = 2;
 constexpr int kBlockDepth = 3;
 constexpr uint32_t kQueueStale = 0x80u;
 constexpr int kViewDw = 8;
@@ -2557,7 +2579,7 @@
   if (L.stagger && blockIdx.x == 0 && threadIdx.x == 0) S.wg_ticks[0] = wall_clock64() - t0;
 }
 
-template <bool TR, bool BIG>
+template <bool TR, bool BIG, bool SLOT = false>
 __global__ void __launch_bounds__(kBlock, TR ? 3 : 4) k_env(const DevCfg* __restrict__ cfg, const Tables* __restrict__ gtab,
                                                  DevState S, const uint8_t* __restrict__ actions,
                                                  const uint8_t* __restrict__ mask, PgtgOutputs out, int mode, Lds L,
@@ -2613,7 +2635,7 @@
       ts.fresh = (tr4.w & kTrafFresh) ? 1u : 0u;
       occ_valid = (tr4.w & kTrafOccValid) != 0u;
     }
-    stage_plan<BIG>(S.plan + i * (uint64_t)c.plan_stride, c.plan_dq, plan_w, L.plan_stride_dw);
+    stage_plan<BIG>(plan_row<SLOT>(c, S, i), c.plan_dq, plan_w, L.plan_stride_dw);
   }
   for (int k = tid; k < L.lm_words; k += kBlock) lm[k] = 0u;
   lds_barrier();
@@ -2687,7 +2709,7 @@
       }
       occ_valid = (TR && c.need_car) && !occ_sat && err == 0;
       const bool done = (v.flags & (kFlagTerminated | kFlagTruncated)) != 0;
-      if (BIG && res.plan_dirty && !(done && c.autoreset && err == 0)) store_plan_row(c, S, i, plan_w, L.plan_stride_dw);
+      if (BIG && res.plan_dirty && !(done && c.autoreset && err == 0)) store_plan_row<SLOT>(c, S, i, plan_w, L.plan_stride_dw);
       if (out.reward) out.reward[i] = res.reward;
       if (out.cost) out.cost[i] = res.cost;
       if (out.terminated) out.terminated[i] = (v.flags & kFlagTerminated) ? 1 : 0;
@@ -2776,7 +2798,7 @@
       vv.spawn = xw[0];
       TrafState tw{0, 0, 0, 0};
       const int e2 = env_reset<TR, BIG>(c, S, iw, vv, reinterpret_cast<uint16_t*>(pw), tw);
-      store_plan_row(c, S, iw, pw, L.plan_stride_dw);
+      store_plan_row<SLOT>(c, S, iw, pw, L.plan_stride_dw);
       xw[0] = ((uint32_t)vv.px & 0xffffu) | ((uint32_t)vv.py << 16);
       xw[1] = vv.sg;
       xw[2] = vv.path_len | (uint32_t)(-e2) << 16;
@@ -2803,7 +2825,7 @@
     int e2 = env_reset<TR, BIG>(c, S, i, v, pl.p, ts);
     if (e2) err = e2;
     tr_push = (TR && c.need_car) && e2 == 0;
-    store_plan_row(c, S, i, plan_w, L.plan_stride_dw);
+    store_plan_row<SLOT>(c, S, i, plan_w, L.plan_stride_dw);
   }
   STAMP(4);
   if (live) {
@@ -2814,7 +2836,7 @@
                                (occ_valid && !reset_now ? kTrafOccValid : 0u) | (ts.fresh ? kTrafFresh : 0u));
     }
     if (mode != MODE_OBSERVE || err) S.err[i] = (uint8_t)(-err);
-    if (S.qstate && reset_now) S.qstate[i] = (uint8_t)kQueueStale;
+    if (S.qstate && reset_now) S.qstate[i] = (uint8_t)(SLOT ? (queue_cur(S.qstate[i]) | kQueueStale) : kQueueStale);
   }
   if (TR && c.need_car) {
     const uint64_t m = __ballot(tr_push);
@@ -2973,7 +2995,7 @@
 
 template <bool BIG>
 __device__ __forceinline__ uint3 ring_take(const DevCfg& c, const DevState& S, const Lds& L, uint64_t i, uint32_t qh,
-                                           uint32_t k0, uint32_t* plan_w, int pdw, int depth = kQueueDepth) {
+                                           uint32_t k0, uint32_t* plan_w, int pdw, int depth) {
   const uint4* q4 = reinterpret_cast<const uint4*>(S.qbuf + (i * (uint64_t)depth + qh) * (uint64_t)c.qrec_dw);
   uint4* dstp = reinterpret_cast<uint4*>(S.plan + i * (uint64_t)c.plan_stride);
   const int nq = c.plan_dq;
@@ -3032,6 +3054,8 @@
     r0 = req_old[lane];
   }
   if (blockIdx.x == 0 && tid < 8) S.qctr[kQctrOvfLen + ((set_new + 1u) % 3u) * 8u + tid] = 0u;
+  uint32_t qs_nx = 0;
+  if (tid < L.envs && (uint64_t)blockIdx.x * L.envs + tid < S.n) qs_nx = S.qstate[(uint64_t)blockIdx.x * L.envs + tid];
   const int pdw = L.plan_stride_dw;
   stage_tables(gtab, false);
   uint32_t* st = lds + L.envs * (pdw + L.scratch_dw + L.traf_dw + L.hist_dw);
@@ -3048,6 +3072,7 @@
     *qn = 0u;
   }
   lds_barrier();
+  asm volatile("" : "+v"(qs_nx));
 
   if (wave == gen_wave) {
     STAMP(1);
@@ -3079,8 +3104,8 @@
         ovs += oth;
         if ((uint32_t)lane < own + oth) {
           const uint2 r = (uint32_t)lane >= own ? ovf[ob + (lane - own)] : base == 0 ? r0 : req_old[base + lane];
-          const uint64_t ie = r.x >> 1;
-          gen_queue_entry<BIG>(c, S, ie, r.y, gplan, pdw, S.qbuf + (ie * kQueueDepth + (r.x & 1u)) * (uint64_t)c.qrec_dw,
+          const uint64_t ie = r.x >> 2;
+          gen_queue_entry<BIG>(c, S, ie, r.y, gplan, pdw, S.qbuf + (ie * kQueueDepth + queue_slot(r.x)) * (uint64_t)c.qrec_dw,
                                ABLATE(L, 16), false);
         }
         if (base + kQueueLanes >= cnt) break;
@@ -3091,8 +3116,8 @@
         ovs += m;
         if ((uint32_t)lane < m) {
           const uint2 r = ovf[st0 + lane];
-          const uint64_t ie = r.x >> 1;
-          gen_queue_entry<BIG>(c, S, ie, r.y, gplan, pdw, S.qbuf + (ie * kQueueDepth + (r.x & 1u)) * (uint64_t)c.qrec_dw,
+          const uint64_t ie = r.x >> 2;
+          gen_queue_entry<BIG>(c, S, ie, r.y, gplan, pdw, S.qbuf + (ie * kQueueDepth + queue_slot(r.x)) * (uint64_t)c.qrec_dw,
                                ABLATE(L, 16), false);
         }
       }
@@ -3123,13 +3148,13 @@
     const uint64_t i = env0 + slot;
     const bool live = env_wave && slot < nb;
     EnvView v{};
-    uint32_t qh = 0;
+    const uint32_t qs = qs_nx;
+    const auto ring_slot = [&](uint32_t s) { return S.qbuf + (i * kQueueDepth + s) * (uint64_t)c.qrec_dw; };
     int act = 0;
     if (live) {
       v = rec_load(S.rec, i);
-      qh = S.qstate[i] & 1u;
       act = actions[i];
-      stage_plan<BIG>(S.plan + i * (uint64_t)c.plan_stride, c.plan_dq, plan_w, pdw);
+      stage_plan<BIG>(reinterpret_cast<const uint16_t*>(ring_slot(queue_cur(qs))), c.plan_dq, plan_w, pdw);
     }
     for (int k = rank; k < L.lm_words; k += nthr) lm[k] = 0u;
     sub_barrier(ctr, bar += (uint32_t)np);
@@ -3149,7 +3174,8 @@
       if (out.truncated) out.truncated[i] = (v.flags & kFlagTruncated) ? 1 : 0;
       if (out.braking) out.braking[i] = 0;
       my_sel = (done && c.autoreset && err == 0) ? 1 : 0;
-      if (BIG && res.plan_dirty && !my_sel) store_plan_row(c, S, i, plan_w, pdw);
+      if (BIG && res.plan_dirty && !my_sel)
+        store_plan_quads(c, reinterpret_cast<uint4*>(ring_slot(queue_cur(qs))), c.plan_dq, plan_w, pdw);
       if (lm && my_sel && out.final_obs) mark_lines(lm, out.final_obs + env0 * (uint64_t)c.obs_bytes, (uint32_t)slot, (uint32_t)c.obs_bytes);
       STAMP(23);
     }
@@ -3161,38 +3187,29 @@
     if (env_wave) sel[slot] = my_sel;
     const uint64_t rm = __ballot(my_sel == 1);
     if (env_wave && lane == 0 && rm) atomicAdd(&S.counters[1], (unsigned long long)__popcll(rm));
+    if (tid == 0) *nxt = got;
     STAMP(2);
     STAMP(28);
     sub_barrier(ctr, bar += (uint32_t)np);
     STAMP(29);
+    {
+      const uint32_t g = *nxt;
+      const uint64_t ni = ((uint64_t)gridDim.x + g) * (uint64_t)L.envs + (uint64_t)slot;
+      qs_nx = 0;
+      if (g != 0xffffffffu && slot < L.envs && ni < S.n) qs_nx = S.qstate[ni];
+    }
     if (out.final_obs && !ABLATE(L, 2))
       write_obs(out.final_obs + env0 * (uint64_t)c.obs_bytes, (uint32_t)nb, (uint32_t)c.obs_bytes, st, sel, rank, nthr, lm);
     STAMP(3);
     sub_barrier(ctr, bar += (uint32_t)np);
     const bool reset_now = my_sel != 0;
     const uint32_t k0 = v.spawn;
+    const uint32_t qc = queue_cur(qs), qh = queue_head(qs);
     if (reset_now) {
-      const uint4* q4 = reinterpret_cast<const uint4*>(S.qbuf + (i * kQueueDepth + qh) * (uint64_t)c.qrec_dw);
-      uint4* dstp = reinterpret_cast<uint4*>(S.plan + i * (uint64_t)c.plan_stride);
+      const uint4* q4 = reinterpret_cast<const uint4*>(ring_slot(qh));
       const int nq = c.plan_dq;
       const uint4 meta = q4[nq];
-      for (int k0q = 0; k0q < (BIG ? nq : 1); k0q += 8) {
-        uint4 qw[8];
-#pragma unroll
-        for (int k = 0; k < 8; k++) qw[k] = q4[k0q + k < nq ? k0q + k : k0q];
-#pragma unroll
-        for (int k = 0; k < 8; k++) {
-          if (k0q + k < nq) {
-            if (!ABLATE(L, 32)) dstp[k0q + k] = qw[k];
-            const uint32_t wv[4] = {qw[k].x, qw[k].y, qw[k].z, qw[k].w};
-#pragma unroll
-            for (int j = 0; j < 4; j++)
-              if ((k0q + k) * 4 + j < pdw) plan_w[(k0q + k) * 4 + j] = wv[j];
-          }
-        }
-      }
-      if (!ABLATE(L, 32))
-        for (int k = nq; k < c.plan_stride / 8; k++) dstp[k] = make_uint4(0u, 0u, 0u, 0u);
+      stage_plan<BIG>(reinterpret_cast<const uint16_t*>(q4), nq, plan_w, pdw);
       if (c.need_ice || c.need_broken || c.need_sand) {
         SeedPool sp = ss_pool(S.seed[i]);
         if (c.need_ice) stream_store_all(S.ice, i, ss_child(sp, k0 + 2u));
@@ -3218,6 +3235,7 @@
         vis[b >> 5] |= 1u << (b & 31);
       }
     }
+    asm volatile("" : "+v"(qs_nx));
     STAMP(4);
     const uint64_t rb = __ballot(reset_now);
     if (rb) {
@@ -3233,12 +3251,12 @@
       }
       if (reset_now) {
         const uint32_t p = base + (uint32_t)__popcll(rb & ((1ull << lane) - 1ull));
-        const uint2 r = make_uint2((uint32_t)i << 1 | qh, k0 + 10u);
+        const uint2 r = make_uint2((uint32_t)i << 2 | qc, k0 + 10u);
         if (one_round && p >= (uint32_t)kQueueLanes)
           S.qovf[((uint64_t)par * 8u + ox) * ocap + obase + (p - max(base, (uint32_t)kQueueLanes))] = r;
         else
           req_new[p] = r;
-        S.qstate[i] = (uint8_t)(qh ^ 1u);
+        S.qstate[i] = (uint8_t)(qh | queue_spare(qc, qh) << 2);
       }
     }
     if (live) {
@@ -3251,7 +3269,6 @@
       group_obs<BIG>(c, S, v, reset_now, st, oi, L, wave, lane, ctr, bar, np, rank, vw, false);
       if (reset_now) write_small_outputs(c, out, i, v, oi, false);
     }
-    if (tid == 0) *nxt = got;
     STAMP(30);
     sub_barrier(ctr, bar += (uint32_t)np);
     STAMP(31);
@@ -3398,7 +3415,7 @@
     if (out.truncated) out.truncated[i] = (v.flags & kFlagTruncated) ? 1 : 0;
     if (out.braking) out.braking[i] = 0;
     my_sel = (done && c.autoreset && err == 0) ? 1 : 0;
-    if (BIG && res.plan_dirty && !my_sel) store_plan_row(c, S, i, plan_w, pdw);
+    if (BIG && res.plan_dirty && !my_sel) store_plan_row<false>(c, S, i, plan_w, pdw);
     if (lm && my_sel && out.final_obs) mark_lines(lm, out.final_obs + env0 * (uint64_t)c.obs_bytes, (uint32_t)slot, (uint32_t)c.obs_bytes);
     STAMP(23);
   }
@@ -3489,19 +3506,21 @@
   uint32_t made = 0;
   if (i < S.n) {
     const uint32_t qs = S.qstate[i];
-    const bool stale = (qs & kQueueStale) != 0;
-    const uint32_t qh = stale ? 0u : (qs & 1u);
+    const uint32_t qc = queue_cur(qs);
+    const bool stale = (qs & kQueueStale) != 0 || queue_head(qs) == qc || ((qs >> 2) & 3u) == 3u;
+    const uint32_t qh = stale ? (qc + 1u) % 3u : queue_head(qs);
+    const uint32_t qsp = queue_spare(qc, qh);
     const uint32_t spawn = S.rec[i].b.y;
     const int tag_w = c.plan_dq * 4 + 3;
     uint16_t* plan = reinterpret_cast<uint16_t*>(lds + threadIdx.x * pdw);
-    for (uint32_t l = 0; l < (uint32_t)kQueueDepth; l++) {
-      uint32_t* dst = S.qbuf + (i * kQueueDepth + (qh ^ l)) * (uint64_t)c.qrec_dw;
+    for (uint32_t l = 0; l < 2u; l++) {
+      uint32_t* dst = S.qbuf + (i * kQueueDepth + (l == 0 ? qh : qsp)) * (uint64_t)c.qrec_dw;
       if (stale || dst[tag_w] != queue_tag(spawn + 5u * l)) {
         gen_queue_entry<BIG>(c, S, i, spawn + 5u * l, plan, pdw, dst);
         made++;
       }
     }
-    if (stale) S.qstate[i] = 0;
+    if (stale) S.qstate[i] = (uint8_t)(qc | qh << 2);
   }
   const uint32_t wsum = (uint32_t)__popcll(__ballot(made & 1u)) + 2u * (uint32_t)__popcll(__ballot(made & 2u));
   if ((threadIdx.x & 63) == 0 && wsum) atomicAdd(&S.counters[2], (unsigned long long)wsum);
@@ -3665,7 +3684,8 @@
     for (int k = tid; k < (int)(sizeof(TablesHead) / 4); k += blockDim.x) dstt[k] = src[k];
     uint32_t* dstx = reinterpret_cast<uint32_t*>(&sTX);
     for (int k = tid; k < (int)(sizeof(TablesTail) / 4); k += blockDim.x) dstx[k] = src[kTabHead / 4 + k];
-    for (int t = tid; t < c.nt; t += blockDim.x) plan_s[t] = S.plan[i * (uint64_t)c.plan_stride + t];
+    const uint16_t* prow = S.plan ? plan_row<false>(c, S, i) : plan_row<true>(c, S, i);
+    for (int t = tid; t < c.nt; t += blockDim.x) plan_s[t] = prow[t];
   }
   __syncthreads();
   const EnvView v = rec_load(S.rec, i);
@@ -4010,6 +4030,7 @@
   uint64_t q_launch = 0;
   uint64_t q_grid = 0;
   int q_block = -1;
+  bool slot_plan = false;
   int tune_queue_mode = 0;
   FlatArgs flat{};
   const void* flat_fn = nullptr;
@@ -4027,6 +4048,10 @@
 
 static const void* step_fn(const pgtg_handle* h, int mode) {
   const bool big = h->hcfg.nt > kSmallTiles;
+  if (h->slot_plan) {
+    if (h->hcfg.n_rules > 0) return big ? (const void*)k_env<true, true, true> : (const void*)k_env<true, false, true>;
+    if (mode != MODE_STEP || !h->L.queue) return big ? (const void*)k_env<false, true, true> : (const void*)k_env<false, false, true>;
+  }
   if (h->hcfg.need_car || h->hcfg.n_rules > 0) return big ? (const void*)k_env<true, true> : (const void*)k_env<true, false>;
   if (mode == MODE_STEP && h->L.queue) {
     if (h->q_block == 1) return big ? (const void*)k_envb<true> : (const void*)k_envb<false>;
@@ -4469,7 +4494,9 @@
   if (h->lds > 64 * 1024) {
     const void* fns[] = {(const void*)k_env<true, false>, (const void*)k_env<false, false>, (const void*)k_envq<false>,
                          (const void*)k_env<true, true>, (const void*)k_env<false, true>, (const void*)k_envq<true>,
-                         (const void*)k_envb<false>, (const void*)k_envb<true>};
+                         (const void*)k_envb<false>, (const void*)k_envb<true>,
+                         (const void*)k_env<true, false, true>, (const void*)k_env<false, false, true>,
+                         (const void*)k_env<true, true, true>, (const void*)k_env<false, true, true>};
     for (const void* f : fns) (void)hipFuncSetAttribute(f, hipFuncAttributeMaxDynamicSharedMemorySize, (int)h->lds);
   }
   if (!c.need_car && c.n_rules == 0) {
@@ -4529,7 +4556,6 @@
   ALLOC(h->dcfg, 1);
   ALLOC(S.rec, n);
   ALLOC(S.seed, n);
-  ALLOC(S.plan, n * (uint64_t)c.plan_stride);
   ALLOC(S.err, n);
   ALLOC(S.counters, 4);
   ALLOC(S.wg_ticks, 1);
@@ -4643,8 +4669,21 @@
     pgtg_destroy(h);
     return rc;
   }
+  const bool slot_plan = h->slot_plan = h->L.queue && h->q_block == 0;
+  if (slot_plan && n > (1ull << 30)) {
+    rc = fail(h, PGTG_E_UNSUPPORTED, "more than 2^30 envs with the persistent map-queue step kernel");
+    g_create_err = h->err;
+    pgtg_destroy(h);
+    return rc;
+  }
+  if (!slot_plan && (rc = dalloc(h, &h->S.plan, n * (uint64_t)c.plan_stride))) {
+    g_create_err = h->err;
+    pgtg_destroy(h);
+    return rc;
+  }
   if (h->L.queue) {
     if ((rc = dalloc(h, &h->S.qbuf, n * (uint64_t)queue_depth(h) * (uint64_t)c.qrec_dw)) || (rc = dalloc(h, &h->S.qstate, n)) ||
+        (slot_plan && (rc = hipMemset(h->S.qstate, 0x04, n) == hipSuccess ? 0 : fail(h, PGTG_E_DEVICE, "hipMemset failed"))) ||
         (!h->q_block &&
          ((rc = dalloc(h, &h->S.qreq, 2 * h->q_grid * queue_req_cap((n + h->L.envs - 1) / h->L.envs, h->q_grid, h->L.envs))) ||
           (rc = dalloc(h, &h->S.qovf, 2 * 8 * ((h->q_grid + 7) / 8) * (uint64_t)h->L.envs)) ||
@@ -4874,6 +4913,20 @@
   return 0;
 }
 
+static int read_plan_row(pgtg_handle* h, uint64_t env, std::vector<uint16_t>& p) {
+  const DevCfg& c = h->hcfg;
+  p.assign((size_t)c.plan_stride, 0);
+  if (h->S.plan) {
+    HIPCHK(h, hipMemcpy(p.data(), h->S.plan + env * (uint64_t)c.plan_stride, p.size() * 2, hipMemcpyDeviceToHost));
+    return 0;
+  }
+  uint8_t qs = 0;
+  HIPCHK(h, hipMemcpy(&qs, h->S.qstate + env, 1, hipMemcpyDeviceToHost));
+  const uint32_t* slot = h->S.qbuf + (env * kQueueDepth + queue_cur(qs)) * (uint64_t)c.qrec_dw;
+  HIPCHK(h, hipMemcpy(p.data(), slot, std::min(p.size() * 2, (size_t)c.plan_dq * 16), hipMemcpyDeviceToHost));
+  return 0;
+}
+
 int pgtg_get_env_state(pgtg_handle* h, uint64_t env, PgtgEnvState* st) {
   if (!h || !st || env >= h->n) return PGTG_E_INVALID;
   HIPCHK(h, hipSetDevice(h->device));
@@ -4898,8 +4951,8 @@
   st->spawn_counter = r.b.y;
   st->used_subgoals[0] = (uint64_t)r.b.z | ((uint64_t)r.b.w << 32);
   if (h->hcfg.nt > kSmallTiles) {
-    std::vector<uint16_t> p(h->hcfg.plan_stride);
-    HIPCHK(h, hipMemcpy(p.data(), h->S.plan + env * (uint64_t)h->hcfg.plan_stride, p.size() * 2, hipMemcpyDeviceToHost));
+    std::vector<uint16_t> p;
+    if (int rc = read_plan_row(h, env, p)) return rc;
     st->used_subgoals[0] = 0;
     for (int t = 0; t < h->hcfg.nt; t++) st->used_subgoals[t >> 6] |= (uint64_t)((p[t] & kPlanUsed) != 0) << (t & 63);
   }
@@ -4989,9 +5042,9 @@
   HIPCHK(h, hipSetDevice(h->device));
   HIPCHK(h, hipStreamSynchronize(h->stream));
   const DevCfg& c = h->hcfg;
-  std::vector<uint16_t> p(c.plan_stride);
+  std::vector<uint16_t> p;
   EnvRec r;
-  HIPCHK(h, hipMemcpy(p.data(), h->S.plan + env * (uint64_t)c.plan_stride, c.plan_stride * 2, hipMemcpyDeviceToHost));
+  if (int rc = read_plan_row(h, env, p)) return rc;
   HIPCHK(h, hipMemcpy(&r, h->S.rec + env, sizeof r, hipMemcpyDeviceToHost));
   *w = c.tw;
   *h_ = c.th;
@@ -5263,7 +5316,7 @@
   hd->qrec_dw = (uint32_t)h->hcfg.qrec_dw;
   hd->car_slots = (uint32_t)h->hcfg.car_slots;
   hd->cfg_hash = cfg_hash(h->hcfg);
-  *depth = h->S.qbuf ? queue_depth(h) : 0;
+  *depth = h->S.qbuf ? (queue_depth(h) | (h->S.plan ? 0 : 0x100)) : 0;
 }
 
 static uint64_t section_bytes(const StateSection& s, uint64_t n) {
@@ -5330,7 +5383,7 @@
     return fail(h, PGTG_E_INVALID, std::string(who) + ": the snapshot was created from a handle of another configuration");
   if (depth != s->depth)
     return fail(h, PGTG_E_INVALID, std::string(who) + ": the snapshot was created from a handle with another map-queue step "
-                                                      "kernel (its rings hold another number of maps)");
+                                                      "kernel (its map rings have another layout)");
   memset(T, 0, sizeof *T);
   uint32_t k = 0;
   for (const auto& hs : state_sections(h)) {
```

Measured after the change: 2.749 billion env-steps/s (median of 6 runs). +2.4%, better.
